# tohtsky/myFM

Hardware: AMD Instinct MI355X
Metric: Gibbs iterations/sec (rank=32) (higher is better)
Workload: dtype f64

## Files before the change

### include/myfm_hip.h

```cpp
#ifndef MYFM_HIP_H_
#define MYFM_HIP_H_

#include <stdint.h>

#ifdef __cplusplus
extern "C" {
#endif

#define MFM_OK 0
#define MFM_ERR_INVALID 1
#define MFM_ERR_RUNTIME 2
#define MFM_ERR_DEVICE 3

#define MFM_TASK_REGRESSION 0
#define MFM_TASK_CLASSIFICATION 1
#define MFM_TASK_ORDERED 2

typedef struct mfm_ctx mfm_ctx;
typedef struct mfm_design mfm_design;
typedef struct mfm_store mfm_store;

const char *mfm_version(void);
int mfm_device_count(void);
const char *mfm_global_error(void);

int mfm_create(int device, mfm_ctx **out);
void mfm_destroy(mfm_ctx *ctx);
const char *mfm_last_error(const mfm_ctx *ctx);
int mfm_get_device(const mfm_ctx *ctx);
int mfm_set_stream(mfm_ctx *ctx, void *hip_stream);
int mfm_synchronize(mfm_ctx *ctx);

int mfm_set_allreduce(mfm_ctx *ctx, int (*fn)(void *user, void *dev_buf, int64_t count), void *user);
int mfm_set_shard(mfm_ctx *ctx, int32_t rank, int32_t world);
int mfm_comm_unique_id(void *out128);
int mfm_comm_init(mfm_ctx *ctx, const void *id128, int32_t rank, int32_t world);
int mfm_comm_stats(const mfm_ctx *ctx, int64_t *calls, int64_t *doubles);
int mfm_comm_info(const mfm_ctx *ctx, int32_t *n_ranks, char *path, int64_t path_cap);
int mfm_peer_info(mfm_ctx *ctx, int32_t *pending, void **sum_buf, void **flag_buf, int64_t *sum_bytes, int64_t *flag_bytes);
int mfm_peer_set(mfm_ctx *ctx, int32_t world, int32_t rank, void *const *sum_bufs, void *const *flag_bufs);
int mfm_peer_model_info(mfm_ctx *ctx, void **w_buf, void **V_buf);
int mfm_peer_set_model(mfm_ctx *ctx, int32_t world, int32_t rank, void *const *w_bufs, void *const *V_bufs);
int mfm_peer_export(mfm_ctx *ctx, void *handles256);
int mfm_peer_import(mfm_ctx *ctx, int32_t world, int32_t rank, const void *all_handles);
int mfm_peer_drop(mfm_ctx *ctx);
int mfm_set_main_levels(mfm_ctx *ctx, const int32_t *level, int64_t D0);
int mfm_set_row_offset(mfm_ctx *ctx, int64_t first_global_row);

int mfm_set_main(mfm_ctx *ctx, int64_t N, int64_t D0, const int64_t *indptr, const int32_t *indices,
                 const double *data, const double *y);
int mfm_add_block(mfm_ctx *ctx, int64_t B, int64_t Db, const int64_t *indptr, const int32_t *indices,
                  const double *data, const int64_t *original_to_block);
int mfm_set_groups(mfm_ctx *ctx, const int32_t *group_index, int64_t D, int32_t G);
int mfm_set_residual_policy(mfm_ctx *ctx, int32_t recomputable);
int mfm_finalize(mfm_ctx *ctx, int32_t rank);

int64_t mfm_dim_all(const mfm_ctx *ctx);
int mfm_plan_info(const mfm_ctx *ctx, int64_t *n_levels_main, int64_t *n_launches_per_sweep);
int mfm_plan_flags(const mfm_ctx *ctx);
#define MFM_RES_INFO_FIELDS 13
int mfm_res_info(const mfm_ctx *ctx, int64_t *out, int n_out, char *why, int why_len);
#define MFM_CELL_INFO_FIELDS 74
int mfm_cell_info(const mfm_ctx *ctx, int64_t *out, int n_out, char *why, int why_len);

int mfm_set_state(mfm_ctx *ctx, double w0, const double *w, const double *V);
int mfm_get_state(mfm_ctx *ctx, double *w0, double *w, double *V);
int mfm_set_w0(mfm_ctx *ctx, double w0);
int mfm_zero_w(mfm_ctx *ctx);
int mfm_get_e(mfm_ctx *ctx, double *e);
int mfm_get_q(mfm_ctx *ctx, double *q);
int mfm_set_e(mfm_ctx *ctx, const double *e);

int mfm_reduce_e(mfm_ctx *ctx, double *sum_e, double *sum_e2);
int mfm_shift_e(mfm_ctx *ctx, double delta);
int mfm_group_stats_w(mfm_ctx *ctx, const double *mu_w, double *sum, double *ssd);
int mfm_group_stats_V(mfm_ctx *ctx, const double *mu_V, double *sum, double *ssd);
int mfm_hyper_stats(mfm_ctx *ctx, int32_t need_e, const double *mu_w, const double *mu_V, double *sum_e, double *sum_e2,
                    double *sum_w, double *ssd_w, double *sum_V, double *ssd_V);
int mfm_sweep_w(mfm_ctx *ctx, double alpha, const double *lambda_w, const double *mu_w, const double *z);
int mfm_sweep_V(mfm_ctx *ctx, int32_t f_begin, int32_t f_end, double alpha, const double *lambda_V,
                const double *mu_V, const double *z);
int mfm_sweep_wV(mfm_ctx *ctx, double alpha, double e_shift, const double *lambda_w, const double *mu_w, const double *zw,
                 int32_t f_begin, int32_t f_end, const double *lambda_V, const double *mu_V, const double *zv);

typedef struct mfm_hyper_prior {
  double alpha_0, beta_0, gamma_0, mu_0, reg_0, n_total;
  int32_t fit_w0, reserved;
} mfm_hyper_prior;
int mfm_regression_iteration_ready(mfm_ctx *ctx);
int mfm_regression_iteration(mfm_ctx *ctx, const mfm_hyper_prior *prior, const double *n_in_group, double *alpha, double *w0,
                             double *lambda_w, double *mu_w, double *lambda_V, double *mu_V);
int mfm_update_e_regression(mfm_ctx *ctx);
int mfm_update_e_classification(mfm_ctx *ctx, uint64_t seed, uint64_t draw_index);
int mfm_score_train(mfm_ctx *ctx);

int mfm_oprobit_add_group(mfm_ctx *ctx, int32_t n_class, const int64_t *rows, int64_t n_rows, int32_t *group);
int mfm_oprobit_eval(mfm_ctx *ctx, int32_t group, const double *gamma, double *ll, double *dgamma, double *H);
int mfm_oprobit_sample_z(mfm_ctx *ctx, int32_t group, const double *gamma, uint64_t seed, uint64_t draw_index);

#define MFM_RNG_NORMALS 0
#define MFM_RNG_GAMMA 1
#define MFM_RNG_LATENT 2
typedef struct mfm_rng_op {
  int32_t kind;
  int32_t dest;
  int64_t count;
  int64_t offset;
  double shape;
} mfm_rng_op;
int mfm_rng_prepare(int64_t n_features, int32_t rank, int32_t n_groups);
int mfm_rng_seed_mt19937(mfm_ctx *ctx, const uint32_t *state624, int32_t position);
int mfm_rng_set_program(mfm_ctx *ctx, const mfm_rng_op *ops, int32_t n_ops);
int mfm_rng_prefetch(mfm_ctx *ctx);
int mfm_rng_acquire(mfm_ctx *ctx, double *hyper_variates, int64_t n_hyper_variates);
int mfm_rng_get_z(mfm_ctx *ctx, double *zw, double *zv);

int mfm_update_e_classification_exact(mfm_ctx *ctx, int32_t *status);
int mfm_set_latent_order(mfm_ctx *ctx, const int64_t *rows, int64_t n);
int mfm_oprobit_sample_z_exact(mfm_ctx *ctx, int32_t group, const double *gamma, int32_t *status);
int mfm_latent_stats(mfm_ctx *ctx, int64_t *out8);
int mfm_rng_host_read(mfm_ctx *ctx, uint64_t offset, int64_t n, uint32_t *out);
int mfm_rng_host_advance(mfm_ctx *ctx, uint64_t words);

int mfm_timing_enable(mfm_ctx *ctx, int on);
int mfm_timing_select(mfm_ctx *ctx, int32_t kernel_class);
int mfm_timing_reset(mfm_ctx *ctx);
int mfm_timing_n_classes(void);
const char *mfm_timing_class_name(int cls);
int mfm_timing_get(mfm_ctx *ctx, int cls, double *ms_total, int64_t *launches, double *alg_bytes_total);

int mfm_design_create(int device, int64_t N, int64_t D0, const int64_t *indptr, const int32_t *indices,
                      const double *data, mfm_design **out);
int mfm_design_add_block(mfm_design *d, int64_t B, int64_t Db, const int64_t *indptr, const int32_t *indices,
                         const double *data, const int64_t *original_to_block);
void mfm_design_destroy(mfm_design *d);
const char *mfm_design_last_error(const mfm_design *d);
int64_t mfm_design_dim_all(const mfm_design *d);
int64_t mfm_design_n_rows(const mfm_design *d);
int mfm_design_predict(mfm_design *d, int32_t rank, int32_t n_samples, const double *w0s, const double *ws,
                       const double *Vs, int32_t mode, int32_t n_cut, const double *cutpoints, double *out);

int mfm_store_create(int device, int64_t D, int32_t rank, mfm_store **out);
void mfm_store_destroy(mfm_store *st);
const char *mfm_store_last_error(const mfm_store *st);
int32_t mfm_store_size(const mfm_store *st);
int mfm_store_reserve(mfm_store *st, int32_t n_samples);
int mfm_store_push_ctx(mfm_store *st, mfm_ctx *ctx);
int mfm_store_push_host(mfm_store *st, double w0, const double *w, const double *V);
int mfm_store_get(mfm_store *st, int32_t idx, double *w0, double *w, double *V);
int mfm_design_predict_store(mfm_design *d, mfm_store *st, int32_t first, int32_t count, int32_t mode, int32_t n_cut,
                             const double *cutpoints, double *out);

int mfm_design_summary_store(mfm_design *d, mfm_store *st, int32_t first, int32_t count, int32_t mode, int32_t n_q,
                             const double *probs, const double *precisions, const double *z, int64_t tile_rows,
                             int32_t chunk_samples, double *out_mean, double *out_std, double *out_q);
int mfm_design_summary(mfm_design *d, int32_t rank, int32_t n_samples, const double *w0s, const double *ws, const double *Vs,
                       int32_t mode, int32_t n_q, const double *probs, const double *precisions, const double *z,
                       int64_t tile_rows, int32_t chunk_samples, double *out_mean, double *out_std, double *out_q);

typedef struct mfm_pairs mfm_pairs;
int mfm_pairs_create(int device, int64_t D, int64_t U, const int64_t *q_indptr, const int32_t *q_indices, const double *q_data,
                     int64_t I, const int64_t *c_indptr, const int32_t *c_indices, const double *c_data, mfm_pairs **out);
void mfm_pairs_destroy(mfm_pairs *p);
const char *mfm_pairs_last_error(const mfm_pairs *p);
int mfm_pairs_set_exclude(mfm_pairs *p, const int64_t *indptr, const int32_t *indices);
int mfm_pairs_set_scratch_bound(mfm_pairs *p, int64_t bytes);
int mfm_pairs_add_block(mfm_pairs *p, int32_t side , int64_t col_offset, int64_t width, int64_t block_rows,
                        const int64_t *o2b , const int64_t *indptr, const int32_t *indices, const double *data);
int mfm_pairs_set_cutpoints(mfm_pairs *p, int32_t n_samples, int32_t n_cut, const double *cutpoints );
int mfm_pairs_scores_store(mfm_pairs *p, mfm_store *st, int32_t first, int32_t count, int32_t mode, double *out);
int mfm_pairs_topk_store(mfm_pairs *p, mfm_store *st, int32_t first, int32_t count, int32_t mode, int32_t k, int64_t *idx,
                         double *score);
int mfm_pairs_scores(mfm_pairs *p, int32_t rank, int32_t n_samples, const double *w0s, const double *ws, const double *Vs,
                     int32_t mode, double *out);
int mfm_pairs_topk(mfm_pairs *p, int32_t rank, int32_t n_samples, const double *w0s, const double *ws, const double *Vs,
                   int32_t mode, int32_t k, int64_t *idx, double *score);

int mfm_design_score_ctx(mfm_design *d, mfm_ctx *ctx, double *out);

int mfm_test_erfcx(int device, const double *x, int64_t n, double *out);
int mfm_test_truncated_normal(int device, int32_t kind, double lo, double hi, uint64_t seed, uint64_t draw_index,
                              int64_t n, double *out);

int mfm_host_column_levels(int64_t n_rows, int64_t n_cols, const int64_t *indptr, const int32_t *indices,
                           int32_t *level, int32_t *n_levels);
int mfm_cs_plan_selftest(int64_t n_rows, int32_t n_cols, const int64_t *colptr, const int32_t *rowidx, const double *val, int32_t cg,
                         int32_t lw, int32_t nb, int32_t rd, int32_t cap, double *max_rel_diff, int64_t *info);

typedef struct mfm_vb mfm_vb;
int mfm_vb_create(int device, int64_t N, int64_t D0, const int64_t *indptr, const int32_t *indices, const double *data,
                  const double *y, mfm_vb **out);
int mfm_vb_add_block(mfm_vb *v, int64_t B, int64_t Db, const int64_t *indptr, const int32_t *indices, const double *data,
                     const int64_t *original_to_block);
int mfm_vb_finalize(mfm_vb *v, const int32_t *group_index, int32_t G, int32_t rank);
int mfm_vb_set_stream(mfm_vb *v, void *hip_stream);
int mfm_vb_set_allreduce(mfm_vb *v, int (*fn)(void *user, void *dev_buf, int64_t count), void *user);
int mfm_vb_set_shard(mfm_vb *v, int32_t rank, int32_t world, int64_t n_total_rows, int64_t row_offset);
int mfm_vb_comm_init(mfm_vb *v, const void *id128, int32_t rank, int32_t world);
int mfm_vb_comm_stats(const mfm_vb *v, int64_t *calls, int64_t *doubles);
int mfm_vb_set_levels(mfm_vb *v, const int32_t *level, int64_t D);
int mfm_vb_design_levels(int64_t N, int64_t D0, const int64_t *indptr, const int32_t *indices, const double *data,
                         int32_t n_blocks, const int64_t *block_rows, const int64_t *block_cols,
                         const int64_t *const *block_indptr, const int32_t *const *block_indices,
                         const double *const *block_data, const int64_t *const *block_maps, int32_t *level_out,
                         int32_t *n_levels);
void mfm_vb_destroy(mfm_vb *v);
const char *mfm_vb_last_error(const mfm_vb *v);
int mfm_vb_plan_info(const mfm_vb *v, int64_t *n_levels, int64_t *n_launches_per_iteration);
int mfm_vb_set_state(mfm_vb *v, double w0, double w0_var, const double *w, const double *w_var, const double *V,
                     const double *V_var);
int mfm_vb_get_state(mfm_vb *v, double *w0, double *w0_var, double *w, double *w_var, double *V, double *V_var);
int mfm_vb_set_w0(mfm_vb *v, double w0, double w0_var);
int mfm_vb_update_e(mfm_vb *v, int32_t mode, double *out4);
int mfm_vb_shift_e(mfm_vb *v, double delta);
int mfm_vb_get_e(mfm_vb *v, double *e);
int mfm_vb_get_cache(mfm_vb *v, double *q, double *x2s, double *x3sv);
int mfm_vb_zero_w(mfm_vb *v);
int mfm_vb_sweep_w(mfm_vb *v, double alpha, const double *lambda_w, const double *mu_w);
int mfm_vb_sweep_V(mfm_vb *v, int32_t f_begin, int32_t f_end, double alpha, const double *lambda_V, const double *mu_V);
int mfm_vb_group_stats(mfm_vb *v, int32_t s_begin, int32_t s_end, const double *mu, const double *mu_var, double *out);
int mfm_vb_synchronize(mfm_vb *v);
int mfm_vb_truncated_normal(int32_t right, double mu, double *out3);

#ifdef __cplusplus
}
#endif
#endif
```

### myfm_amd/_capi.py

```python
import ctypes as C
import os

import numpy as np
import scipy.sparse as sps

_HERE = os.path.dirname(os.path.abspath(__file__))
LIB_PATH = os.path.join(_HERE, "libmyfm_hip.so")

MFM_OK, MFM_ERR_INVALID, MFM_ERR_RUNTIME, MFM_ERR_DEVICE = 0, 1, 2, 3
TASK_REGRESSION, TASK_CLASSIFICATION, TASK_ORDERED = 0, 1, 2

SYMBOLS = [
    "mfm_version", "mfm_device_count", "mfm_global_error", "mfm_create", "mfm_destroy", "mfm_last_error",
    "mfm_set_stream", "mfm_synchronize", "mfm_set_main", "mfm_add_block", "mfm_set_groups", "mfm_finalize",
    "mfm_peer_info", "mfm_peer_set", "mfm_peer_model_info", "mfm_peer_set_model", "mfm_peer_export", "mfm_peer_import", "mfm_peer_drop", "mfm_set_residual_policy", "mfm_dim_all", "mfm_plan_info", "mfm_plan_flags", "mfm_res_info", "mfm_cell_info", "mfm_set_state", "mfm_get_state", "mfm_set_w0", "mfm_zero_w", "mfm_get_e",
    "mfm_get_q", "mfm_set_e", "mfm_reduce_e", "mfm_shift_e", "mfm_group_stats_w", "mfm_group_stats_V",
    "mfm_sweep_w", "mfm_sweep_V", "mfm_sweep_wV", "mfm_update_e_regression", "mfm_update_e_classification", "mfm_score_train",
    "mfm_oprobit_add_group", "mfm_oprobit_eval", "mfm_oprobit_sample_z", "mfm_hyper_stats", "mfm_timing_enable", "mfm_timing_select", "mfm_timing_reset",
    "mfm_timing_n_classes", "mfm_timing_class_name", "mfm_timing_get", "mfm_design_create", "mfm_design_add_block",
    "mfm_design_destroy", "mfm_design_last_error", "mfm_design_dim_all", "mfm_design_predict",
    "mfm_host_column_levels", "mfm_rng_prepare", "mfm_rng_seed_mt19937", "mfm_rng_set_program", "mfm_rng_prefetch", "mfm_rng_acquire",
    "mfm_rng_get_z", "mfm_design_score_ctx", "mfm_design_n_rows", "mfm_set_allreduce", "mfm_set_row_offset", "mfm_set_main_levels",
    "mfm_test_erfcx", "mfm_test_truncated_normal", "mfm_get_device", "mfm_set_shard", "mfm_comm_unique_id", "mfm_comm_init",
    "mfm_comm_stats", "mfm_comm_info", "mfm_store_create", "mfm_store_destroy", "mfm_store_last_error", "mfm_store_size", "mfm_store_push_ctx",
# ... 113 lines not shown
    L.mfm_set_allreduce.argtypes = [vp, vp, vp]
    L.mfm_set_row_offset.argtypes = [vp, i64]
    L.mfm_set_main_levels.argtypes = [vp, P, i64]
    L.mfm_get_device.argtypes = [vp]
    L.mfm_set_shard.argtypes = [vp, i32, i32]
    L.mfm_comm_unique_id.argtypes = [P]
    L.mfm_comm_init.argtypes = [vp, P, i32, i32]
    L.mfm_comm_stats.argtypes = [vp, C.POINTER(i64), C.POINTER(i64)]
    L.mfm_comm_info.argtypes = [vp, C.POINTER(i32), C.c_char_p, i64]
    L.mfm_store_create.argtypes = [C.c_int, i64, i32, C.POINTER(vp)]
    L.mfm_store_destroy.argtypes = [vp]
    L.mfm_store_destroy.restype = None
    L.mfm_store_last_error.restype = C.c_char_p
    L.mfm_store_last_error.argtypes = [vp]
    L.mfm_store_size.argtypes = [vp]
    L.mfm_store_reserve.argtypes = [vp, i32]
    L.mfm_store_push_ctx.argtypes = [vp, vp]
    L.mfm_store_push_host.argtypes = [vp, dbl, P, P]
    L.mfm_store_get.argtypes = [vp, i32, C.POINTER(dbl), P, P]
    L.mfm_design_predict_store.argtypes = [vp, vp, i32, i32, i32, i32, P, P]
    L.mfm_design_summary_store.argtypes = [vp, vp, i32, i32, i32, i32, P, P, P, i64, i32, P, P, P]
    L.mfm_design_summary.argtypes = [vp, i32, i32, P, P, P, i32, i32, P, P, P, i64, i32, P, P, P]
    L.mfm_pairs_create.argtypes = [C.c_int, i64, i64, P, P, P, i64, P, P, P, C.POINTER(vp)]
    L.mfm_pairs_destroy.argtypes = [vp]
    L.mfm_pairs_destroy.restype = None
    L.mfm_pairs_last_error.restype = C.c_char_p
    L.mfm_pairs_last_error.argtypes = [vp]
    L.mfm_pairs_set_exclude.argtypes = [vp, P, P]
    L.mfm_pairs_set_scratch_bound.argtypes = [vp, i64]
    L.mfm_pairs_add_block.argtypes = [vp, i32, i64, i64, i64, P, P, P, P]
    L.mfm_pairs_set_cutpoints.argtypes = [vp, i32, i32, P]
    L.mfm_pairs_scores_store.argtypes = [vp, vp, i32, i32, i32, P]
    L.mfm_pairs_topk_store.argtypes = [vp, vp, i32, i32, i32, i32, P, P]
    L.mfm_pairs_scores.argtypes = [vp, i32, i32, P, P, P, i32, P]
    L.mfm_pairs_topk.argtypes = [vp, i32, i32, P, P, P, i32, i32, P, P]
    L.mfm_test_erfcx.argtypes = [C.c_int, P, i64, P]
    L.mfm_test_truncated_normal.argtypes = [C.c_int, i32, dbl, dbl, u64, u64, i64, P]
    _lib = L
    return L


def _p(a):
    return None if a is None else a.ctypes.data_as(C.c_void_p)


def _f64(a):
    return np.ascontiguousarray(a, dtype=np.float64)


def csr_parts(X):
    X = sps.csr_matrix(X, dtype=np.float64)
    return (
        X,
        np.ascontiguousarray(X.indptr, dtype=np.int64),
        np.ascontiguousarray(X.indices, dtype=np.int32),
        np.ascontiguousarray(X.data, dtype=np.float64),
    )


def _raise(code, msg):
    msg = msg.decode() if isinstance(msg, bytes) else msg
    if code == MFM_ERR_INVALID:
        raise ValueError(msg)
    raise RuntimeError(msg)


def column_levels(X):
    X, ip, ix, _ = csr_parts(X)
    level = np.zeros(X.shape[1], dtype=np.int32)
    n = C.c_int32()
    rc = lib().mfm_host_column_levels(X.shape[0], X.shape[1], _p(ip), _p(ix), _p(level), C.byref(n))
    if rc:
        _raise(rc, lib().mfm_global_error())
    return level, n.value


def device_erfcx(x, device=0):
    x = _f64(x)
    out = np.empty_like(x)
    rc = lib().mfm_test_erfcx(device, _p(x), x.size, _p(out))
    if rc:
        _raise(rc, lib().mfm_global_error())
    return out


def device_truncated_normal(kind, lo, hi, n, seed=1, draw_index=0, device=0):
    k = {"left": 0, "right": 1, "twoside": 2}[kind]
    out = np.empty(n)
    rc = lib().mfm_test_truncated_normal(device, k, float(lo), float(hi), seed, draw_index, n, _p(out))
    if rc:
        _raise(rc, lib().mfm_global_error())
    return out


class Context:

    def __init__(self, X, y, blocks=(), rank=4, group_index=None, device=0):
        L = lib()
        h = C.c_void_p()
        rc = L.mfm_create(device, C.byref(h))
        if rc:
            _raise(rc, L.mfm_global_error())
        self.h = h
        X, ip, ix, dv = csr_parts(X)
        y = _f64(y)
        self.N, self.D0 = X.shape
        self._ck(L.mfm_set_main(h, X.shape[0], X.shape[1], _p(ip), _p(ix), _p(dv), _p(y)))
        D = X.shape[1]
        for mp, B in blocks:
            B, bp, bx, bv = csr_parts(B)
            mp = np.ascontiguousarray(mp, dtype=np.int64)
            self._ck(L.mfm_add_block(h, B.shape[0], B.shape[1], _p(bp), _p(bx), _p(bv), _p(mp)))
            D += B.shape[1]
        if group_index is None:
            group_index = np.zeros(D, dtype=np.int32)
        group_index = np.ascontiguousarray(group_index, dtype=np.int32)
        self.G = int(group_index.max()) + 1 if D else 1
        self._ck(L.mfm_set_groups(h, _p(group_index), group_index.shape[0], self.G))
        self._ck(L.mfm_finalize(h, rank))
        self.D, self.K = D, rank

    def _ck(self, rc):
        if rc:
            _raise(rc, lib().mfm_last_error(self.h))

    def close(self):
        if getattr(self, "h", None):
            lib().mfm_destroy(self.h)
            self.h = None

    def __del__(self):
        try:
            self.close()
        except Exception:
            pass

    def set_state(self, w0, w, V):
        w = _f64(w)
        Vt = _f64(np.asarray(V, dtype=np.float64).T)
        self._ck(lib().mfm_set_state(self.h, float(w0), _p(w), _p(Vt)))

    def get_state(self):
        w0 = C.c_double()
        w = np.empty(self.D)
        V = np.empty((self.K, self.D))
        self._ck(lib().mfm_get_state(self.h, C.byref(w0), _p(w), _p(V)))
        return w0.value, w, np.ascontiguousarray(V.T)

    def set_w0(self, w0):
        self._ck(lib().mfm_set_w0(self.h, float(w0)))

    def zero_w(self):
        self._ck(lib().mfm_zero_w(self.h))

    def get_e(self):
        e = np.empty(self.N)
        self._ck(lib().mfm_get_e(self.h, _p(e)))
        return e

    def get_q(self):
        q = np.empty(self.N)
        self._ck(lib().mfm_get_q(self.h, _p(q)))
        return q

    def set_e(self, e):
        e = _f64(e)
        self._ck(lib().mfm_set_e(self.h, _p(e)))

    def reduce_e(self):
        a, b = C.c_double(), C.c_double()
        self._ck(lib().mfm_reduce_e(self.h, C.byref(a), C.byref(b)))
        return a.value, b.value

    def shift_e(self, delta):
        self._ck(lib().mfm_shift_e(self.h, float(delta)))

    def group_stats_w(self, mu_w):
        mu_w = _f64(mu_w)
        s, ss = np.empty(self.G), np.empty(self.G)
        self._ck(lib().mfm_group_stats_w(self.h, _p(mu_w), _p(s), _p(ss)))
        return s, ss

    def group_stats_V(self, mu_V):
        mu = _f64(np.asarray(mu_V).T)
        s, ss = np.empty((self.K, self.G)), np.empty((self.K, self.G))
        self._ck(lib().mfm_group_stats_V(self.h, _p(mu), _p(s), _p(ss)))
        return s.T.copy(), ss.T.copy()

    def sweep_w(self, alpha, lambda_w, mu_w, z):
        lambda_w, mu_w = _f64(lambda_w), _f64(mu_w)
        if z is not None:
            z = _f64(z)
            assert z.shape[0] == self.D
        self._ck(lib().mfm_sweep_w(self.h, float(alpha), _p(lambda_w), _p(mu_w), _p(z)))

    def sweep_V(self, f_begin, f_end, alpha, lambda_V, mu_V, z):
        lam, mu = _f64(np.asarray(lambda_V).T), _f64(np.asarray(mu_V).T)
        if z is not None:
            z = _f64(z)
            assert z.size == (f_end - f_begin) * self.D
        self._ck(lib().mfm_sweep_V(self.h, f_begin, f_end, float(alpha), _p(lam), _p(mu), _p(z)))

    def sweep_wV(self, alpha, e_shift, lambda_w, mu_w, zw, f_begin, f_end, lambda_V, mu_V, zv):
        lambda_w, mu_w = _f64(lambda_w), _f64(mu_w)
        lam, mu = _f64(np.asarray(lambda_V).T), _f64(np.asarray(mu_V).T)
        if zw is not None:
            zw, zv = _f64(zw), _f64(zv)
            assert zw.shape[0] == self.D and zv.size == (f_end - f_begin) * self.D
        self._ck(lib().mfm_sweep_wV(self.h, float(alpha), float(e_shift), _p(lambda_w), _p(mu_w), _p(zw), f_begin, f_end,
                                    _p(lam), _p(mu), _p(zv)))

    def update_e_regression(self):
        self._ck(lib().mfm_update_e_regression(self.h))

    def update_e_classification(self, seed, draw_index):
        self._ck(lib().mfm_update_e_classification(self.h, seed, draw_index))

    def score_train(self):
        self._ck(lib().mfm_score_train(self.h))

    def oprobit_add_group(self, n_class, rows=None):
        g = C.c_int32()
        if rows is None:
            self._ck(lib().mfm_oprobit_add_group(self.h, n_class, None, 0, C.byref(g)))
        else:
            rows = np.ascontiguousarray(rows, dtype=np.int64)
            self._ck(lib().mfm_oprobit_add_group(self.h, n_class, _p(rows), rows.shape[0], C.byref(g)))
        return g.value

    def oprobit_eval(self, group, gamma, want_h=True):
        gamma = _f64(gamma)
        m = gamma.shape[0]
        ll = C.c_double()
        dg = np.empty(m)
        H = np.empty((m, m)) if want_h else None
        self._ck(lib().mfm_oprobit_eval(self.h, group, _p(gamma), C.byref(ll), _p(dg), _p(H)))
        return ll.value, dg, H

    def oprobit_sample_z(self, group, gamma, seed, draw_index):
        gamma = _f64(gamma)
        self._ck(lib().mfm_oprobit_sample_z(self.h, group, _p(gamma), seed, draw_index))

    def synchronize(self):
        self._ck(lib().mfm_synchronize(self.h))

    RNG_OP = np.dtype([("kind", np.int32), ("dest", np.int32), ("count", np.int64), ("offset", np.int64), ("shape", np.float64)])

    def rng_seed_mt19937(self, state624, position):
        st = np.ascontiguousarray(state624, dtype=np.uint32)
        assert st.shape[0] == 624
        self._ck(lib().mfm_rng_seed_mt19937(self.h, _p(st), int(position)))

    def rng_set_program(self, ops):
        arr = np.array([tuple(o) for o in ops], dtype=self.RNG_OP)
        self._n_hv = int(sum(o[2] for o in ops if o[1] == 0))
        self._ck(lib().mfm_rng_set_program(self.h, _p(arr), len(ops)))

    def rng_prefetch(self):
        self._ck(lib().mfm_rng_prefetch(self.h))

    def rng_acquire(self):
        hv = np.empty(max(self._n_hv, 1))
        self._ck(lib().mfm_rng_acquire(self.h, _p(hv), self._n_hv))
        return hv[: self._n_hv]

    def rng_get_z(self):
        zw, zv = np.empty(self.D), np.empty((max(self.K, 1), self.D))
        self._ck(lib().mfm_rng_get_z(self.h, _p(zw), _p(zv)))
        return zw, zv[: self.K]

    def update_e_classification_exact(self):
        st = C.c_int32()
        self._ck(lib().mfm_update_e_classification_exact(self.h, C.byref(st)))
        return st.value

    def oprobit_sample_z_exact(self, group, gamma):
        gamma = _f64(gamma)
        st = C.c_int32()
        self._ck(lib().mfm_oprobit_sample_z_exact(self.h, group, _p(gamma), C.byref(st)))
        return st.value

    def latent_stats(self):
        out = np.zeros(8, dtype=np.int64)
        self._ck(lib().mfm_latent_stats(self.h, _p(out)))
        return dict(zip(("status", "chunks", "subs", "lq", "quads", "walkers", "attempts"), (int(v) for v in out)))

    def rng_host_read(self, offset, n):
        out = np.empty(max(int(n), 1), dtype=np.uint32)
        self._ck(lib().mfm_rng_host_read(self.h, int(offset), int(n), _p(out)))
        return out[: int(n)]

    def rng_host_advance(self, words):
        self._ck(lib().mfm_rng_host_advance(self.h, int(words)))

    def set_residual_policy(self, recomputable):
        self._ck(lib().mfm_set_residual_policy(self.h, 1 if recomputable else 0))

    def plan_flags(self):
        f = lib().mfm_plan_flags(self.h)
        return {"qfree": bool(f & 1), "unit": bool(f & 2), "ell": bool(f & 4), "sharded": bool(f & 8), "soa": bool(f & 16),
                "fused_next": bool(f & 32), "sharded_fused": bool(f & 64), "mf": bool(f & 128), "resident": bool(f & 256), "cell": bool(f & 512), "streamed_chain": bool(f & 1024), "resident_overflow": bool(f & 2048)}

    RES_INFO = ("ready", "G", "RV", "RL", "RX", "umax", "n_items", "item_bits", "n_runs", "max_wg_users", "max_slice_items",
                "e_where", "n_rows")
    E_WHERE = ("rows", "slots", "slots_with_sums", "cell", "dropped")

    def res_info(self):
        out = np.zeros(len(self.RES_INFO), dtype=np.int64)
        why = C.create_string_buffer(256)
        self._ck(lib().mfm_res_info(self.h, _p(out), out.shape[0], why, len(why)))
        d = dict(zip(self.RES_INFO, (int(v) for v in out)))
        d["ready"] = bool(d["ready"])
        d["e_where"] = self.E_WHERE[d["e_where"]]
        d["why"] = why.value.decode()
        return d

    CELL_INFO = ("ready", "G", "umax", "item32", "n_streams", "n_fields", "N", "Npad", "max_steps", "chunk_max", "chunk_min",
                 "chunks_empty", "split_mask", "score_fb")
    CELL_STREAM_TYPE = ("U", "I", "C")
    CELL_MAX_STREAMS, CELL_MAX_FIELDS = 4, 16
    CELL_INFO_FIELDS = len(CELL_INFO) + 3 * CELL_MAX_STREAMS + 3 * CELL_MAX_FIELDS

    def cell_info(self):
        out = np.zeros(self.CELL_INFO_FIELDS, dtype=np.int64)
        why = C.create_string_buffer(256)
        self._ck(lib().mfm_cell_info(self.h, _p(out), out.shape[0], why, len(why)))
        n = len(self.CELL_INFO)
        nf = n + 3 * self.CELL_MAX_STREAMS
        d = dict(zip(self.CELL_INFO, (int(v) for v in out[:n])))
        d["ready"], d["item32"] = bool(d["ready"]), bool(d["item32"])
        d["streams"] = [(self.CELL_STREAM_TYPE[int(out[n + 3 * s])], int(out[n + 3 * s + 1]), int(out[n + 3 * s + 2]))
                        for s in range(d["n_streams"])]
        d["fields"] = [tuple(int(x) for x in out[nf + 3 * k:nf + 3 * k + 3]) for k in range(d["n_fields"])]
        d["why"] = why.value.decode()
        return d

    def plan_info(self):
        a, b = C.c_int64(), C.c_int64()
        lib().mfm_plan_info(self.h, C.byref(a), C.byref(b))
        return a.value, b.value

    def timing_enable(self, on=True):
        self._ck(lib().mfm_timing_enable(self.h, int(on)))

    def timing_reset(self):
        self._ck(lib().mfm_timing_reset(self.h))

    def timing(self):
        L = lib()
        out = {}
        for c in range(L.mfm_timing_n_classes()):
            ms, n, by = C.c_double(), C.c_int64(), C.c_double()
            self._ck(L.mfm_timing_get(self.h, c, C.byref(ms), C.byref(n), C.byref(by)))
            if n.value:
                out[L.mfm_timing_class_name(c).decode()] = (ms.value, n.value, by.value)
        return out


class Design:

    def __init__(self, X, blocks=(), device=0):
        L = lib()
        h = C.c_void_p()
        X, ip, ix, dv = csr_parts(X)
        rc = L.mfm_design_create(device, X.shape[0], X.shape[1], _p(ip), _p(ix), _p(dv), C.byref(h))
        if rc:
            _raise(rc, L.mfm_global_error())
        self.h = h
        self.N = X.shape[0]
        for mp, B in blocks:
            B, bp, bx, bv = csr_parts(B)
            mp = np.ascontiguousarray(mp, dtype=np.int64)
            if mp.shape[0] != self.N:
                self.close()
                raise ValueError("Relation blocks have inconsistent mapper size with case_size")
            rc = L.mfm_design_add_block(h, B.shape[0], B.shape[1], _p(bp), _p(bx), _p(bv), _p(mp))
            if rc:
                msg = L.mfm_design_last_error(h)
                self.close()
                _raise(rc, msg)
        self.D = L.mfm_design_dim_all(h)

    def close(self):
        if getattr(self, "h", None):
            lib().mfm_design_destroy(self.h)
            self.h = None

    def __del__(self):
        try:
            self.close()
        except Exception:
            pass

    def score_ctx(self, ctx):
        out = np.empty(self.N)
        rc = lib().mfm_design_score_ctx(self.h, ctx.h, _p(out))
        if rc:
            _raise(rc, lib().mfm_design_last_error(self.h))
        return out

    def predict(self, samples, mode=0, cutpoints=None):
        K, S, w0s, ws, Vs = _pack_samples(samples)
        n_cut = 0
        cp = None
        if mode == 2:
            cp = _f64(np.stack([np.asarray(c, dtype=np.float64) for c in cutpoints]))
            n_cut = cp.shape[1]
        out = np.empty((self.N, n_cut + 1) if mode == 2 else self.N)
        rc = lib().mfm_design_predict(self.h, K, S, _p(w0s), _p(ws), _p(Vs), mode, n_cut, _p(cp), _p(out))
        if rc:
            _raise(rc, lib().mfm_design_last_error(self.h))
        return out

    def summary(self, samples, mode=0, quantiles=(), precisions=None, tile_rows=0, chunk_samples=0):
        K, S, w0s, ws, Vs = _pack_samples(samples)
        probs, prec, z, mean, std, q = _summary_args(self.N, quantiles, precisions)
        rc = lib().mfm_design_summary(self.h, K, S, _p(w0s), _p(ws), _p(Vs), mode, len(probs), _p(probs), _p(prec), _p(z),
                                      int(tile_rows), int(chunk_samples), _p(mean), _p(std), _p(q))
        if rc:
            _raise(rc, lib().mfm_design_last_error(self.h))
        return mean, std, q


def _summary_args(N, quantiles, precisions):
    from statistics import NormalDist

    probs = _f64(quantiles).reshape(-1)
    prec = None if precisions is None else _f64(precisions).reshape(-1)
    z = None
    if prec is not None:
        z = _f64([NormalDist().inv_cdf(float(p)) if 0.0 < p < 1.0 else np.nan for p in probs])
    return probs, prec, z, np.empty(N), np.empty(N), np.empty((len(probs), N))


class Store:

    def __init__(self, D, K, device=0):
        h = C.c_void_p()
        rc = lib().mfm_store_create(device, D, K, C.byref(h))
        if rc:
            _raise(rc, lib().mfm_global_error())
        self.h, self.D, self.K = h, D, K

    def close(self):
        if getattr(self, "h", None):
            lib().mfm_store_destroy(self.h)
            self.h = None

    def __del__(self):
        try:
            self.close()
        except Exception:
            pass

    def _ck(self, rc):
        if rc:
            _raise(rc, lib().mfm_store_last_error(self.h))

    def __len__(self):
        return lib().mfm_store_size(self.h)

    def push_ctx(self, ctx):
        self._ck(lib().mfm_store_push_ctx(self.h, ctx.h))

    def push(self, w0, w, V):
        w, Vt = _f64(w), _f64(np.asarray(V, dtype=np.float64).T)
        self._ck(lib().mfm_store_push_host(self.h, float(w0), _p(w), _p(Vt)))

    def get(self, idx):
        w0, w, V = C.c_double(), np.empty(self.D), np.empty((self.K, self.D))
        self._ck(lib().mfm_store_get(self.h, idx, C.byref(w0), _p(w), _p(V)))
        return w0.value, w, np.ascontiguousarray(V.T)

    def predict(self, design, mode=0, cutpoints=None, first=0, count=None):
        count = len(self) - first if count is None else count
        n_cut, cp = 0, None
        if mode == 2:
            cp = _f64(np.stack([np.asarray(c, dtype=np.float64) for c in cutpoints]))
            n_cut = cp.shape[1]
        out = np.empty((design.N, n_cut + 1) if mode == 2 else design.N)
        rc = lib().mfm_design_predict_store(design.h, self.h, first, count, mode, n_cut, _p(cp), _p(out))
        if rc:
            _raise(rc, lib().mfm_design_last_error(design.h))
        return out

    def summary(self, design, mode=0, quantiles=(), precisions=None, first=0, count=None, tile_rows=0, chunk_samples=0):
        count = len(self) - first if count is None else count
        probs, prec, z, mean, std, q = _summary_args(design.N, quantiles, precisions)
        rc = lib().mfm_design_summary_store(design.h, self.h, first, count, mode, len(probs), _p(probs), _p(prec), _p(z),
                                            int(tile_rows), int(chunk_samples), _p(mean), _p(std), _p(q))
        if rc:
            _raise(rc, lib().mfm_design_last_error(design.h))
        return mean, std, q


def _pack_samples(samples):
    S = len(samples)
    K = np.asarray(samples[0][2]).shape[1] if S else 0
    w0s = _f64([s[0] for s in samples])
    ws = _f64(np.stack([np.asarray(s[1], dtype=np.float64) for s in samples])) if S else np.empty(0)
    Vs = _f64(np.stack([np.asarray(s[2], dtype=np.float64).T for s in samples])) if S else np.empty(0)
    return K, S, w0s, ws, Vs


class Pairs:

    def __init__(self, X_query, X_cand, exclude=None, scratch_bound=None, device=0, rel_query=(), rel_cand=(), cutpoints=None):
        L = lib()
        h = C.c_void_p()
        Xq, qp, qx, qv = csr_parts(X_query)
        Xc, cp, cx, cv = csr_parts(X_cand)
        if Xq.shape[1] != Xc.shape[1]:
            raise ValueError("X_query and X_cand differ in width")
        rc = L.mfm_pairs_create(device, Xq.shape[1], Xq.shape[0], _p(qp), _p(qx), _p(qv), Xc.shape[0], _p(cp), _p(cx), _p(cv),
                                C.byref(h))
        if rc:
            _raise(rc, L.mfm_pairs_last_error(None))
        self.h, self.U, self.I, self.D = h, Xq.shape[0], Xc.shape[0], Xq.shape[1]
        if exclude is not None:
            E = sps.csr_matrix(exclude)
            if E.shape != (self.U, self.I):
                self.close()
                raise ValueError("exclude must have shape (n_queries, n_candidates)")
            ep = np.ascontiguousarray(E.indptr, dtype=np.int64)
            ex = np.ascontiguousarray(E.indices, dtype=np.int32)
            self._ck(L.mfm_pairs_set_exclude(h, _p(ep), _p(ex)))
        if scratch_bound is not None:
            self._ck(L.mfm_pairs_set_scratch_bound(h, int(scratch_bound)))
        try:
            for side, rels in ((0, rel_query), (1, rel_cand)):
                for off, o2b, B in rels:
                    B, bp, bx, bv = csr_parts(B)
                    o2b = np.ascontiguousarray(o2b, dtype=np.int64)
                    if o2b.shape != ((self.U, self.I)[side],):
                        raise ValueError("a block's o2b must have one entry per row of its side")
                    self._ck(L.mfm_pairs_add_block(h, side, int(off), B.shape[1], B.shape[0], _p(o2b), _p(bp), _p(bx), _p(bv)))
            if cutpoints is not None:
                cp = _f64(np.atleast_2d(np.asarray(cutpoints, dtype=np.float64)))
                self._ck(L.mfm_pairs_set_cutpoints(h, cp.shape[0], cp.shape[1], _p(cp)))
        except Exception:
            self.close()
            raise

    def _ck(self, rc):
        if rc:
            _raise(rc, lib().mfm_pairs_last_error(self.h))

    def close(self):
        if getattr(self, "h", None):
            lib().mfm_pairs_destroy(self.h)
            self.h = None

    def __del__(self):
        try:
            self.close()
        except Exception:
            pass

    def scores(self, samples, mode=0):
        K, S, w0s, ws, Vs = _pack_samples(samples)
        out = np.empty((self.U, self.I))
        self._ck(lib().mfm_pairs_scores(self.h, K, S, _p(w0s), _p(ws), _p(Vs), mode, _p(out)))
        return out

    def topk(self, samples, k, mode=0):
        K, S, w0s, ws, Vs = _pack_samples(samples)
        kk = max(int(k), 1)
        idx, val = np.empty((self.U, kk), dtype=np.int64), np.empty((self.U, kk))
        self._ck(lib().mfm_pairs_topk(self.h, K, S, _p(w0s), _p(ws), _p(Vs), mode, int(k), _p(idx), _p(val)))
        return idx, val

    def scores_store(self, store, mode=0, first=0, count=None):
        count = len(store) - first if count is None else count
        out = np.empty((self.U, self.I))
        self._ck(lib().mfm_pairs_scores_store(self.h, store.h, first, count, mode, _p(out)))
        return out

    def topk_store(self, store, k, mode=0, first=0, count=None):
        count = len(store) - first if count is None else count
        kk = max(int(k), 1)
        idx, val = np.empty((self.U, kk), dtype=np.int64), np.empty((self.U, kk))
        self._ck(lib().mfm_pairs_topk_store(self.h, store.h, first, count, mode, int(k), _p(idx), _p(val)))
        return idx, val
```

### myfm_amd/csrc/mfm_hip.hip

```cpp
#include <algorithm>
#include <cerrno>
#include <chrono>
#include <cmath>
#include <cstdio>
#include <cstring>
#include <map>
#include <memory>
#include <mutex>
#include <string>
#include <thread>
#include <type_traits>
#include <vector>

#include <fcntl.h>
#include <sys/file.h>
#include <sys/stat.h>
#include <unistd.h>

#include <hipcub/hipcub.hpp>

#include "mfm_common.hpp"
#include "mfm_kernels.hpp"
#include "mfm_plan.hpp"
#include "mfm_res_plan.hpp"
// ... 1273 lines not shown
    std::vector<int32_t> fs((size_t)c->D);
    std::vector<int64_t> cur(gptr.begin(), gptr.end() - 1);
    for (int64_t j = 0; j < c->D; j++) fs[cur[c->hgroup[j]]++] = (int32_t)j;
    c->group_ptr.upload(gptr);
    c->feat_sorted.upload(fs);
    int64_t big = 1;
    for (int g = 0; g < c->G; g++) big = std::max(big, gptr[g + 1] - gptr[g]);
    c->gs_chunks = (int)((big + GS_CHUNK - 1) / GS_CHUNK);
  }
  int64_t off = c->D0;
  int max_chunks = std::max(c->plan_V.max_hchunks, c->plan_W.max_hchunks);
  int max_long = std::max(c->plan_V.max_huge, c->plan_W.max_huge);
  {
    std::vector<std::unique_ptr<DevBlock>> built(c->hblocks.size());
    std::vector<std::exception_ptr> errs(c->hblocks.size());
    std::vector<int64_t> offs(c->hblocks.size());
    for (size_t b = 0; b < c->hblocks.size(); b++) {
      offs[b] = off;
      off += c->hblocks[b].X.cols;
    }
    auto build_one = [&](size_t b) {
      try {
        MFM_HIP_CHECK(hipSetDevice(c->device));
        built[b].reset(new DevBlock());
        built[b]->col_off = offs[b];
        built[b]->build(c->hblocks[b].X, c->hblocks[b].map.get(), c->N, c->KS, c->stream, c->cell_w,
                        b < c->pre_maps.size() ? &c->pre_maps[b] : nullptr);
      } catch (...) {
        errs[b] = std::current_exception();
      }
    };
    {
      (void)coop_capacity<PBlockV>();
      (void)coop_capacity<PBlockW>();
      std::vector<std::thread> pool;
      const bool par = c->hblocks.size() > 1;
      for (size_t b = 0; b < c->hblocks.size(); b++) {
        if (par && b + 1 < c->hblocks.size())
          pool.emplace_back(build_one, b);
        else
          build_one(b);
      }
      for (auto &t : pool) t.join();
    }
    for (size_t b = 0; b < built.size(); b++) {
      if (errs[b]) std::rethrow_exception(errs[b]);
      std::unique_ptr<DevBlock> &B = built[b];
      max_chunks = std::max({max_chunks, B->plan_V.max_hchunks, B->plan_W.max_hchunks});
      max_long = std::max({max_long, B->plan_V.max_huge, B->plan_W.max_huge});
      B->allreduce_fields(c->stream, c->comm, 6, 1);
      c->blocks.push_back(std::move(B));
    }
  }
  c->ls.reserve(std::max(max_chunks, 1), std::max(max_long, 1));
  c->w.alloc_zero((size_t)c->D, c->stream);
  c->V.alloc_zero((size_t)c->D * c->K, c->stream);
  c->Vt.alloc_zero((size_t)c->D * c->KS, c->stream);
  c->z.alloc((size_t)std::max<int64_t>(c->D, 1) * std::max(c->K, 1));
  c->lam.alloc((size_t)c->G * std::max(c->K, 1));
  c->mu.alloc((size_t)c->G * std::max(c->K, 1));
  c->red_partial.alloc(REDUCE_BLOCKS);
  c->red_out.alloc((size_t)1 + (size_t)c->G * std::max(c->K, 1));
  c->scratch_n.alloc((size_t)std::max<int64_t>(c->N, 1));
  if (c->v_path != VPath::Deferred) c->v_path = decide_main_paths(c);
  if (c->res.ready) {
    if (c->v_path != VPath::Deferred && env_flag("MFM_PLAN_CHECK")) {
      ResPlan chk;
      chk.build(Xt_keep, c->plan_V.h_level, &c->hgroup, c->res_plan_cus);
      const std::string diff = chk.ready ? res_plan_compare(c->res, chk, c->stream) : ("host builder: " + chk.why);
      if (!diff.empty()) throw Error(MFM_ERR_RUNTIME, "plan check: device and host resident layouts differ (" + diff + ")");
      lap("resident plan (host, check)");
    }
  } else if (!c->res_refused && c->v_path == VPath::TwoField && c->X.unit && c->N >= res_min_rows(c) && !env_flag("MFM_NO_RESIDENT")) {
    plan_resident(c, [&](ResPlan &rp, int n_cu) { rp.build(Xt_keep, c->plan_V.h_level, &c->hgroup, n_cu); }, tlog);
    lap("resident plan (host)");
  }
  if (c->v_path == VPath::ShardedTwoField && c->comm.shard_set && c->comm.world <= RES_MAX_PEERS && c->comm.world > 1 &&
      !env_flag("MFM_NO_RESIDENT") && !env_flag("MFM_NO_SHARDED_RESIDENT")) {
    const int64_t min_rows = res_min_rows(c);
    const bool want = c->X.unit && c->X.ell_width == 2 && c->N >= std::max<int64_t>(1, min_rows / c->comm.world) && c->K > 0;
    bool mine = false;
    if (want) {
      std::vector<char> draw_empty((size_t)c->D0, 0);
      for (int64_t j = 0; j < c->D0; j++) draw_empty[j] = (size_t)j < c->plan_V.special.size() && c->plan_V.special[j] == 2;
      plan_resident(c, [&](ResPlan &rp, int n_cu) {
        rp.allow_overflow = false;
        res_plan_build_device(rp, c->X, &c->hgroup, n_cu, c->stream, &c->hlevels, &draw_empty);
      }, tlog);
      if (c->res.ready && env_flag("MFM_PLAN_CHECK")) {
        ResPlan chk;
        chk.allow_overflow = false;
        chk.build(Xt_keep, c->hlevels, &c->hgroup, c->res_plan_cus, &draw_empty);
        const std::string diff = chk.ready ? res_plan_compare(c->res, chk, c->stream) : ("host builder: " + chk.why);
        if (!diff.empty()) throw Error(MFM_ERR_RUNTIME, "plan check: device and host resident layouts differ (sharded; " + diff + ")");
      }
      mine = c->res.ready;
      c->res.ready = false;
    }
    if (mine) {
      try {
        c->res.alloc_exchange(c->comm.world, c->comm.rank, c->stream);
      } catch (const Error &) {
        mine = false;
      }
    }
    double bad = mine ? 0.0 : 1.0;
    {
      DevBuf<double> d;
      d.upload(&bad, 1);
      c->comm.allreduce(d.p, 1);
      MFM_HIP_CHECK(hipStreamSynchronize(c->stream));
      MFM_HIP_CHECK(hipMemcpy(&bad, d.p, sizeof(double), hipMemcpyDeviceToHost));
    }
    if (bad == 0.0) {
      c->res_sharded_pending = true;
    } else {
      c->drop_resident();
    }
    lap("resident plan (row-sharded)");
  }
  Xt_keep = HostCsr();
  MFM_HIP_CHECK(hipStreamSynchronize(c->stream));
  lap("blocks, state, scratch");
  lap("(sync)");
  c->hX = HostCsr();
  c->hX_valid = false;
  c->hy = std::vector<double>();
  c->hblocks.clear();
  c->pre_maps.clear();
  lap("host copies released");
  c->finalized = true;
  MFM_CATCH(ctx)
}

int mfm_peer_info(mfm_ctx *ctx, int32_t *pending, void **sum_buf, void **flag_buf, int64_t *sum_bytes, int64_t *flag_bytes) {
  MFM_TRY(ctx)
  ctx->need_final();
  const bool p = ctx->res_sharded_pending;
  if (pending) *pending = p ? 1 : 0;
  if (sum_buf) *sum_buf = p ? (void *)ctx->res.xsum.p : nullptr;
  if (flag_buf) *flag_buf = p ? (void *)ctx->res.xflag.p : nullptr;
  if (sum_bytes) *sum_bytes = p ? (int64_t)(ctx->res.xsum.n * sizeof(double)) : 0;
  if (flag_bytes) *flag_bytes = p ? (int64_t)(ctx->res.xflag.n * sizeof(unsigned long long)) : 0;
  MFM_CATCH(ctx)
}

int mfm_peer_set(mfm_ctx *ctx, int32_t world, int32_t rank, void *const *sum_bufs, void *const *flag_bufs) {
  MFM_TRY(ctx)
  ctx->need_final();
  mfm_ctx *c = ctx;
  if (!c->res_sharded_pending) throw Error(MFM_ERR_RUNTIME, "mfm_peer_set: this context has no row-sharded persistent sweep waiting for its peers");
  if (world != c->res.xworld || rank != c->res.xrank) throw Error(MFM_ERR_INVALID, "mfm_peer_set: world / rank differ from the communicator's");
  for (int r = 0; r < world; r++) {
    if (!sum_bufs[r] || !flag_bufs[r]) throw Error(MFM_ERR_INVALID, "mfm_peer_set: null buffer");
    c->res.peer_sum[r] = (double *)sum_bufs[r];
    c->res.peer_flag[r] = (unsigned long long *)flag_bufs[r];
  }
  if (c->res.peer_sum[rank] != c->res.xsum.p || c->res.peer_flag[rank] != c->res.xflag.p)
    throw Error(MFM_ERR_INVALID, "mfm_peer_set: this rank's own entry must be the buffers of mfm_peer_info");
  MFM_HIP_CHECK(hipStreamSynchronize(c->stream));
  c->res.peers_set = true;
  c->res.ready = true;
  c->res_sharded_pending = false;
  MFM_CATCH(ctx)
}

int mfm_peer_set_model(mfm_ctx *ctx, int32_t world, int32_t rank, void *const *w_bufs, void *const *V_bufs) {
  MFM_TRY(ctx)
  ctx->need_final();
  mfm_ctx *c = ctx;
  if (!c->res.ready || !c->res.peers_set) throw Error(MFM_ERR_RUNTIME, "mfm_peer_set_model: mfm_peer_set comes first");
  if (world != c->res.xworld || rank != c->res.xrank) throw Error(MFM_ERR_INVALID, "mfm_peer_set_model: world / rank differ from the communicator's");
  for (int r = 0; r < world; r++) {
    if (!w_bufs[r] || (c->K > 0 && !V_bufs[r])) throw Error(MFM_ERR_INVALID, "mfm_peer_set_model: null buffer");
    c->res.peer_w[r] = (double *)w_bufs[r];
    c->res.peer_V[r] = (double *)V_bufs[r];
  }
  if (c->res.peer_w[rank] != c->w.p || c->res.peer_V[rank] != c->V.p)
    throw Error(MFM_ERR_INVALID, "mfm_peer_set_model: this rank's own entry must be its own w / V (mfm_peer_model_info)");
  MFM_HIP_CHECK(hipStreamSynchronize(c->stream));
  c->res.peers_model = true;
  MFM_CATCH(ctx)
}

int mfm_peer_model_info(mfm_ctx *ctx, void **w_buf, void **V_buf) {
  MFM_TRY(ctx)
  ctx->need_final();
  if (w_buf) *w_buf = ctx->w.p;
  if (V_buf) *V_buf = ctx->V.p;
  MFM_CATCH(ctx)
}

int mfm_peer_export(mfm_ctx *ctx, void *handles256) {
  MFM_TRY(ctx)
  ctx->need_final();
  if (!ctx->res_sharded_pending) throw Error(MFM_ERR_RUNTIME, "mfm_peer_export: no row-sharded persistent sweep waiting for its peers");
  static_assert(sizeof(hipIpcMemHandle_t) == 64, "IPC handle size");
  hipIpcMemHandle_t h[4];
  std::memset(h, 0, sizeof h);
  MFM_HIP_CHECK(hipIpcGetMemHandle(&h[0], ctx->res.xsum.p));
  MFM_HIP_CHECK(hipIpcGetMemHandle(&h[1], ctx->res.xflag.p));
  MFM_HIP_CHECK(hipIpcGetMemHandle(&h[2], ctx->w.p));
  if (ctx->K > 0) MFM_HIP_CHECK(hipIpcGetMemHandle(&h[3], ctx->V.p));
  std::memcpy(handles256, h, sizeof h);
  MFM_CATCH(ctx)
}

int mfm_peer_import(mfm_ctx *ctx, int32_t world, int32_t rank, const void *all_handles) {
  MFM_TRY(ctx)
  ctx->need_final();
  mfm_ctx *c = ctx;
  if (!c->res_sharded_pending) throw Error(MFM_ERR_RUNTIME, "mfm_peer_import: no row-sharded persistent sweep waiting for its peers");
  if (world != c->res.xworld || rank != c->res.xrank) throw Error(MFM_ERR_INVALID, "mfm_peer_import: world / rank differ from the communicator's");
  void *sums[RES_MAX_PEERS], *flags[RES_MAX_PEERS], *ws[RES_MAX_PEERS], *Vs[RES_MAX_PEERS];
  for (int r = 0; r < world; r++) {
    if (r == rank) {
      sums[r] = c->res.xsum.p;
      flags[r] = c->res.xflag.p;
      ws[r] = c->w.p;
      Vs[r] = c->V.p;
      continue;
    }
    hipIpcMemHandle_t h[4];
    std::memcpy(h, (const char *)all_handles + (size_t)r * 256, sizeof h);
    MFM_HIP_CHECK(hipIpcOpenMemHandle(&sums[r], h[0], hipIpcMemLazyEnablePeerAccess));
    c->res.peer_mapped.push_back(sums[r]);
    MFM_HIP_CHECK(hipIpcOpenMemHandle(&flags[r], h[1], hipIpcMemLazyEnablePeerAccess));
    c->res.peer_mapped.push_back(flags[r]);
    MFM_HIP_CHECK(hipIpcOpenMemHandle(&ws[r], h[2], hipIpcMemLazyEnablePeerAccess));
    c->res.peer_mapped.push_back(ws[r]);
    Vs[r] = nullptr;
    if (c->K > 0) {
      MFM_HIP_CHECK(hipIpcOpenMemHandle(&Vs[r], h[3], hipIpcMemLazyEnablePeerAccess));
      c->res.peer_mapped.push_back(Vs[r]);
    }
  }
  int rc = mfm_peer_set(ctx, world, rank, sums, flags);
  if (rc != MFM_OK) return rc;
  if (env_int("MYFM_PEER_MODEL", 0) != 0) {
    rc = mfm_peer_set_model(ctx, world, rank, ws, Vs);
    if (rc != MFM_OK) return rc;
  }
  MFM_CATCH(ctx)
}

int mfm_peer_drop(mfm_ctx *ctx) {
  MFM_TRY(ctx)
  ctx->need_final();
  MFM_HIP_CHECK(hipStreamSynchronize(ctx->stream));
  materialize_e(ctx);
  ctx->drop_resident();
  MFM_CATCH(ctx)
}

int mfm_set_residual_policy(mfm_ctx *ctx, int32_t recomputable) {
  if (!ctx) return MFM_ERR_INVALID;
  ctx->e_recomputable = recomputable != 0;
  return MFM_OK;
}

int64_t mfm_dim_all(const mfm_ctx *ctx) { return ctx->D; }

int mfm_plan_info(const mfm_ctx *ctx, int64_t *n_levels_main, int64_t *n_launches_per_sweep) {
  if (ctx->v_path == VPath::Deferred) {
    if (n_levels_main) *n_levels_main = 2;
    if (n_launches_per_sweep) *n_launches_per_sweep = 1;
    return MFM_OK;
  }
  if (n_levels_main) *n_levels_main = (int64_t)ctx->plan_V.n_levels;
  if (n_launches_per_sweep) {
    int64_t n = ctx->plan_V.launches;
    for (auto &B : ctx->blocks) n += B->plan_V.launches + 3;
    *n_launches_per_sweep = n;
  }
  return MFM_OK;
}

int mfm_plan_flags(const mfm_ctx *ctx) {
  bool streamed = false;
  for (auto &B : ctx->blocks)
    for (const Step &st : B->plan_V.steps) streamed = streamed || (st.is_chain && st.chain.stream);
  int form = 0;
  switch (ctx->v_path) {
    case VPath::QFree: form = 1; break;
    case VPath::Split: form = 16; break;
    case VPath::SplitFused: form = 16 | 32; break;
    case VPath::TwoField: form = 16 | 32 | 128; break;
    case VPath::ShardedSplit: form = 64; break;
    case VPath::ShardedTwoField: form = 64 | 128; break;
    case VPath::Deferred:
    case VPath::Generic:
    case VPath::Cell:
      break;
  }
  return (streamed ? 1024 : 0) | (ctx->res.ready && ctx->res.RX > 0 ? 2048 : 0) | form | (ctx->X.unit ? 2 : 0) | (ctx->X.ell_width >= 0 ? 4 : 0) |
         (ctx->comm.active() ? 8 : 0) | (ctx->res.ready ? 256 : 0) | (ctx->cell.ready ? 512 : 0);
}

int mfm_res_info(const mfm_ctx *ctx, int64_t *out, int n_out, char *why, int why_len) {
  if (!ctx || n_out < 0 || (n_out > 0 && !out) || why_len < 0 || (why_len > 0 && !why)) return MFM_ERR_INVALID;
  const ResPlan &rp = ctx->res;
  const int64_t v[MFM_RES_INFO_FIELDS] = {rp.ready ? 1 : 0, rp.G,       rp.RV,     rp.RL,           rp.RX,
                                          rp.umax,          rp.n_items, rp.item_bits, rp.n_runs,    rp.max_wg_users,
                                          rp.max_slice_items, (int64_t)ctx->e_where, rp.n_rows};
  for (int i = 0; i < n_out; i++) out[i] = i < MFM_RES_INFO_FIELDS ? v[i] : 0;
  if (why_len > 0) {
    std::strncpy(why, rp.ready ? "" : rp.why.c_str(), (size_t)why_len - 1);
    why[why_len - 1] = 0;
  }
  return MFM_OK;
}

int mfm_cell_info(const mfm_ctx *ctx, int64_t *out, int n_out, char *why, int why_len) {
  if (!ctx || n_out < 0 || (n_out > 0 && !out) || why_len < 0 || (why_len > 0 && !why)) return MFM_ERR_INVALID;
  const CellPlan &cp = ctx->cell;
  int64_t v[MFM_CELL_INFO_FIELDS] = {0};
  const int m = (int)cp.fields.size(), ns = (int)cp.streams.size();
  int64_t split = 0;
  const bool typed = ns > 0 && cp.sU == 0;
  for (int k = 0; k < m && typed; k++)
    if (cp.split_pass(k == 0 ? m - 1 : k - 1, k, k == 0)) split |= (int64_t)1 << k;
  const int64_t head[14] = {cp.ready ? 1 : 0, cp.G,         cp.umax,      cp.item32 ? 1 : 0, ns,    m, cp.N, cp.Npad, cp.max_steps,
                            cp.chunk_max,     cp.chunk_min, cp.chunks_empty, split,          cp.ready ? cp.score_fb() : 0};
  for (int i = 0; i < 14; i++) v[i] = head[i];
  for (int i = 0; i < ns && i < CELL_MAX_STREAMS; i++) {
    v[14 + 3 * i] = cp.streams[i].type;
    v[15 + 3 * i] = cp.streams[i].slot;
    v[16 + 3 * i] = cp.streams[i].card;
  }
  for (int k = 0; k < m && k < CELL_MAX_FIELDS; k++) {
    v[14 + 3 * CELL_MAX_STREAMS + 3 * k] = cp.fields[k].stream;
    v[15 + 3 * CELL_MAX_STREAMS + 3 * k] = cp.fields[k].kind;
    v[16 + 3 * CELL_MAX_STREAMS + 3 * k] = cp.fields[k].n;
  }
  for (int i = 0; i < n_out; i++) out[i] = i < MFM_CELL_INFO_FIELDS ? v[i] : 0;
  if (why_len > 0) {
    std::strncpy(why, cp.ready ? "" : cp.why.c_str(), (size_t)why_len - 1);
    why[why_len - 1] = 0;
  }
  return MFM_OK;
}

int mfm_set_state(mfm_ctx *ctx, double w0, const double *w, const double *V) {
  MFM_TRY(ctx)
  ctx->need_final();
  ctx->w0 = w0;
  ctx->ring.upload(ctx->w.p, w, (size_t)ctx->D * sizeof(double), ctx->stream);
  if (ctx->K) ctx->ring.upload(ctx->V.p, V, (size_t)ctx->D * ctx->K * sizeof(double), ctx->stream);
  MFM_CATCH(ctx)
}

int mfm_get_state(mfm_ctx *ctx, double *w0, double *w, double *V) {
  MFM_TRY(ctx)
  ctx->need_final();
  *w0 = ctx->w0;
  if (ctx->D)
    MFM_HIP_CHECK(hipMemcpyAsync(w, ctx->w.p, (size_t)ctx->D * sizeof(double), hipMemcpyDeviceToHost, ctx->stream));
  if (ctx->K && ctx->D)
    MFM_HIP_CHECK(
        hipMemcpyAsync(V, ctx->V.p, (size_t)ctx->D * ctx->K * sizeof(double), hipMemcpyDeviceToHost, ctx->stream));
  ctx->sync_and_check();
  MFM_CATCH(ctx)
}

int mfm_set_w0(mfm_ctx *ctx, double w0) {
  MFM_TRY(ctx)
  if (w0 != ctx->w0) ensure_e(ctx);
  ctx->w0 = w0;
  MFM_CATCH(ctx)
}

int mfm_zero_w(mfm_ctx *ctx) {
  MFM_TRY(ctx)
  ctx->need_final();
  if (ctx->D) MFM_HIP_CHECK(hipMemsetAsync(ctx->w.p, 0, (size_t)ctx->D * sizeof(double), ctx->stream));
  MFM_CATCH(ctx)
}

static int get_eq(mfm_ctx *ctx, double *dst, int which) {
  MFM_TRY(ctx)
  ctx->need_final();
  materialize_e(ctx);
  if (ctx->N) {
    hipLaunchKernelGGL(k_get_eq, dim3(cdiv(ctx->N, WG)), dim3(WG), 0, ctx->stream, ctx->eq_rows(), ctx->scratch_n.p, ctx->N,
                       which);
    MFM_HIP_CHECK(
        hipMemcpyAsync(dst, ctx->scratch_n.p, (size_t)ctx->N * sizeof(double), hipMemcpyDeviceToHost, ctx->stream));
    MFM_HIP_CHECK(hipStreamSynchronize(ctx->stream));
  }
  MFM_CATCH(ctx)
}
int mfm_get_e(mfm_ctx *ctx, double *e) { return get_eq(ctx, e, 0); }
int mfm_get_q(mfm_ctx *ctx, double *q) {
  if (ctx->finalized && ctx->q_stale_factor >= 0) {
    try {
      ctx->use_device();
      for (auto &B : ctx->blocks)
        if (ctx->cell.ready) block_rowcache(ctx->stream, ctx->timing, *B, ctx->V.p + (size_t)ctx->q_stale_factor * ctx->D + B->col_off, true);
      launch_qbuild(ctx, ctx->V.p + (size_t)ctx->q_stale_factor * ctx->D);
      ctx->q_stale_factor = -1;
    } catch (const std::exception &ex) {
      ctx->err = ex.what();
      return MFM_ERR_RUNTIME;
    }
  }
  return get_eq(ctx, q, 1);
}
int mfm_set_e(mfm_ctx *ctx, const double *e) {
  MFM_TRY(ctx)
  ctx->need_final();
  if (ctx->e_where == EWhere::Dropped) ctx->e_where = EWhere::Rows;
  ctx->e_is_residual = false;
  materialize_e(ctx);
  if (ctx->N) {
    MFM_HIP_CHECK(hipStreamSynchronize(ctx->stream));
    MFM_HIP_CHECK(hipMemcpy(ctx->scratch_n.p, e, (size_t)ctx->N * sizeof(double), hipMemcpyHostToDevice));
    hipLaunchKernelGGL(k_set_eq, dim3(cdiv(ctx->N, WG)), dim3(WG), 0, ctx->stream, ctx->eq_rows(), ctx->scratch_n.p, ctx->N, 0);
    MFM_HIP_CHECK(hipStreamSynchronize(ctx->stream));
  }
  MFM_CATCH(ctx)
}

int mfm_reduce_e(mfm_ctx *ctx, double *sum_e, double *sum_e2) {
  MFM_TRY(ctx)
  ctx->need_final();
  materialize_e(ctx);
  hipStream_t s = ctx->stream;
  {
    TimedLaunch t(ctx->timing, s, KC_REDUCE_E, 8.0 * ctx->N);
    hipLaunchKernelGGL(k_reduce_e_partial, dim3(REDUCE_BLOCKS), dim3(WG), 0, s, ctx->eq_rows(), ctx->N, ctx->red_partial.p);
    hipLaunchKernelGGL(k_reduce_final, dim3(1), dim3(WG), 0, s, ctx->red_partial.p, REDUCE_BLOCKS, ctx->red_out.p);
  }
  ctx->comm.allreduce(ctx->red_out.p, 2);
  double2 *h = ctx->readback(2);
  MFM_HIP_CHECK(hipMemcpyAsync(h, ctx->red_out.p, sizeof(double2), hipMemcpyDeviceToHost, s));
  MFM_HIP_CHECK(hipMemcpyAsync(h + 1, ctx->ls.error.p, sizeof(int), hipMemcpyDeviceToHost, s));
  MFM_HIP_CHECK(hipStreamSynchronize(s));
  ctx->check_coresident(*(const int *)(h + 1));
  *sum_e = h[0].x;
  *sum_e2 = h[0].y;
  MFM_CATCH(ctx)
}

int mfm_shift_e(mfm_ctx *ctx, double delta) {
  MFM_TRY(ctx)
  ctx->need_final();
  materialize_e(ctx);
  ctx->e_is_residual = false;
  if (ctx->N) {
    TimedLaunch t(ctx->timing, ctx->stream, KC_SHIFT_E, 16.0 * ctx->N);
    hipLaunchKernelGGL(k_shift_e, dim3(cdiv(ctx->N, WG)), dim3(WG), 0, ctx->stream, ctx->eq_rows(), ctx->N, delta);
    MFM_HIP_CHECK(hipGetLastError());
  }
  MFM_CATCH(ctx)
}

static int group_stats(mfm_ctx *ctx, const double *theta, int nf, const double *mu_host, double *sum, double *ssd) {
  MFM_TRY(ctx)
  ctx->need_final();
  hipStream_t s = ctx->stream;
  const int G = ctx->G;
  if (nf > 0) {
    ctx->ring.upload(ctx->mu.p, mu_host, (size_t)G * nf * sizeof(double), s);
    {
      TimedLaunch t(ctx->timing, s, KC_GROUP_STATS, 12.0 * ctx->D * nf);
      const int n_ch = std::max(1, ctx->gs_chunks);
      if (ctx->gs_partial.n < (size_t)G * nf * n_ch) ctx->gs_partial.alloc((size_t)G * nf * n_ch);
      hipLaunchKernelGGL(k_group_stats, dim3(G, nf, n_ch), dim3(WG), 0, s, theta, ctx->D, ctx->feat_sorted.p,
                         ctx->group_ptr.p, ctx->mu.p, G, ctx->gs_partial.p);
      hipLaunchKernelGGL(k_group_stats_final, dim3(cdiv(G * nf, 64)), dim3(64), 0, s, ctx->gs_partial.p, G * nf, n_ch,
                         ctx->red_out.p + 1);
    }
    if (ctx->res.peers_model && ctx->comm.active()) ctx->comm.allreduce(ctx->red_out.p, 1);
    double2 *h = ctx->readback((size_t)G * nf + 1);
    MFM_HIP_CHECK(hipMemcpyAsync(h, ctx->red_out.p + 1, (size_t)G * nf * sizeof(double2), hipMemcpyDeviceToHost, s));
    MFM_HIP_CHECK(hipStreamSynchronize(s));
    for (int i = 0; i < G * nf; i++) {
      sum[i] = h[i].x;
      ssd[i] = h[i].y;
    }
  }
  MFM_CATCH(ctx)
}
int mfm_group_stats_w(mfm_ctx *ctx, const double *mu_w, double *sum, double *ssd) {
  return group_stats(ctx, ctx->w.p, 1, mu_w, sum, ssd);
}
int mfm_group_stats_V(mfm_ctx *ctx, const double *mu_V, double *sum, double *ssd) {
  return group_stats(ctx, ctx->V.p, ctx->K, mu_V, sum, ssd);
}

int mfm_hyper_stats(mfm_ctx *ctx, int32_t need_e, const double *mu_w, const double *mu_V, double *sum_e, double *sum_e2,
                    double *sum_w, double *ssd_w, double *sum_V, double *ssd_V) {
  MFM_TRY(ctx)
  ctx->need_final();
  mfm_ctx *c = ctx;
  const bool slot_sums = need_e && c->e_where == EWhere::SlotsWithSums;
  if (need_e && !slot_sums) materialize_e(ctx);
  hipStream_t s = c->stream;
  const int G = c->G, K = c->K, n_ch = std::max(1, c->gs_chunks);
  const size_t n_out = 1 + (size_t)G * (K + 1);
  if (c->hs_out.n < n_out) c->hs_out.alloc(n_out);
  if (c->hs_mu.n < (size_t)G * (K + 1)) c->hs_mu.alloc((size_t)G * (K + 1));
  if (c->gs_partial.n < (size_t)G * (K + 1) * n_ch) c->gs_partial.alloc((size_t)G * (K + 1) * n_ch);
  {
    c->hs_stage.resize((size_t)G * (K + 1));
    std::memcpy(c->hs_stage.data(), mu_w, (size_t)G * sizeof(double));
    if (K) std::memcpy(c->hs_stage.data() + G, mu_V, (size_t)G * K * sizeof(double));
    c->ring.upload(c->hs_mu.p, c->hs_stage.data(), c->hs_stage.size() * sizeof(double), s);
  }
  {
    TimedLaunch t(c->timing, s, KC_GROUP_STATS, 12.0 * c->D * (K + 1));
    hipLaunchKernelGGL(k_group_stats, dim3(G, 1, n_ch), dim3(WG), 0, s, c->w.p, c->D, c->feat_sorted.p, c->group_ptr.p,
                       c->hs_mu.p, G, c->gs_partial.p);
    if (K)
      hipLaunchKernelGGL(k_group_stats, dim3(G, K, n_ch), dim3(WG), 0, s, c->V.p, c->D, c->feat_sorted.p, c->group_ptr.p,
                         c->hs_mu.p + G, G, c->gs_partial.p + (size_t)G * n_ch);
    hipLaunchKernelGGL(k_group_stats_final, dim3(cdiv(G * (K + 1), 64)), dim3(64), 0, s, c->gs_partial.p, G * (K + 1), n_ch,
                       c->hs_out.p + 1);
  }
  if (slot_sums) {
    TimedLaunch t(c->timing, s, KC_REDUCE_E, 16.0 * c->res.G);
    hipLaunchKernelGGL(k_reduce_final, dim3(1), dim3(WG), 0, s, c->res.sums.p, c->res.G, c->hs_out.p);
    c->comm.allreduce(c->hs_out.p, 2);
  } else if (need_e) {
    TimedLaunch t(c->timing, s, KC_REDUCE_E, 8.0 * c->N);
    hipLaunchKernelGGL(k_reduce_e_partial, dim3(REDUCE_BLOCKS), dim3(WG), 0, s, c->eq_rows(), c->N, c->red_partial.p);
    hipLaunchKernelGGL(k_reduce_final, dim3(1), dim3(WG), 0, s, c->red_partial.p, REDUCE_BLOCKS, c->hs_out.p);
    c->comm.allreduce(c->hs_out.p, 2);
  }
  if (!need_e && c->res.peers_model && c->comm.active()) c->comm.allreduce(c->hs_out.p, 1);
  MFM_HIP_CHECK(hipGetLastError());
  double2 *h = c->readback(n_out + 1);
  MFM_HIP_CHECK(hipMemcpyAsync(h, c->hs_out.p, n_out * sizeof(double2), hipMemcpyDeviceToHost, s));
  MFM_HIP_CHECK(hipMemcpyAsync(h + n_out, c->ls.error.p, sizeof(int), hipMemcpyDeviceToHost, s));
  MFM_HIP_CHECK(hipStreamSynchronize(s));
  c->check_coresident(*(const int *)(h + n_out));
  if (need_e) {
    *sum_e = h[0].x;
    *sum_e2 = h[0].y;
  }
  for (int g = 0; g < G; g++) {
    sum_w[g] = h[1 + g].x;
    ssd_w[g] = h[1 + g].y;
  }
  for (int i = 0; i < G * K; i++) {
    sum_V[i] = h[1 + G + i].x;
    ssd_V[i] = h[1 + G + i].y;
  }
  MFM_CATCH(ctx)
}

static void sync_model_sharded(mfm_ctx *c, bool with_w, int f_begin, int f_end) {
  hipStream_t s = c->stream;
  if (with_w) {
    hipLaunchKernelGGL(k_mask_rows, dim3(cdiv(c->D, 256)), dim3(256), 0, s, c->w.p, c->sync_mask.p, c->D, c->D);
    c->comm.allreduce(c->w.p, c->D);
  }
  if (f_end > f_begin) {
    const int64_t n = (int64_t)(f_end - f_begin) * c->D;
    double *Vb = c->V.p + (size_t)f_begin * c->D;
    hipLaunchKernelGGL(k_mask_rows, dim3(cdiv(n, 256)), dim3(256), 0, s, Vb, c->sync_mask.p, c->D, n);
    c->comm.allreduce(Vb, n);
  }
}

struct ResidentLinear {
  double *w = nullptr;
  const double *zw = nullptr, *lam_w = nullptr, *mu_w = nullptr;
  double e_shift = 0.0;
};
static void launch_resident(mfm_ctx *c, int f_begin, int f_end, const double *zbase, const double *lam, const double *mu, double alpha,
                            const ResidentLinear &lin = ResidentLinear(), const double *hyp = nullptr) {
  ensure_e(c);
  const mfm_ctx::ResidentE e = c->e_for_resident(lin.w != nullptr, f_begin, f_end);
  run_sweep_resident(c->stream, c->timing, c->res, KC_SWEEP_V_RESIDENT, c->eq_raw(), c->V.p, c->D, f_begin, f_end, zbase, lam, mu,
                     c->group.p, c->G, alpha, c->ls.error.p, lin.w, lin.zw, lin.lam_w, lin.mu_w, lin.e_shift, e.load_slots, e.no_store,
                     hyp);
  c->e_left_by_resident(e);
  c->q_stale_factor = f_end - 1;
  if (c->comm.active() && !c->res.peers_model) sync_model_sharded(c, lin.w != nullptr, f_begin, f_end);
}

int mfm_sweep_w(mfm_ctx *ctx, double alpha, const double *lambda_w, const double *mu_w, const double *z) {
  MFM_TRY(ctx)
  ctx->need_final();
  if (!ctx->cell_w) materialize_e(ctx);
  mfm_ctx *c = ctx;
  hipStream_t s = c->stream;
  c->ring.upload(c->lam.p, lambda_w, (size_t)c->G * sizeof(double), s);
  c->ring.upload(c->mu.p, mu_w, (size_t)c->G * sizeof(double), s);
  const double *zdev = c->z.p;
  if (z) {
    c->ring.upload(c->z.p, z, (size_t)c->D * sizeof(double), s);
  } else {
    if (c->rng.current < 0 || c->rng.n_zw != c->D)
      throw Error(MFM_ERR_RUNTIME, "mfm_sweep_w(z = NULL) needs an acquired device random set with D z_w variates");
    zdev = c->rng.slot[c->rng.current].zw.p;
  }
  if (c->cell_w) {
    run_sweep_w_cell(c, zdev, alpha);
    return MFM_OK;
  }
  c->ensure_main_plans();
  SweepArgs a = main_args(c, c->w.p, zdev, c->lam.p, c->mu.p, alpha);
  const SweepClasses kcw{KC_SWEEP_W_LIGHT, KC_SWEEP_W_HEAVY, KC_SWEEP_W_COOP, KC_SWEEP_W_LSTATS, KC_SWEEP_W_LDRAW,
                         KC_SWEEP_W_LAPPLY, KC_SWEEP_W_CHAIN, KC_SWEEP_W_SCAT};
  if (c->comm.active())
// ... 627 lines not shown
```

### myfm_amd/csrc/mfm_res.hpp

```cpp
#pragma once
#include <algorithm>
#include <cstdlib>
#include <cstring>
#include <atomic>
#include <string>
#include <thread>
#include <vector>

#include "mfm_common.hpp"
#include "mfm_mf_kernels.hpp"

namespace mfm {

#ifndef MFM_RES_CH
#define MFM_RES_CH 4
#endif
constexpr int RES_MAX_PEERS = 8;

struct ResArgs {
  double2 *eq;
  const double *e_in;
  double *e_slots;
  const int32_t *perm;
  const uint32_t *uidw;
  const uint32_t *headw;
  const int32_t *run_item;
  const int32_t *first_run;
  const int32_t *wg_run_ptr;
  const int32_t *wg_nruns;
  const int32_t *wg_user_ptr;
  const int2 *user_desc;
  const int32_t *wg_item_ptr;
  const int32_t *ent_ptr;
  const int2 *entries;
  const int32_t *scols;
  const int2 *item_desc;
  double *partials;
  double *dv;
  double *V;
  int64_t D;
  int f_begin, f_end;
  int linear;
  int n_sw;
  double *w;
  const double *zw;
  const double *lam_w, *mu_w;
  double e_shift;
  const double *z;
  const double *lam, *mu;
  const int32_t *group;
  int n_groups;
  double alpha;
  const double *scal;
  int n_items, umax;
  unsigned long long *bar;
  int n_wg;
  int *error;
  unsigned long long *prof;
  int xworld, xrank;
  unsigned long long xepoch0;
  double *xsum[RES_MAX_PEERS];
  unsigned long long *xflag[RES_MAX_PEERS];
  unsigned long long *xarrive;
  int xmodel;
  double *xw[RES_MAX_PEERS], *xV[RES_MAX_PEERS];
  int ngx;
  int no_store;
  int xch_break;
};

__device__ __forceinline__ void res_store2(double *p, double a, double b) {
  __hip_atomic_store(p, a, __ATOMIC_RELAXED, __HIP_MEMORY_SCOPE_AGENT);
  __hip_atomic_store(p + 1, b, __ATOMIC_RELAXED, __HIP_MEMORY_SCOPE_AGENT);
}

enum { RES_BAR_START = 0, RES_BAR_TOP = 16, RES_BAR_XCNT = 32, RES_BAR_GEN = 160, RES_BAR_CENSUS = 288, RES_BAR_WORDS = 416 };
struct ResBar {
  int xcc;
  unsigned long long n_x, nx;
};

__device__ __forceinline__ bool res_spin(const ResArgs &a, const unsigned long long *w, unsigned long long target, bool &dead) {
  unsigned spins = 0;
  while (__hip_atomic_load(w, __ATOMIC_RELAXED, __HIP_MEMORY_SCOPE_AGENT) < target) {
#ifndef MFM_RES_NO_SLEEP
    __builtin_amdgcn_s_sleep(1);
#endif
    if ((++spins & 1023u) == 0u) {
      if (spins > (1u << 22) || __hip_atomic_load(a.error, __ATOMIC_RELAXED, __HIP_MEMORY_SCOPE_AGENT) != 0) {
        __hip_atomic_store(a.error, 1, __ATOMIC_RELAXED, __HIP_MEMORY_SCOPE_AGENT);
        dead = true;
        return false;
      }
    }
  }
  return true;
}

__device__ __forceinline__ bool res_spin_sys(const ResArgs &a, const unsigned long long *w, unsigned long long target, bool &dead) {
  unsigned spins = 0;
  while (__hip_atomic_load(w, __ATOMIC_RELAXED, __HIP_MEMORY_SCOPE_SYSTEM) < target) {
    __builtin_amdgcn_s_sleep(2);
    if ((++spins & 1023u) == 0u) {
      const int seen = __hip_atomic_load(a.error, __ATOMIC_RELAXED, __HIP_MEMORY_SCOPE_AGENT);
      if (spins > (1u << 23) || seen != 0) {
        if (seen == 0) __hip_atomic_store(a.error, 2, __ATOMIC_RELAXED, __HIP_MEMORY_SCOPE_AGENT);
        dead = true;
        return false;
      }
    }
  }
  return true;
}

__device__ __forceinline__ void res_bar_init(const ResArgs &a, ResBar &rb, bool &dead) {
  unsigned x;
  asm volatile("s_getreg_b32 %0, hwreg(HW_REG_XCC_ID, 0, 4)" : "=s"(x));
  rb.xcc = (int)(x & 7u);
  __hip_atomic_fetch_add(a.bar + RES_BAR_CENSUS + 16 * rb.xcc, 1ull, __ATOMIC_RELAXED, __HIP_MEMORY_SCOPE_AGENT);
  asm volatile("s_waitcnt vmcnt(0)" ::: "memory");
  __hip_atomic_fetch_add(a.bar + RES_BAR_START, 1ull, __ATOMIC_RELAXED, __HIP_MEMORY_SCOPE_AGENT);
  rb.n_x = 1;
  rb.nx = 1;
  if (!res_spin(a, a.bar + RES_BAR_START, (unsigned long long)a.n_wg, dead)) return;
  rb.nx = 0;
  for (int i = 0; i < 8; i++) {
    const unsigned long long c = __hip_atomic_load(a.bar + RES_BAR_CENSUS + 16 * i, __ATOMIC_RELAXED, __HIP_MEMORY_SCOPE_AGENT);
    rb.nx += c > 0 ? 1 : 0;
    if (i == rb.xcc) rb.n_x = c;
  }
}

__device__ __forceinline__ void res_grid_barrier(const ResArgs &a, const ResBar &rb, unsigned long long k, int tid, bool &dead) {
  asm volatile("s_waitcnt vmcnt(0)" ::: "memory");
  __syncthreads();
  if (tid == 0 && !dead) {
    const unsigned long long old =
        __hip_atomic_fetch_add(a.bar + RES_BAR_XCNT + 16 * rb.xcc, 1ull, __ATOMIC_RELAXED, __HIP_MEMORY_SCOPE_AGENT);
    if (old + 1 == k * rb.n_x) {
      __builtin_amdgcn_fence(__ATOMIC_RELEASE, "agent");
      asm volatile("s_waitcnt vmcnt(0)" ::: "memory");
      __hip_atomic_fetch_add(a.bar + RES_BAR_TOP, 1ull, __ATOMIC_RELAXED, __HIP_MEMORY_SCOPE_AGENT);
      if (res_spin(a, a.bar + RES_BAR_TOP, k * rb.nx, dead))
        __hip_atomic_store(a.bar + RES_BAR_GEN + 16 * rb.xcc, k, __ATOMIC_RELAXED, __HIP_MEMORY_SCOPE_AGENT);
    } else {
      res_spin(a, a.bar + RES_BAR_GEN + 16 * rb.xcc, k, dead);
    }
    __builtin_amdgcn_fence(__ATOMIC_ACQUIRE, "agent");
  }
  __syncthreads();
}

typedef double res_d16_t __attribute__((ext_vector_type(16)));
typedef unsigned res_u4_t __attribute__((ext_vector_type(4)));

template <int NT, int NGV, int NGL, bool XCH = false, bool OVF = false>
__global__ __launch_bounds__(NT) void k_mf_resident(ResArgs a) {
  extern __shared__ __attribute__((aligned(16))) char res_smem[];
  constexpr int NW = NT / WAVE, NG = NGV + NGL, R = 16 * NG, RL = 16 * NGL;
  constexpr int B = 4;
  const int g = (int)blockIdx.x, tid = threadIdx.x, lane = tid & 63;
  const int wv = __builtin_amdgcn_readfirstlane(tid >> 6);
  const int U = a.umax;
  const double alpha_k = a.scal ? a.scal[0] : a.alpha, e_shift_k = a.scal ? a.scal[2] : a.e_shift;
  const int ngx = OVF ? a.ngx : 0, NGt = NG + ngx, Rt = 16 * NGt;
  d2_t *utab = (d2_t *)res_smem;
  double *elds = (double *)(utab + U);
  double *acc1 = elds + (size_t)RL * NT;
  double *acc2 = acc1 + NW * U;
  d2_t *wcarry = (d2_t *)(acc2 + NW * U);
  int *wflag = (int *)(wcarry + NW);
  const int32_t *perm_g = a.perm + (int64_t)g * Rt * NT;
  const int u0 = a.wg_user_ptr[g], nu = a.wg_user_ptr[g + 1] - u0;
  const int rb0 = a.wg_run_ptr[g];
  const int pad_item = a.n_items;
  const unsigned rb0b = 4u * (unsigned)rb0, padb = 16u * (unsigned)pad_item;
  const char *run_item_b = (const char *)a.run_item, *dv_b = (const char *)a.dv;
  double *acc1w = acc1 + wv * U, *acc2w = acc2 + wv * U;
  bool dead = false;
  unsigned long long nbar = 0;
  ResBar rbar;
  rbar.xcc = 0;
  rbar.n_x = rbar.nx = 1;
#define RES_STAMP0(k) \
  if (a.prof && tid == 0) a.prof[(int64_t)g * a.n_sw * 64 + 56 + (k)] = __builtin_amdgcn_s_memrealtime()
  RES_STAMP0(0);
  if (tid == 0) res_bar_init(a, rbar, dead);
  RES_STAMP0(1);
  const int wv_hi = wv >> 2;
#define RES_PRIO(j)                  \
  if ((((j) & 1) ^ wv_hi) != 0)      \
    __builtin_amdgcn_s_setprio(1);   \
  else                               \
    __builtin_amdgcn_s_setprio(0)
  const int trash_run = a.wg_run_ptr[g] + a.wg_nruns[g];
#define RES_STAMP(k)                                                                                      \
  if (a.prof && tid == 0) a.prof[((int64_t)g * a.n_sw + (f - f_first)) * 64 + (k)] = __builtin_amdgcn_s_memrealtime()

  for (int i = tid; i < 2 * NW * U; i += NT) acc1[i] = 0.0;
  for (int i = tid; i < U; i += NT) utab[i] = d2_t{0.0, 0.0};

  res_u4_t uw[NG];
  unsigned ux[NG];
  unsigned hbv[NG], nbv[NG];
#pragma unroll
  for (int j = 0; j < NG; j++) {
#pragma unroll
    for (int w = 0; w < 4; w++) uw[j][w] = a.uidw[((int64_t)g * (5 * NGt) + 5 * j + w) * NT + tid];
    ux[j] = a.uidw[((int64_t)g * (5 * NGt) + 5 * j + 4) * NT + tid];
    hbv[j] = a.headw[((int64_t)g * NGt + j) * NT + tid];
    nbv[j] = hbv[j] | (j == 0 ? 1u : 0u);
  }
  const unsigned nbx0 = OVF && ngx > 0 ? a.headw[((int64_t)g * NGt + NG) * NT + tid] : 0u;
  double *eog = OVF ? a.e_slots + ((int64_t)g * Rt + 16 * NG) * NT + tid : nullptr;
  const uint32_t *uidw_x = a.uidw + ((int64_t)g * (5 * NGt) + 5 * NG) * NT + tid;
  const uint32_t *headw_x = a.headw + ((int64_t)g * NGt + NG) * NT + tid;
  const int run0 = a.first_run[g * NT + tid];
  const bool head0 = (hbv[0] & 1u) != 0u;
#define RES_NIB(j, q) ((((nbv[j]) | ((j) + 1 < NG ? nbv[(j) + 1 < NG ? (j) + 1 : (j)] << 16 : nbx0 << 16)) >> (4 * (q))) & 15u)
#define RES_UIDS(j, bb, uid)                                                     \
  {                                                                              \
    const unsigned lo_ = uw[j][bb];                                              \
    uid[0] = (int)(lo_ & 0x3ffu);                                                \
    uid[1] = (int)((lo_ >> 10) & 0x3ffu);                                        \
    uid[2] = (int)((lo_ >> 20) & 0x3ffu);                                        \
    uid[3] = (int)((lo_ >> 30) | (((ux[j] >> (8 * (bb))) & 0xffu) << 2));        \
  }

#define RES_UIDSX(bb, uid)                                                       \
  {                                                                              \
    const unsigned lo_ = uwx[bb];                                                \
    uid[0] = (int)(lo_ & 0x3ffu);                                                \
    uid[1] = (int)((lo_ >> 10) & 0x3ffu);                                        \
    uid[2] = (int)((lo_ >> 20) & 0x3ffu);                                        \
    uid[3] = (int)((lo_ >> 30) | (((uxx >> (8 * (bb))) & 0xffu) << 2));          \
  }

#define RES_OPAQUE()                                                                            \
  _Pragma("unroll") for (int j_ = 0; j_ < NG; j_++) {                                           \
    asm volatile("" : "+v"(uw[j_]), "+v"(ux[j_]), "+v"(hbv[j_]), "+v"(nbv[j_]));                \
  }
  res_d16_t ev[NGV > 0 ? NGV : 1];
#pragma unroll
  for (int j = 0; j < NG; j++) {
#pragma unroll 1
    for (int bb = 0; bb < 4; bb++) {
      int row[B];
#pragma unroll
      for (int k = 0; k < B; k++) row[k] = a.e_in ? 0 : perm_g[(16 * j + 4 * bb + k) * NT + tid];
#pragma unroll
      for (int k = 0; k < B; k++) {
        const double x = (a.e_in ? a.e_in[((int64_t)g * Rt + 16 * j + 4 * bb + k) * NT + tid] : a.eq[row[k] < 0 ? 0 : row[k]].x) + e_shift_k;
        if (j < NGV)
          ev[j < NGV ? j : 0][4 * bb + k] = x;
        else
          elds[(16 * (j - NGV) + 4 * bb + k) * NT + tid] = x;
      }
    }
  }
  if (OVF) {
    for (int jx = 0; jx < ngx; jx++) {
#pragma unroll 4
      for (int i = 0; i < 16; i++) {
        const int64_t sl = 16 * (NG + jx) + i;
        const int row = a.e_in ? 0 : perm_g[sl * NT + tid];
        const double x = (a.e_in ? a.e_in[((int64_t)g * Rt + sl) * NT + tid] : a.eq[row < 0 ? 0 : row].x) + e_shift_k;
        eog[(16 * jx + i) * NT] = x;
      }
    }
  }
  __syncthreads();

  RES_STAMP0(2);
  const int f_first = a.f_begin - a.linear;
  for (int f = f_first; f < a.f_end; f++) {
    const bool lin = f < a.f_begin;
    double *Vf = lin ? a.w : a.V + (int64_t)f * a.D;
    const double *zf = lin ? a.zw : a.z + (int64_t)(f - a.f_begin) * a.D;
    const double *lamf = lin ? a.lam_w : a.lam + (int64_t)f * a.n_groups;
    const double *muf = lin ? a.mu_w : a.mu + (int64_t)f * a.n_groups;
    int uj = 0;
    double uold = 0.0, uz = 0.0, ulam = 0.0, umu = 0.0;
    if (tid < nu) {
      const int2 d = a.user_desc[u0 + tid];
      uj = d.x;
      uold = Vf[uj];
      uz = zf[uj];
      ulam = lamf[d.y];
      umu = muf[d.y];
    }
    RES_STAMP(0);
    {
      RES_OPAQUE();
      asm volatile(";; res sweep A");
      unsigned rcb = 4u * (unsigned)(run0 - 1);
      int itA[B];
      d2_t ddA[B];
      {
        int it0[B];
        const unsigned n0 = RES_NIB(0, 0), n1 = RES_NIB(0, 1);
#pragma unroll
        for (int k = 0; k < B; k++) {
          rcb += ((n0 >> k) & 1u) << 2;
          it0[k] = *(const int *)(run_item_b + ((n0 >> k) & 1u ? rcb : rb0b));
        }
#pragma unroll
        for (int k = 0; k < B; k++) {
          rcb += ((n1 >> k) & 1u) << 2;
          itA[k] = *(const int *)(run_item_b + ((n1 >> k) & 1u ? rcb : rb0b));
        }
#pragma unroll
        for (int k = 0; k < B; k++) ddA[k] = *(const d2_t *)(dv_b + ((n0 >> k) & 1u ? (unsigned)it0[k] << 4 : padb));
      }
      d2_t ddc = d2_t{0.0, 0.0};
      int itB[B];
      d2_t ddB[B];
#define RES_STEP_A(j, bb, iti, ito, ddi, ddo)                                                                              \
  {                                                                                                                        \
    const unsigned n4 = RES_NIB(j, bb), n4a = RES_NIB(j, (bb) + 1), n4b = RES_NIB(j, (bb) + 2);                            \
    _Pragma("unroll") for (int k = 0; k < B; k++) {                                                                        \
      rcb += ((n4b >> k) & 1u) << 2;                                                                                       \
      ito[k] = *(const int *)(run_item_b + ((n4b >> k) & 1u ? rcb : rb0b));                                                \
    }                                                                                                                      \
    _Pragma("unroll") for (int k = 0; k < B; k++)                                                                          \
      ddo[k] = *(const d2_t *)(dv_b + ((n4a >> k) & 1u ? (unsigned)iti[k] << 4 : padb));                                   \
    int uid[B];                                                                                                            \
    RES_UIDS(j, bb, uid);                                                                                                  \
    double up[B], ex[B];                                                                                                   \
    _Pragma("unroll") for (int k = 0; k < B; k++) {                                                                        \
      up[k] = utab[uid[k]][0];                                                                                             \
      ex[k] = j < NGV ? ev[j < NGV ? j : 0][4 * (bb) + k] : elds[(16 * (j - NGV) + 4 * (bb) + k) * NT + tid];              \
    }                                                                                                                      \
    _Pragma("unroll") for (int k = 0; k < B; k++) {                                                                        \
      const bool need = ((n4 >> k) & 1u) != 0u;                                                                            \
      ddc[0] = need ? ddi[k][0] : ddc[0];                                                                                  \
      ddc[1] = need ? ddi[k][1] : ddc[1];                                                                                  \
      const double er = ex[k] + up[k] * ddc[0];                                                                            \
      if (j < NGV)                                                                                                         \
        ev[j < NGV ? j : 0][4 * (bb) + k] = er;                                                                            \
      else                                                                                                                 \
        elds[(16 * (j - NGV) + 4 * (bb) + k) * NT + tid] = er;                                                             \
      const double c = ddc[1];                                                                                             \
      __hip_atomic_fetch_add(&acc1w[uid[k]], (-er) * c, __ATOMIC_RELAXED, __HIP_MEMORY_SCOPE_WORKGROUP);                   \
      __hip_atomic_fetch_add(&acc2w[uid[k]], c * c, __ATOMIC_RELAXED, __HIP_MEMORY_SCOPE_WORKGROUP);                       \
    }                                                                                                                      \
  }
#define RES_STEP_AX(bb, iti, ito, ddi, ddo)                                                                                 \
  {                                                                                                                        \
    const unsigned n4 = ((nbw >> (4 * (bb))) & 15u), n4a = ((nbw >> (4 * ((bb) + 1))) & 15u), n4b = ((nbw >> (4 * ((bb) + 2))) & 15u);                            \
    _Pragma("unroll") for (int k = 0; k < B; k++) {                                                                        \
      rcb += ((n4b >> k) & 1u) << 2;                                                                                       \
      ito[k] = *(const int *)(run_item_b + ((n4b >> k) & 1u ? rcb : rb0b));                                                \
    }                                                                                                                      \
    _Pragma("unroll") for (int k = 0; k < B; k++)                                                                          \
      ddo[k] = *(const d2_t *)(dv_b + ((n4a >> k) & 1u ? (unsigned)iti[k] << 4 : padb));                                   \
    int uid[B];                                                                                                            \
    RES_UIDSX(bb, uid);                                                                                                      \
    double up[B], ex[B];                                                                                                   \
    _Pragma("unroll") for (int k = 0; k < B; k++) {                                                                        \
      up[k] = utab[uid[k]][0];                                                                                             \
      ex[k] = eo[4 * (bb) + k];              \
    }                                                                                                                      \
    _Pragma("unroll") for (int k = 0; k < B; k++) {                                                                        \
      const bool need = ((n4 >> k) & 1u) != 0u;                                                                            \
      ddc[0] = need ? ddi[k][0] : ddc[0];                                                                                  \
      ddc[1] = need ? ddi[k][1] : ddc[1];                                                                                  \
      const double er = ex[k] + up[k] * ddc[0];                                                                            \
      eo[4 * (bb) + k] = er;                                                             \
      const double c = ddc[1];                                                                                             \
      __hip_atomic_fetch_add(&acc1w[uid[k]], (-er) * c, __ATOMIC_RELAXED, __HIP_MEMORY_SCOPE_WORKGROUP);                   \
      __hip_atomic_fetch_add(&acc2w[uid[k]], c * c, __ATOMIC_RELAXED, __HIP_MEMORY_SCOPE_WORKGROUP);                       \
    }                                                                                                                      \
  }
#pragma unroll
      for (int j = 0; j < NG; j++) {
        RES_PRIO(j);
#pragma unroll
        for (int bp = 0; bp < 2; bp++) {
          RES_STEP_A(j, 2 * bp, itA, itB, ddA, ddB);
          RES_STEP_A(j, 2 * bp + 1, itB, itA, ddB, ddA);
        }
      }
      asm volatile(";; res sweep end");
      if (OVF) {
        unsigned hb_c = nbx0;
        for (int jx = 0; jx < ngx; jx++) {
          res_u4_t uwx;
#pragma unroll
          for (int w = 0; w < 4; w++) uwx[w] = uidw_x[(5 * jx + w) * NT];
          const unsigned uxx = uidw_x[(5 * jx + 4) * NT];
          const unsigned hb_n = jx + 1 < ngx ? headw_x[(jx + 1) * NT] : 0u;
          const unsigned nbw = hb_c | (hb_n << 16);
          res_d16_t eo;
#pragma unroll
          for (int i = 0; i < 16; i++) eo[i] = eog[(16 * jx + i) * NT];
#pragma unroll 1
          for (int bp = 0; bp < 2; bp++) {
            RES_STEP_AX(2 * bp, itA, itB, ddA, ddB);
            RES_STEP_AX(2 * bp + 1, itB, itA, ddB, ddA);
          }
#pragma unroll
          for (int i = 0; i < 16; i++) eog[(16 * jx + i) * NT] = eo[i];
          hb_c = hb_n;
        }
      }
#undef RES_STEP_A
#undef RES_STEP_AX
    }
    __syncthreads();
    RES_STAMP(1);
    if (tid < nu) {
      double S1 = 0.0, S2 = 0.0;
#pragma unroll
      for (int w = 0; w < NW; w++) {
        S1 += acc1[w * U + tid];
        S2 += acc2[w * U + tid];
        acc1[w * U + tid] = 0.0;
        acc2[w * U + tid] = 0.0;
      }
      const double fresh = PMainV::draw(S1, S2, uold, alpha_k, ulam, umu, uz);
      Vf[uj] = fresh;
      if (XCH && a.xmodel) {
        for (int r = 0; r < a.xworld; r++)
          if (r != a.xrank)
            __hip_atomic_store((lin ? a.xw[r] : a.xV[r] + (int64_t)f * a.D) + uj, fresh, __ATOMIC_RELAXED, __HIP_MEMORY_SCOPE_SYSTEM);
      }
      utab[tid] = d2_t{lin ? 1.0 : fresh, fresh - uold};
    }
    __syncthreads();
    RES_STAMP(2);
    {
      bool have_head = false;
      double f1 = 0.0, f2 = 0.0, s1 = 0.0, s2 = 0.0;
      d2_t *part2 = (d2_t *)a.partials;
      char *part_b = (char *)a.partials - 16;
      const unsigned trashb = 16u * (unsigned)(trash_run + 1);
      {
        RES_OPAQUE();
        asm volatile(";; res sweep B");
        unsigned rcb = 4u * (unsigned)(run0 - 1);
        unsigned rcCb = 16u * (unsigned)(run0 - 1);
        int itA[B];
        double ccA[B];
        {
          int it0[B];
          const unsigned n0 = RES_NIB(0, 0), n1 = RES_NIB(0, 1);
#pragma unroll
          for (int k = 0; k < B; k++) {
            rcb += ((n0 >> k) & 1u) << 2;
            it0[k] = *(const int *)(run_item_b + ((n0 >> k) & 1u ? rcb : rb0b));
          }
#pragma unroll
          for (int k = 0; k < B; k++) {
            rcb += ((n1 >> k) & 1u) << 2;
            itA[k] = *(const int *)(run_item_b + ((n1 >> k) & 1u ? rcb : rb0b));
          }
#pragma unroll
          for (int k = 0; k < B; k++) ccA[k] = *(const double *)(dv_b + 8 + ((n0 >> k) & 1u ? (unsigned)it0[k] << 4 : padb));
        }
        double ccc = 0.0;
        int itB[B];
        double ccB[B];
#define RES_PARTIAL_STORE() *(d2_t *)(part_b + (head && have_head ? rcCb : trashb)) = d2_t{s1, s2}
#define RES_STEP_B(j, bb, iti, ito, cci, cco)                                                                              \
  {                                                                                                                        \
    const unsigned n4 = RES_NIB(j, bb), n4a = RES_NIB(j, (bb) + 1), n4b = RES_NIB(j, (bb) + 2);                            \
    const unsigned h4 = (hbv[j] >> (4 * (bb))) & 15u;                                                                      \
    _Pragma("unroll") for (int k = 0; k < B; k++) {                                                                        \
      rcb += ((n4b >> k) & 1u) << 2;                                                                                       \
      ito[k] = *(const int *)(run_item_b + ((n4b >> k) & 1u ? rcb : rb0b));                                                \
    }                                                                                                                      \
    _Pragma("unroll") for (int k = 0; k < B; k++)                                                                          \
      cco[k] = *(const double *)(dv_b + 8 + ((n4a >> k) & 1u ? (unsigned)iti[k] << 4 : padb));                             \
    int uid[B];                                                                                                            \
    RES_UIDS(j, bb, uid);                                                                                                  \
    d2_t ut[B];                                                                                                            \
    double ex[B];                                                                                                          \
    _Pragma("unroll") for (int k = 0; k < B; k++) {                                                                        \
      ut[k] = utab[uid[k]];                                                                                                \
      ex[k] = j < NGV ? ev[j < NGV ? j : 0][4 * (bb) + k] : elds[(16 * (j - NGV) + 4 * (bb) + k) * NT + tid];              \
    }                                                                                                                      \
    _Pragma("unroll") for (int k = 0; k < B; k++) {                                                                        \
      const bool need = ((n4 >> k) & 1u) != 0u;                                                                            \
      const bool head = ((h4 >> k) & 1u) != 0u;                                                                            \
      ccc = need ? cci[k] : ccc;                                                                                           \
      rcCb += need ? 16u : 0u;                                                         \
                              \
      RES_PARTIAL_STORE();                                                                                                 \
      f1 = head && !have_head ? s1 : f1;                                                                                   \
      f2 = head && !have_head ? s2 : f2;                                                                                   \
      have_head = have_head || head;                                                                                       \
      const double er = ex[k] + ccc * ut[k][1];                                                                            \
      if (j < NGV)                                                                                                         \
        ev[j < NGV ? j : 0][4 * (bb) + k] = er;                                                                            \
      else                                                                                                                 \
        elds[(16 * (j - NGV) + 4 * (bb) + k) * NT + tid] = er;                                                             \
      s1 = (head ? 0.0 : s1) + (-er) * ut[k][0];                                                                           \
      s2 = (head ? 0.0 : s2) + ut[k][0] * ut[k][0];                                                                        \
    }                                                                                                                      \
  }
#define RES_STEP_BX(bb, iti, ito, cci, cco)                                                                                 \
  {                                                                                                                        \
    const unsigned n4 = ((nbw >> (4 * (bb))) & 15u), n4a = ((nbw >> (4 * ((bb) + 1))) & 15u), n4b = ((nbw >> (4 * ((bb) + 2))) & 15u);                            \
    const unsigned h4 = (hb_c >> (4 * (bb))) & 15u;                                                                       \
    _Pragma("unroll") for (int k = 0; k < B; k++) {                                                                        \
      rcb += ((n4b >> k) & 1u) << 2;                                                                                       \
      ito[k] = *(const int *)(run_item_b + ((n4b >> k) & 1u ? rcb : rb0b));                                                \
    }                                                                                                                      \
    _Pragma("unroll") for (int k = 0; k < B; k++)                                                                          \
      cco[k] = *(const double *)(dv_b + 8 + ((n4a >> k) & 1u ? (unsigned)iti[k] << 4 : padb));                             \
    int uid[B];                                                                                                            \
    RES_UIDSX(bb, uid);                                                                                                      \
    d2_t ut[B];                                                                                                            \
    double ex[B];                                                                                                          \
    _Pragma("unroll") for (int k = 0; k < B; k++) {                                                                        \
      ut[k] = utab[uid[k]];                                                                                                \
      ex[k] = eo[4 * (bb) + k];              \
    }                                                                                                                      \
    _Pragma("unroll") for (int k = 0; k < B; k++) {                                                                        \
      const bool need = ((n4 >> k) & 1u) != 0u;                                                                            \
      const bool head = ((h4 >> k) & 1u) != 0u;                                                                            \
      ccc = need ? cci[k] : ccc;                                                                                           \
      rcCb += need ? 16u : 0u;                                                         \
                              \
      RES_PARTIAL_STORE();                                                                                                 \
      f1 = head && !have_head ? s1 : f1;                                                                                   \
      f2 = head && !have_head ? s2 : f2;                                                                                   \
      have_head = have_head || head;                                                                                       \
      const double er = ex[k] + ccc * ut[k][1];                                                                            \
      eo[4 * (bb) + k] = er;                                                             \
      s1 = (head ? 0.0 : s1) + (-er) * ut[k][0];                                                                           \
      s2 = (head ? 0.0 : s2) + ut[k][0] * ut[k][0];                                                                        \
    }                                                                                                                      \
  }
#pragma unroll
        for (int j = 0; j < NG; j++) {
          RES_PRIO(j);
#pragma unroll 1
          for (int bp = 0; bp < 2; bp++) {
            RES_STEP_B(j, 2 * bp, itA, itB, ccA, ccB);
            RES_STEP_B(j, 2 * bp + 1, itB, itA, ccB, ccA);
          }
          if (a.prof && lane == 0 && (wv == 4 || wv == 7))
            a.prof[((int64_t)g * a.n_sw + (f - f_first)) * 64 + 16 + (wv == 4 ? 0 : 20) + j] = __builtin_amdgcn_s_memrealtime();
        }
        asm volatile(";; res sweep end");
        if (OVF) {
          unsigned hb_c = nbx0;
          for (int jx = 0; jx < ngx; jx++) {
            res_u4_t uwx;
#pragma unroll
            for (int w = 0; w < 4; w++) uwx[w] = uidw_x[(5 * jx + w) * NT];
            const unsigned uxx = uidw_x[(5 * jx + 4) * NT];
            const unsigned hb_n = jx + 1 < ngx ? headw_x[(jx + 1) * NT] : 0u;
            const unsigned nbw = hb_c | (hb_n << 16);
            res_d16_t eo;
#pragma unroll
            for (int i = 0; i < 16; i++) eo[i] = eog[(16 * jx + i) * NT];
#pragma unroll 1
            for (int bp = 0; bp < 2; bp++) {
              RES_STEP_BX(2 * bp, itA, itB, ccA, ccB);
              RES_STEP_BX(2 * bp + 1, itB, itA, ccB, ccA);
            }
#pragma unroll
            for (int i = 0; i < 16; i++) eog[(16 * jx + i) * NT] = eo[i];
            hb_c = hb_n;
          }
        }
#undef RES_STEP_B
#undef RES_STEP_BX
#undef RES_PARTIAL_STORE
      }
      if (a.prof && lane == 0)
        a.prof[((int64_t)g * a.n_sw + (f - f_first)) * 64 + 8 + wv] = __builtin_amdgcn_s_memrealtime();
      double v1 = s1, v2 = s2;
      int fl = have_head ? 1 : 0;
      wave_segscan2(v1, v2, fl);
      if (lane == 63) {
        wcarry[wv] = d2_t{v1, v2};
        wflag[wv] = fl;
      }
      double x1 = dpp_f64<0x138, 0xf>(v1), x2 = dpp_f64<0x138, 0xf>(v2);
      int xf = dpp_i32<0x138, 0xf>(fl, 0);
      if (lane == 0) {
        x1 = 0.0;
        x2 = 0.0;
        xf = 0;
      }
      lds_barrier();
      if (have_head && tid > 0) {
        if (!xf) {
          double c1 = 0.0, c2 = 0.0;
          for (int w = 0; w < wv; w++) {
            const d2_t cw = wcarry[w];
            const bool fw = wflag[w] != 0;
            c1 = (fw ? 0.0 : c1) + cw[0];
            c2 = (fw ? 0.0 : c2) + cw[1];
          }
          x1 = c1 + x1;
          x2 = c2 + x2;
        }
        const int closing = head0 ? run0 - 1 : run0;
        part2[closing] = d2_t{x1 + f1, x2 + f2};
      }
    }
    RES_STAMP(3);
    constexpr int CH = MFM_RES_CH;
    const int c0 = a.ent_ptr[g] >> 6, c1 = a.ent_ptr[g + 1] >> 6;
    const int per = (c1 - c0 + NW - 1) / NW;
    const int wb = c0 + wv * per, we = wb + per < c1 ? wb + per : c1;
    const int i0 = a.wg_item_ptr[g], ni = a.wg_item_ptr[g + 1] - i0;
    const bool more = f + 1 < a.f_end;
    int ij = 0;
    double iold = 0.0, iz = 0.0, ivn = 0.0, ilam = 0.0, imu = 0.0;
    if (tid < ni) {
      const int2 d = a.item_desc[i0 + tid];
      ij = d.x;
      iold = Vf[ij];
      iz = zf[ij];
      ivn = more ? a.V[(int64_t)(f + 1) * a.D + ij] : 0.0;
      ilam = lamf[d.y];
      imu = muf[d.y];
    }
    int2 en[CH];
#pragma unroll
    for (int k = 0; k < CH; k++) en[k] = make_int2(0, 0);
    if (wb < we) {
#pragma unroll
      for (int k = 0; k < CH; k++) en[k] = a.entries[(int64_t)(wb + k < we ? wb + k : wb) * WAVE + lane];
    }
    res_grid_barrier(a, rbar, ++nbar, tid, dead);
    RES_STAMP(4);
    {
      const d2_t *part2 = (const d2_t *)a.partials;
      for (int cb = wb; cb < we; cb += CH) {
        d2_t sv[CH];
#pragma unroll
        for (int k = 0; k < CH; k++) sv[k] = part2[en[k].x];
        int il[CH];
#pragma unroll
        for (int k = 0; k < CH; k++) il[k] = en[k].y;
        if (cb + CH < we) {
#pragma unroll
          for (int k = 0; k < CH; k++) en[k] = a.entries[(int64_t)(cb + CH + k < we ? cb + CH + k : cb + CH) * WAVE + lane];
        }
#pragma unroll
        for (int k = 0; k < CH; k++) {
          if (cb + k >= we) break;
          __hip_atomic_fetch_add(&acc1[wv * U + il[k]], sv[k][0], __ATOMIC_RELAXED, __HIP_MEMORY_SCOPE_WORKGROUP);
          __hip_atomic_fetch_add(&acc2[wv * U + il[k]], sv[k][1], __ATOMIC_RELAXED, __HIP_MEMORY_SCOPE_WORKGROUP);
        }
      }
      __syncthreads();
      double S1 = 0.0, S2 = 0.0;
      if (tid < ni) {
#pragma unroll
        for (int w = 0; w < NW; w++) {
          S1 += acc1[w * U + tid];
          S2 += acc2[w * U + tid];
          acc1[w * U + tid] = 0.0;
          acc2[w * U + tid] = 0.0;
        }
      }
      if (XCH) {
        const unsigned long long E = a.xepoch0 + (unsigned long long)(f - f_first) + 1ull;
        const int64_t stride = 2 * ((int64_t)a.n_items + 1), par = (int64_t)(E & 1ull);
        if (tid < ni) {
          const int64_t off = ((int64_t)a.xrank * 2 + par) * stride + 2 * (int64_t)(i0 + tid);
          for (int r = 0; r < a.xworld; r++) {
            __hip_atomic_store(a.xsum[r] + off, S1, __ATOMIC_RELAXED, __HIP_MEMORY_SCOPE_SYSTEM);
            __hip_atomic_store(a.xsum[r] + off + 1, S2, __ATOMIC_RELAXED, __HIP_MEMORY_SCOPE_SYSTEM);
          }
        }
        asm volatile("s_waitcnt vmcnt(0)" ::: "memory");
        __syncthreads();
        if (tid == 0 && !dead) {
          const unsigned long long old = __hip_atomic_fetch_add(a.xarrive, 1ull, __ATOMIC_RELAXED, __HIP_MEMORY_SCOPE_AGENT);
          if (old + 1 == (unsigned long long)a.n_wg * E) {
            for (int r = 0; r < a.xworld && !a.xch_break; r++)
              __hip_atomic_store(a.xflag[r] + 16 * a.xrank, E, __ATOMIC_RELEASE, __HIP_MEMORY_SCOPE_SYSTEM);
          }
          for (int r = 0; r < a.xworld && !dead; r++) res_spin_sys(a, a.xflag[a.xrank] + 16 * r, E, dead);
        }
        __syncthreads();
        if (tid < ni) {
          S1 = S2 = 0.0;
          for (int r = 0; r < a.xworld; r++) {
            const int64_t off = ((int64_t)r * 2 + par) * stride + 2 * (int64_t)(i0 + tid);
            S1 += __hip_atomic_load(a.xsum[a.xrank] + off, __ATOMIC_RELAXED, __HIP_MEMORY_SCOPE_SYSTEM);
            S2 += __hip_atomic_load(a.xsum[a.xrank] + off + 1, __ATOMIC_RELAXED, __HIP_MEMORY_SCOPE_SYSTEM);
          }
        }
      }
      if (tid < ni) {
        const double fresh = PMainV::draw(S1, S2, iold, alpha_k, ilam, imu, iz);
        Vf[ij] = fresh;
        res_store2(a.dv + 2 * (int64_t)(i0 + tid), fresh - iold, ivn);
      }
    }
    RES_STAMP(5);
    res_grid_barrier(a, rbar, ++nbar, tid, dead);
    RES_STAMP(6);
  }
#undef RES_STAMP
  RES_STAMP0(3);
  if (!a.no_store) {
    int run_last = run0;
#pragma unroll
    for (int j = 0; j < NG; j++) {
#pragma unroll 1
      for (int bb = 0; bb < 4; bb++) {
        const unsigned h4 = (hbv[j] >> (4 * bb)) & 15u;
        int row[B], it[B];
#pragma unroll
        for (int k = 0; k < B; k++) {
          if (16 * j + 4 * bb + k > 0) run_last += (int)((h4 >> k) & 1u);
          it[k] = a.run_item[run_last];
          row[k] = perm_g[(16 * j + 4 * bb + k) * NT + tid];
        }
        int uid[B];
        RES_UIDS(j, bb, uid);
#pragma unroll
        for (int k = 0; k < B; k++) {
          const double dl = a.dv[2 * (int64_t)it[k]];
          const double ex = j < NGV ? ev[j < NGV ? j : 0][4 * bb + k] : elds[(16 * (j - NGV) + 4 * bb + k) * NT + tid];
          const double ef = ex + utab[uid[k]][0] * dl;
          if (a.e_slots)
            a.e_slots[((int64_t)g * Rt + 16 * j + 4 * bb + k) * NT + tid] = ef;
          else if (row[k] >= 0)
            a.eq[row[k]].x = ef;
        }
      }
    }
    if (OVF) {
      for (int jx = 0; jx < ngx; jx++) {
        res_u4_t uwx;
#pragma unroll
        for (int w = 0; w < 4; w++) uwx[w] = uidw_x[(5 * jx + w) * NT];
        const unsigned uxx = uidw_x[(5 * jx + 4) * NT];
        const unsigned hbx = headw_x[jx * NT];
#pragma unroll 1
        for (int bb = 0; bb < 4; bb++) {
          const unsigned h4 = (hbx >> (4 * bb)) & 15u;
          int it[B], uid[B];
#pragma unroll
          for (int k = 0; k < B; k++) {
            run_last += (int)((h4 >> k) & 1u);
            it[k] = a.run_item[run_last];
          }
          RES_UIDSX(bb, uid);
#pragma unroll
          for (int k = 0; k < B; k++) {
            const double dl = a.dv[2 * (int64_t)it[k]];
            double *ep = eog + (16 * jx + 4 * bb + k) * NT;
            *ep = *ep + utab[uid[k]][0] * dl;
          }
        }
      }
    }
  }
#undef RES_PRIO
#undef RES_NIB
#undef RES_UIDS
#undef RES_UIDSX
#undef RES_OPAQUE
  asm volatile("s_waitcnt vmcnt(0)" ::: "memory");
  RES_STAMP0(4);
#undef RES_STAMP0
}

__global__ void k_res_init_dv(const double *__restrict__ theta, const int32_t *__restrict__ scols, int n_items,
                              double *__restrict__ dv, unsigned long long *__restrict__ bar) {
  const int i = blockIdx.x * blockDim.x + threadIdx.x;
  if (blockIdx.x == 0)
    for (int k = threadIdx.x; k < RES_BAR_WORDS; k += blockDim.x) bar[k] = 0ull;
  if (i < n_items) {
    dv[2 * i] = 0.0;
    dv[2 * i + 1] = theta ? theta[scols[i]] : 1.0;
  } else if (i == n_items) {
    dv[2 * i] = 0.0;
    dv[2 * i + 1] = 0.0;
  }
}

__global__ void k_res_unpermute(const double *__restrict__ e_slots, const int32_t *__restrict__ perm, int64_t n_slots,
                                double2 *__restrict__ eq) {
  const int64_t i = (int64_t)blockIdx.x * blockDim.x + threadIdx.x;
  if (i >= n_slots) return;
  const int32_t row = perm[i];
  if (row >= 0) eq[row].x = e_slots[i];
}

struct ResScoreArgs {
  const uint32_t *uidw, *headw;
  const int32_t *first_run, *run_feat, *wg_user_ptr, *wg_fill;
  const int2 *user_desc;
  int umax, KS;
  const double *Vt, *w;
  double w0;
  const double *w0p;
  const double *y_slots;
  double *e_slots;
  double2 *sums;
  unsigned long long *prof;
};

template <int NT, int NG, int KPT>
__global__ __launch_bounds__(NT) void k_res_score(ResScoreArgs a) {
  extern __shared__ __attribute__((aligned(16))) char res_smem[];
  constexpr int R = 16 * NG, NW = NT / WAVE;
  constexpr int US = 2 * KPT + 2;
  const int g = blockIdx.x, tid = threadIdx.x, lane = tid & 63, wv = tid >> 6;
  const int KP = a.KS >> 1;
  const double w0_k = a.w0p ? *a.w0p : a.w0;
  double *uV = (double *)res_smem;
  double *uW = uV + (size_t)a.umax * US;
  double2 *wsum = (double2 *)(uW + ((a.umax + 1) & ~1));
  if (a.prof && tid == 0) a.prof[4 * g] = __builtin_amdgcn_s_memrealtime();
  int *ucol = (int *)(wsum + NW);
  const int u0 = a.wg_user_ptr[g], nu = a.wg_user_ptr[g + 1] - u0;
  for (int ul = tid; ul < a.umax; ul += NT) {
    const int ju = ul < nu ? a.user_desc[u0 + ul].x : -1;
    ucol[ul] = ju;
    uW[ul] = ju >= 0 ? a.w[ju] : 0.0;
  }
  __syncthreads();
#pragma unroll 4
  for (int i = tid; i < a.umax * KPT; i += NT) {
    const int ul = i / KPT, pr = i - ul * KPT;
    const int ju = ucol[ul];
    double2 v = make_double2(0.0, 0.0);
    if (ju >= 0 && pr < KP) v = ((const double2 *)(a.Vt + (int64_t)ju * a.KS))[pr];
    ((double2 *)(uV + (size_t)ul * US))[pr] = v;
  }
  res_u4_t uw[NG];
  unsigned ux[NG], hbv[NG];
#pragma unroll
  for (int j = 0; j < NG; j++) {
#pragma unroll
    for (int w = 0; w < 4; w++) uw[j][w] = a.uidw[((int64_t)g * (5 * NG) + 5 * j + w) * NT + tid];
    ux[j] = a.uidw[((int64_t)g * (5 * NG) + 5 * j + 4) * NT + tid];
    hbv[j] = a.headw[((int64_t)g * NG + j) * NT + tid];
  }
  int run = a.first_run[g * NT + tid];
  const int64_t fill = a.wg_fill[g];
  __syncthreads();
  if (a.prof && tid == 0) a.prof[4 * g + 1] = __builtin_amdgcn_s_memrealtime();
  double2 vi[KPT];
  double wi = 0.0, s1 = 0.0, s2 = 0.0;
#pragma unroll
  for (int p = 0; p < KPT; p++) vi[p] = make_double2(0.0, 0.0);
  int jc[4], jn[4];
  double yn[4];
#pragma unroll
  for (int k = 0; k < 4; k++) yn[k] = a.y_slots[((int64_t)g * R + k) * NT + tid];
  {
    const unsigned h0 = hbv[0] & 15u;
    int r = run;
#pragma unroll
    for (int k = 0; k < 4; k++) {
      if (k > 0) r += (int)((h0 >> k) & 1u);
      jc[k] = a.run_feat[r];
    }
    run = r;
  }
#pragma unroll
  for (int j = 0; j < NG; j++) {
    const unsigned hb2 = hbv[j] | (j + 1 < NG ? hbv[j + 1 < NG ? j + 1 : j] << 16 : 0u);
#pragma unroll 1
    for (int bb = 0; bb < 4; bb++) {
      {
        const unsigned hn = (hb2 >> (4 * (bb + 1))) & 15u;
        int r = run;
#pragma unroll
        for (int k = 0; k < 4; k++) {
          r += (int)((hn >> k) & 1u);
          jn[k] = a.run_feat[r];
        }
        run = r;
      }
      const unsigned lo_ = uw[j][bb];
      int uid[4];
      uid[0] = (int)(lo_ & 0x3ffu);
      uid[1] = (int)((lo_ >> 10) & 0x3ffu);
      uid[2] = (int)((lo_ >> 20) & 0x3ffu);
      uid[3] = (int)((lo_ >> 30) | (((ux[j] >> (8 * bb)) & 0xffu) << 2));
      const unsigned h4 = (hbv[j] >> (4 * bb)) & 15u;
      double yv[4], eb[4];
#pragma unroll
      for (int k = 0; k < 4; k++) yv[k] = yn[k];
      {
        const int nb = 16 * j + 4 * bb + 4 < R ? 16 * j + 4 * bb + 4 : 0;
#pragma unroll
        for (int k = 0; k < 4; k++) yn[k] = a.y_slots[((int64_t)g * R + nb + k) * NT + tid];
      }
#pragma unroll
      for (int k = 0; k < 4; k++) {
        const int slot = 16 * j + 4 * bb + k;
        const bool head = slot == 0 || ((h4 >> k) & 1u);
        if (head) {
          const int ji = jc[k];
          wi = 0.0;
          if (ji >= 0) {
            const double2 *src = (const double2 *)(a.Vt + (int64_t)ji * a.KS);
#pragma unroll
            for (int p = 0; p < KPT; p++) vi[p] = p < KP ? src[p] : make_double2(0.0, 0.0);
            wi = a.w[ji];
          } else {
#pragma unroll
            for (int p = 0; p < KPT; p++) vi[p] = make_double2(0.0, 0.0);
          }
        }
        const double2 *vu = (const double2 *)(uV + (size_t)uid[k] * US);
        double d0 = 0.0, d1 = 0.0;
#pragma unroll
        for (int p = 0; p < KPT; p += 2) {
          const double2 x0 = vu[p], x1 = vu[p + 1];
          d0 += x0.x * vi[p].x + x0.y * vi[p].y;
          d1 += x1.x * vi[p + 1].x + x1.y * vi[p + 1].y;
        }
        const double pred = w0_k + (uW[uid[k]] + wi) + (d0 + d1);
        const bool real = (int64_t)tid * R + slot < fill;
        const double e = real ? pred - yv[k] : 0.0;
        eb[k] = e;
        s1 += e;
        s2 += e * e;
      }
#pragma unroll
      for (int k = 0; k < 4; k++) a.e_slots[((int64_t)g * R + 16 * j + 4 * bb + k) * NT + tid] = eb[k];
#pragma unroll
      for (int k = 0; k < 4; k++) jc[k] = jn[k];
    }
  }
  if (a.prof && lane == 0) a.prof[4 * g + 2] = __builtin_amdgcn_s_memrealtime();
  wave_allreduce_sum2(s1, s2);
  if (lane == 0) wsum[wv] = make_double2(s1, s2);
  __syncthreads();
  if (a.prof && tid == 0) a.prof[4 * g + 3] = __builtin_amdgcn_s_memrealtime();
  if (tid == 0) {
    double t1 = 0.0, t2 = 0.0;
    for (int w = 0; w < NW; w++) {
      t1 += wsum[w].x;
      t2 += wsum[w].y;
    }
    a.sums[g] = make_double2(t1, t2);
  }
}

__global__ void k_res_permute_y(const double *__restrict__ y, const int32_t *__restrict__ perm, int64_t n_slots,
                                double *__restrict__ y_slots) {
  const int64_t i = (int64_t)blockIdx.x * blockDim.x + threadIdx.x;
  if (i >= n_slots) return;
  const int32_t row = perm[i];
  y_slots[i] = row >= 0 ? y[row] : 0.0;
}

template <class F>
static inline void res_parallel_for(int n, F f) {
  const int hw = (int)std::thread::hardware_concurrency();
  const int T = std::max(1, std::min({n, 16, hw > 0 ? hw : 1}));
  if (T == 1) {
    for (int i = 0; i < n; i++) f(i);
    return;
  }
  std::atomic<int> next(0);
  auto work = [&]() {
    for (;;) {
      const int i = next.fetch_add(1);
      if (i >= n) return;
      f(i);
    }
  };
  std::vector<std::thread> pool;
  for (int t = 1; t < T; t++) pool.emplace_back(work);
  work();
  for (auto &t : pool) t.join();
}

struct ResPlan {
  bool ready = false;
  int G = 0, NT = 512, RV = 0, RL = 0, umax = 0, item_bits = 0, n_items = 0;
  int RX = 0;
  int R() const { return RV + RL + RX; }
  bool allow_overflow = true;
  int64_t n_rows = 0, n_runs = 0;
  size_t lds_bytes = 0;
  DevBuf<int32_t> perm, first_run, wg_run_ptr, wg_nruns, wg_user_ptr, wg_item_ptr, ent_ptr, scols;
  DevBuf<int2> entries;
  DevBuf<uint32_t> uidw, headw;
  DevBuf<int32_t> run_item;
  DevBuf<int2> user_desc, item_desc;
  DevBuf<double> partials, dv, e_slots;
  DevBuf<unsigned long long> bar;
  DevBuf<int32_t> run_feat, wg_fill;
  DevBuf<double> y_slots;
  DevBuf<double2> sums;
  int max_wg_users = 0, max_slice_items = 0;
  int xworld = 1, xrank = 0;
  bool peers_set = false;
  DevBuf<double> xsum;
  DevBuf<unsigned long long> xflag, xarrive;
  double *peer_sum[RES_MAX_PEERS] = {nullptr, nullptr, nullptr, nullptr, nullptr, nullptr, nullptr, nullptr};
  unsigned long long *peer_flag[RES_MAX_PEERS] = {nullptr, nullptr, nullptr, nullptr, nullptr, nullptr, nullptr, nullptr};
  unsigned long long xepoch = 0;
  bool peers_model = false;
  double *peer_w[RES_MAX_PEERS] = {nullptr, nullptr, nullptr, nullptr, nullptr, nullptr, nullptr, nullptr};
  double *peer_V[RES_MAX_PEERS] = {nullptr, nullptr, nullptr, nullptr, nullptr, nullptr, nullptr, nullptr};
  std::vector<void *> peer_mapped;
  size_t xsum_bytes(int world) const { return (size_t)world * 2 * 2 * ((size_t)n_items + 1) * sizeof(double); }
  void alloc_exchange(int world, int rank, hipStream_t s) {
    xworld = world;
    xrank = rank;
    peers_set = false;
    peers_model = false;
    xepoch = 0;
    auto alloc_shared = [&](auto &buf, size_t count) {
      buf.release();
      void *p = nullptr;
      const size_t bytes = count * sizeof(*buf.p);
      if (hipExtMallocWithFlags(&p, bytes, hipDeviceMallocUncached) != hipSuccess) {
        (void)hipGetLastError();
        throw Error(MFM_ERR_DEVICE, "no uncached device memory for the ranks' exchange buffers (hipExtMallocWithFlags(hipDeviceMallocUncached))");
      }
      buf.p = (decltype(buf.p))p;
      buf.n = count;
      buf.owned = true;
      MFM_HIP_CHECK(hipMemsetAsync(p, 0, bytes, s));
    };
    alloc_shared(xsum, xsum_bytes(world) / sizeof(double));
    alloc_shared(xflag, (size_t)16 * RES_MAX_PEERS);
    xarrive.alloc_zero(16, s);
  }
  std::string why;
  std::vector<int32_t> h_nruns;
  std::vector<std::string> h_diag;

  static int bits_for(int64_t n) {
    int b = 1;
    while (((int64_t)1 << b) < n) b++;
    return b;
  }
  struct Variant {
    int rv, rl;
  };
  static const Variant *variants(int &n) {
    static const Variant v[] = {{16, 0}, {32, 0}, {64, 16}};
    n = 3;
    return v;
  }

  bool choose_layout(int64_t N, const std::vector<int64_t> &ustart, int64_t max_user, int n_cu, std::vector<int64_t> &ucut) {
    const int64_t n_users = (int64_t)ustart.size() - 1;
    int nv = 0;
    const Variant *vs = variants(nv);
    bool found = false;
    for (int vi = 0; vi < nv && !found; vi++) {
      const int64_t cap = (int64_t)NT * (vs[vi].rv + vs[vi].rl) - 1;
      if (max_user > cap) continue;
      const int64_t slack = std::min<int64_t>(cap / 8, max_user);
      int64_t Gw = (N + (cap - slack) - 1) / (cap - slack);
      if (Gw > n_cu && N <= (int64_t)n_cu * cap) Gw = n_cu;
      if (Gw > n_cu) continue;
      if (env_flag("MFM_RES_WGS")) Gw = std::min<int64_t>(n_cu, std::max<int64_t>(Gw, env_i64("MFM_RES_WGS", 0)));
      Gw = std::min<int64_t>(Gw, n_users);
      ucut.assign(1, 0);
      bool ok = true;
      for (int64_t g = 1; g <= Gw && ok; g++) {
        const int64_t lo_u = ucut.back();
        int64_t hi_u;
        if (g == Gw) {
          hi_u = n_users;
        } else {
          const int64_t want = (N * g) / Gw;
          hi_u = std::upper_bound(ustart.begin(), ustart.end(), want) - ustart.begin() - 1;
          if (hi_u + 1 <= n_users && ustart[hi_u + 1] - want < want - ustart[hi_u]) hi_u++;
          hi_u = std::max(hi_u, lo_u + 1);
          hi_u = std::min<int64_t>(hi_u, n_users - (Gw - g));
          hi_u = std::max<int64_t>(hi_u, n_users - (Gw - g) * NT);
          while (hi_u > lo_u + 1 && ustart[hi_u] - ustart[lo_u] > cap) hi_u--;
        }
        if (hi_u <= lo_u || ustart[hi_u] - ustart[lo_u] > cap) ok = false;
        ucut.push_back(hi_u);
      }
      if (!ok) continue;
      G = (int)Gw;
      RV = vs[vi].rv;
      RL = vs[vi].rl;
      found = true;
    }
    RX = 0;
    if (!found && allow_overflow) {
      const Variant big = vs[nv - 1];
      for (int rx = 16; rx <= 80 && !found; rx += 16) {
        const int64_t cap = (int64_t)NT * (big.rv + big.rl + rx) - 1;
        if (max_user > cap || N > (int64_t)n_cu * cap) continue;
        int64_t Gw = std::min<int64_t>(n_cu, n_users);
        ucut.assign(1, 0);
        bool ok = true;
        for (int64_t g = 1; g <= Gw && ok; g++) {
          const int64_t lo_u = ucut.back();
          int64_t hi_u;
          if (g == Gw) {
            hi_u = n_users;
          } else {
            const int64_t want = (N * g) / Gw;
            hi_u = std::upper_bound(ustart.begin(), ustart.end(), want) - ustart.begin() - 1;
            if (hi_u + 1 <= n_users && ustart[hi_u + 1] - want < want - ustart[hi_u]) hi_u++;
            hi_u = std::max(hi_u, lo_u + 1);
            hi_u = std::min<int64_t>(hi_u, n_users - (Gw - g));
            hi_u = std::max<int64_t>(hi_u, n_users - (Gw - g) * NT);
            while (hi_u > lo_u + 1 && ustart[hi_u] - ustart[lo_u] > cap) hi_u--;
          }
          if (hi_u <= lo_u || ustart[hi_u] - ustart[lo_u] > cap) ok = false;
          ucut.push_back(hi_u);
        }
        if (!ok) continue;
        G = (int)Gw;
        RV = big.rv;
        RL = big.rl;
        RX = rx;
        found = true;
      }
    }
    if (!found) return fail("no variant fits (rows per CU, or a first-level column longer than a workgroup's capacity)");
    return true;
  }
  bool choose_item_slices(const std::vector<int32_t> &slot_ptr, int64_t counter, std::vector<int32_t> &iptr) {
    iptr.assign((size_t)G + 1, 0);
    bool ok = false;
    for (double scale = 1.0; scale < 3.0 && !ok; scale *= 1.1) {
      const double target = scale * ((double)counter + 16.0 * n_items) / G;
      double acc = 0.0;
      int gq = 0, cnt = 0;
      for (int c = 0; c < n_items; c++) {
        acc += (double)(slot_ptr[c + 1] - slot_ptr[c]) + 16.0;
        cnt++;
        if ((acc >= target || cnt == NT) && gq + 1 < G) {
          iptr[++gq] = c + 1;
          acc = 0.0;
          cnt = 0;
        }
      }
      ok = cnt <= NT;
      for (gq++; gq <= G; gq++) iptr[gq] = n_items;
    }
    if (!ok) return fail("more second-level columns than the workgroups can draw");
    return true;
  }
  static std::vector<int32_t> run_bases(const std::vector<int32_t> &nruns) {
    const int G = (int)nruns.size();
    std::vector<int32_t> run_base((size_t)G + 1, 0);
    for (int g = 0; g < G; g++) run_base[g + 1] = run_base[g] + nruns[g] + 1;
    return run_base;
  }

  bool build(const HostCsr &csc, const std::vector<int32_t> &level, const std::vector<int32_t> *group_of, int n_cu,
             const std::vector<char> *draw_empty = nullptr) {
    ready = false;
    const int64_t N = csc.cols, D0 = csc.rows;
    n_rows = N;
    if (N < 1 || n_cu < 1 || (int64_t)level.size() != D0) return fail("shape");
    std::vector<int32_t> users, items, empties;
    for (int64_t j = 0; j < D0; j++) {
      if (level[j] == 0) {
        if (csc.ptr[j + 1] > csc.ptr[j])
          users.push_back((int32_t)j);
        else if (!draw_empty || (*draw_empty)[(size_t)j])
          empties.push_back((int32_t)j);
      } else if (level[j] == 1) {
        items.push_back((int32_t)j);
      } else {
        return fail("more than two levels");
      }
    }
    n_items = (int)items.size();
    if (users.empty() || items.empty()) return fail("empty level");
    std::sort(users.begin(), users.end(), [&](int32_t x, int32_t y) { return csc.idx[csc.ptr[x]] < csc.idx[csc.ptr[y]]; });
    std::vector<int64_t> ustart(users.size() + 1);
    int64_t next_row = 0, max_user = 0;
    for (size_t u = 0; u < users.size(); u++) {
      const int32_t j = users[u];
      const int64_t b = csc.ptr[j], len = csc.ptr[j + 1] - b;
      if (csc.idx[b] != next_row || csc.idx[b + len - 1] != next_row + len - 1) return fail("first level not contiguous");
      ustart[u] = next_row;
      next_row += len;
      max_user = std::max(max_user, len);
    }
    ustart[users.size()] = next_row;
    if (next_row != N) return fail("first level does not cover the rows");
    std::vector<int32_t> item_of_row((size_t)N, -1);
    {
      int64_t cnt = 0;
      for (int c = 0; c < n_items; c++) cnt += csc.ptr[items[c] + 1] - csc.ptr[items[c]];
      if (cnt != N) return fail("second level does not cover the rows");
      const int chunks = std::max(1, std::min(n_items, 64));
      res_parallel_for(chunks, [&](int k) {
        for (int c = (int)((int64_t)n_items * k / chunks); c < (int)((int64_t)n_items * (k + 1) / chunks); c++)
          for (int64_t p = csc.ptr[items[c]]; p < csc.ptr[items[c] + 1]; p++) item_of_row[csc.idx[p]] = c;
      });
      std::atomic<bool> bad(false);
      res_parallel_for(chunks, [&](int k) {
        for (int64_t r = N * k / chunks; r < N * (k + 1) / chunks; r++)
          if (item_of_row[r] < 0) bad = true;
      });
      if (bad) return fail("second level touches a row twice");
    }
    std::vector<int64_t> ucut;
    if (!choose_layout(N, ustart, max_user, n_cu, ucut)) return false;
    const int R = RV + RL + RX;
    const int64_t cap_slots = (int64_t)NT * R;
    std::vector<std::vector<int32_t>> wg_users((size_t)G);
    for (int g = 0; g < G; g++)
      for (int64_t u = ucut[g]; u < ucut[g + 1]; u++) wg_users[g].push_back(users[u]);
    for (size_t k = 0; k < empties.size(); k++) wg_users[k % G].push_back(empties[k]);
    int maxu = 0;
    for (int g = 0; g < G; g++) maxu = std::max(maxu, (int)wg_users[g].size());
    max_wg_users = maxu;
    if (maxu > NT) return fail("more first-level columns in a workgroup than threads");
    item_bits = bits_for((int64_t)n_items + 1);
    const int UW = 5 * (R / 16), HW = R / 16;
    std::vector<uint16_t> h_uid((size_t)G * cap_slots, 0xffffu);
    std::vector<uint32_t> h_headw((size_t)G * HW * NT, 0);
    std::vector<int32_t> h_perm((size_t)G * cap_slots, -1), h_first((size_t)G * NT, 0);
    std::vector<std::vector<int32_t>> wg_run_item((size_t)G);
    std::vector<int64_t> fill((size_t)G, 0);
    std::vector<int32_t> nruns((size_t)G, 0);
    res_parallel_for(G, [&](int g) {
      const int64_t row0 = ustart[ucut[g]], row1 = ustart[ucut[g + 1]];
      const int64_t n = row1 - row0;
      std::vector<int32_t> cnt((size_t)n_items + 1, 0), uloc((size_t)n);
      for (int64_t u = ucut[g]; u < ucut[g + 1]; u++)
        for (int64_t r = ustart[u]; r < ustart[u + 1]; r++) uloc[(size_t)(r - row0)] = (int32_t)(u - ucut[g]);
      for (int64_t r = row0; r < row1; r++) cnt[(size_t)item_of_row[r] + 1]++;
      std::vector<int32_t> &runs = wg_run_item[g];
      for (int c = 0; c < n_items; c++) {
        if (cnt[c + 1]) {
          const int64_t sidx = cnt[c];
          const int th = (int)(sidx / R), rh = (int)(sidx % R);
          h_headw[((size_t)g * HW + rh / 16) * NT + th] |= 1u << (rh % 16);
          runs.push_back(c);
        }
        cnt[c + 1] += cnt[c];
      }
      {
        size_t ri = 0;
        std::vector<int32_t> run_start(runs.size());
        for (size_t k = 0; k < runs.size(); k++) run_start[k] = cnt[runs[k]];
        for (int t = 0; t < NT; t++) {
          const int64_t s0 = (int64_t)t * R;
          if (s0 >= n) break;
          while (ri + 1 < runs.size() && run_start[ri + 1] <= s0) ri++;
          h_first[(size_t)g * NT + t] = (int32_t)ri;
        }
      }
      for (int64_t r = row0; r < row1; r++) {
        const int64_t sidx = cnt[(size_t)item_of_row[r]]++;
        const int t = (int)(sidx / R), rr = (int)(sidx % R);
        h_perm[(size_t)g * cap_slots + (size_t)rr * NT + t] = (int32_t)r;
        h_uid[(size_t)g * cap_slots + (size_t)sidx] = (uint16_t)uloc[(size_t)(r - row0)];
      }
      fill[g] = n;
      nruns[g] = (int32_t)runs.size();
    });
    std::vector<int32_t> h_slot_ptr((size_t)n_items + 1, 0);
    int64_t counter = 0;
    for (int g = 0; g < G; g++) {
      counter += nruns[g];
      for (int32_t c : wg_run_item[g]) h_slot_ptr[(size_t)c + 1]++;
    }
    for (int c = 0; c < n_items; c++) h_slot_ptr[(size_t)c + 1] += h_slot_ptr[c];
    h_slot_ptr[n_items] = (int32_t)counter;
    n_runs = counter;
    if (counter >= ((int64_t)1 << 31) - 2) return fail("too many runs");
    std::vector<int32_t> run_base = run_bases(nruns);
    const int32_t zero_run = run_base[G];
    std::vector<int32_t> h_run_item((size_t)zero_run + 1, n_items);
    for (int g = 0; g < G; g++) {
      std::copy(wg_run_item[g].begin(), wg_run_item[g].end(), h_run_item.begin() + run_base[g]);
      if (fill[g] < cap_slots) {
        const int th = (int)(fill[g] / R), rh = (int)(fill[g] % R);
        h_headw[((size_t)g * HW + rh / 16) * NT + th] |= 1u << (rh % 16);
      }
      h_headw[((size_t)g * HW) * NT] |= 1u;
      for (int t = 0; t < NT; t++) {
        const int64_t s0 = (int64_t)t * R;
        int32_t &fr = h_first[(size_t)g * NT + t];
        fr = (s0 >= fill[g] ? nruns[g] : fr) + run_base[g];
      }
    }
    std::vector<int32_t> h_uptr((size_t)G + 1, 0);
    std::vector<int2> h_udesc;
    for (int g = 0; g < G; g++) {
      for (int32_t j : wg_users[g]) h_udesc.push_back(make_int2(j, group_of && (size_t)j < group_of->size() ? (*group_of)[j] : 0));
      h_uptr[g + 1] = (int32_t)h_udesc.size();
    }
    std::vector<int32_t> h_iptr;
    if (!choose_item_slices(h_slot_ptr, counter, h_iptr)) return false;
    int imax = 0;
    for (int g = 0; g < G; g++) imax = std::max(imax, h_iptr[g + 1] - h_iptr[g]);
    max_slice_items = imax;
    umax = std::max(maxu, imax) + 1;
    if (umax > 1024) return fail("internal: user field");
    std::vector<uint32_t> h_uidw((size_t)G * UW * NT, 0);
    res_parallel_for(G, [&](int g) {
      for (int64_t sl = 0; sl < cap_slots; sl++) {
        const uint16_t u16 = h_uid[(size_t)g * cap_slots + (size_t)sl];
        const uint32_t u = u16 == 0xffffu ? (uint32_t)(umax - 1) : u16;
        const int t = (int)(sl / R), r = (int)(sl % R);
        const int w0 = 5 * (r / 16), bb = (r % 16) / 4, k = r % 4;
        if (k < 3) {
          h_uidw[((size_t)g * UW + w0 + bb) * NT + t] |= u << (10 * k);
        } else {
          h_uidw[((size_t)g * UW + w0 + bb) * NT + t] |= (u & 3u) << 30;
          h_uidw[((size_t)g * UW + w0 + 4) * NT + t] |= (u >> 2) << (8 * bb);
        }
      }
    });
    h_uid = std::vector<uint16_t>();
    std::vector<int32_t> slice_of((size_t)n_items);
    for (int g = 0; g < G; g++)
      for (int c = h_iptr[g]; c < h_iptr[g + 1]; c++) slice_of[c] = g;
    std::vector<int32_t> h_eptr((size_t)G + 1, 0);
    {
      std::vector<int64_t> cnt((size_t)G, 0);
      for (int g = 0; g < G; g++)
        for (int32_t c : wg_run_item[g]) cnt[slice_of[c]]++;
      for (int g = 0; g < G; g++) {
        const int64_t e = h_eptr[g] + ((cnt[g] + WAVE - 1) / WAVE) * WAVE;
        if (e >= ((int64_t)1 << 31)) return fail("too many entries");
        h_eptr[g + 1] = (int32_t)e;
      }
    }
    std::vector<int2> h_entries((size_t)h_eptr[G], make_int2(zero_run, 0));
    {
      std::vector<int64_t> pos((size_t)G);
      for (int g = 0; g < G; g++) pos[g] = h_eptr[g];
      for (int g = 0; g < G; g++)
        for (size_t l = 0; l < wg_run_item[g].size(); l++) {
          const int32_t c = wg_run_item[g][l];
          const int sgl = slice_of[c];
          h_entries[(size_t)pos[sgl]++] = make_int2(run_base[g] + (int32_t)l, c - h_iptr[sgl]);
        }
    }
    if (h_entries.size() >= ((size_t)1 << 31)) return fail("too many entries");
    lds_bytes = (size_t)RL * NT * 8 + (size_t)2 * (NT / WAVE) * umax * 8 + (size_t)umax * 16 + (size_t)(NT / WAVE) * 16 + (NT / WAVE) * 4 + 64;
    if (lds_bytes > 160 * 1024 - 512) return fail("LDS");
    uidw.upload(h_uidw);
    headw.upload(h_headw);
    run_item.upload(h_run_item);
    perm.upload(h_perm);
    first_run.upload(h_first);
    wg_user_ptr.upload(h_uptr);
    user_desc.upload(h_udesc.data(), h_udesc.size());
    wg_item_ptr.upload(h_iptr);
    ent_ptr.upload(h_eptr);
    entries.upload(h_entries.data(), h_entries.size());
    wg_run_ptr.upload(run_base);
    wg_nruns.upload(nruns);
    e_slots.alloc((size_t)G * cap_slots);
    {
      std::vector<int32_t> h_run_feat(h_run_item.size() + 8, -1);
      for (size_t r = 0; r < h_run_item.size(); r++) h_run_feat[r] = h_run_item[r] < n_items ? items[(size_t)h_run_item[r]] : -1;
      run_feat.upload(h_run_feat);
      std::vector<int32_t> h_fill((size_t)G);
      for (int g = 0; g < G; g++) h_fill[g] = (int32_t)fill[g];
      wg_fill.upload(h_fill);
      sums.alloc((size_t)G);
      y_slots = DevBuf<double>();
    }
    h_nruns = nruns;
    if (env_flag("MFM_RES_PROF")) {
      h_diag.assign((size_t)G, "");
      for (int g = 0; g < G; g++) {
        int64_t maxlen = 0;
        for (int64_t u = ucut[g]; u < ucut[g + 1]; u++) maxlen = std::max(maxlen, ustart[u + 1] - ustart[u]);
        int64_t sinstr = 0, maxst = 0, nthr_head = 0;
        for (int w = 0; w < NT / WAVE; w++) {
          std::vector<char> hh(WAVE, 0);
          std::vector<int> st(WAVE, 0);
          for (int r = 0; r < R; r++) {
            bool any = false;
            for (int l = 0; l < WAVE; l++) {
              const int t = w * WAVE + l;
              const bool head = (h_headw[((size_t)g * HW + r / 16) * NT + t] >> (r % 16)) & 1u;
              if (head && hh[l]) {
                any = true;
                st[l]++;
              }
              hh[l] = hh[l] || head;
            }
            sinstr += any;
          }
          for (int l = 0; l < WAVE; l++) {
            maxst = std::max<int64_t>(maxst, st[l]);
            nthr_head += hh[l];
          }
        }
        char buf[160];
        std::snprintf(buf, sizeof buf, "users %d maxlen %lld rows %lld store-instr %lld max-stores/thread %lld threads-with-head %lld",
                      (int)(ucut[g + 1] - ucut[g]), (long long)maxlen, (long long)fill[g], (long long)sinstr, (long long)maxst,
                      (long long)nthr_head);
        h_diag[g] = buf;
      }
    }
    scols.upload(items);
    {
      std::vector<int2> h_idesc(items.size());
      for (size_t i = 0; i < items.size(); i++) {
        const int32_t j = items[i];
        h_idesc[i] = make_int2(j, group_of && (size_t)j < group_of->size() ? (*group_of)[j] : 0);
      }
      item_desc.upload(h_idesc.data(), h_idesc.size());
    }
    partials.alloc((size_t)2 * ((size_t)zero_run + 1));
    MFM_HIP_CHECK(hipMemset(partials.p, 0, (size_t)16 * ((size_t)zero_run + 1)));
    dv.alloc((size_t)2 * (n_items + 1));
    bar.alloc(RES_BAR_WORDS);
    ready = true;
    why.clear();
    return true;
  }
  bool fail(const char *w) {
    why = w;
    ready = false;
    return false;
  }
};

static inline hipError_t res_occupancy(const ResPlan &rp, int *per_cu) {
  *per_cu = 0;
  const void *fn = nullptr;
  if (rp.RV == 16 && rp.RL == 0)
    fn = (const void *)k_mf_resident<512, 1, 0>;
  else if (rp.RV == 32 && rp.RL == 0)
    fn = (const void *)k_mf_resident<512, 2, 0>;
  else if (rp.RV == 64 && rp.RL == 16)
    fn = rp.RX ? (const void *)k_mf_resident<512, 4, 1, false, true> : (const void *)k_mf_resident<512, 4, 1>;
  else
    return hipErrorInvalidValue;
  hipError_t e = hipFuncSetAttribute(fn, hipFuncAttributeMaxDynamicSharedMemorySize, 160 * 1024);
  if (e != hipSuccess) return e;
  return hipOccupancyMaxActiveBlocksPerMultiprocessor(per_cu, fn, 512, rp.lds_bytes);
}

static inline void run_sweep_resident(hipStream_t s, Timing &tm, ResPlan &rp, int kernel_class, double2 *eq, double *V, int64_t D,
                                      int f_begin, int f_end, const double *zbase, const double *lam, const double *mu,
                                      const int32_t *group, int n_groups, double alpha, int *error,
                                      double *w = nullptr, const double *zw = nullptr, const double *lam_w = nullptr,
                                      const double *mu_w = nullptr, double e_shift = 0.0, bool load_slots = false,
                                      bool no_store = false, const double *scal = nullptr) {
  ResArgs a;
  std::memset(&a, 0, sizeof(a));
  a.scal = scal;
  a.eq = eq;
  a.e_slots = rp.e_slots.p;
  a.ngx = rp.RX / 16;
  a.no_store = no_store ? 1 : 0;
  a.e_in = load_slots ? rp.e_slots.p : nullptr;
  a.linear = w ? 1 : 0;
  a.n_sw = f_end - f_begin + a.linear;
  a.w = w;
  a.zw = zw;
  a.lam_w = lam_w;
  a.mu_w = mu_w;
  a.e_shift = e_shift;
  a.perm = rp.perm.p;
  a.uidw = rp.uidw.p;
  a.headw = rp.headw.p;
  a.run_item = rp.run_item.p;
  a.first_run = rp.first_run.p;
  a.wg_user_ptr = rp.wg_user_ptr.p;
  a.user_desc = rp.user_desc.p;
  a.wg_item_ptr = rp.wg_item_ptr.p;
  a.ent_ptr = rp.ent_ptr.p;
  a.entries = rp.entries.p;
  a.wg_run_ptr = rp.wg_run_ptr.p;
  a.wg_nruns = rp.wg_nruns.p;
  a.scols = rp.scols.p;
  a.item_desc = rp.item_desc.p;
  a.partials = rp.partials.p;
  a.dv = rp.dv.p;
  a.V = V;
  a.D = D;
  a.f_begin = f_begin;
  a.f_end = f_end;
  a.z = zbase;
  a.lam = lam;
  a.mu = mu;
  a.group = group;
  a.n_groups = n_groups;
  a.alpha = alpha;
  a.n_items = rp.n_items;
  a.umax = rp.umax;
  a.bar = rp.bar.p;
  a.n_wg = rp.G;
  a.error = error;
  const bool xch = rp.xworld > 1;
  a.xch_break = xch && rp.xrank == 1 && env_flag("MFM_RES_XCH_BREAK");
  a.xworld = rp.xworld;
  a.xrank = rp.xrank;
  a.xepoch0 = rp.xepoch;
  a.xarrive = rp.xarrive.p;
  a.xmodel = xch && rp.peers_model ? 1 : 0;
  for (int r = 0; r < RES_MAX_PEERS; r++) {
    a.xsum[r] = rp.peer_sum[r];
    a.xflag[r] = rp.peer_flag[r];
    a.xw[r] = rp.peer_w[r];
    a.xV[r] = rp.peer_V[r];
  }
  if (xch && !rp.peers_set) throw Error(MFM_ERR_RUNTIME, "row-sharded persistent sweep: the peers' exchange buffers are not set (mfm_peer_set)");
  static int prof_launch = 0;
  const bool prof = env_flag("MFM_RES_PROF") && ++prof_launch == env_int("MFM_RES_PROF", 0);
  DevBuf<unsigned long long> prof_buf;
  if (prof) {
    prof_buf.alloc((size_t)rp.G * a.n_sw * 64);
    MFM_HIP_CHECK(hipMemsetAsync(prof_buf.p, 0, (size_t)rp.G * a.n_sw * 512, s));
    a.prof = prof_buf.p;
  }
  const int K = a.n_sw;
  double bytes = (8.0 + (load_slots ? 0.0 : 4.0) + 1.4 + (no_store ? 0.0 : 8.0)) * rp.n_rows + K * 48.0 * rp.n_runs;
  if (rp.RX) bytes += (double)K * (16.0 + 1.75) * (double)rp.G * rp.NT * rp.RX;
  hipLaunchKernelGGL(k_res_init_dv, dim3((rp.n_items + 256) / 256), dim3(256), 0, s,
                     w ? (const double *)nullptr : V + (int64_t)f_begin * D, rp.scols.p, rp.n_items,
                     rp.dv.p, rp.bar.p);
  TimedLaunch t(tm, s, kernel_class, bytes);
#define MFM_RES_LAUNCH(RV_, RL_)                                                                                              \
  do {                                                                                                                        \
    static DeviceOnce raised;                                                                                                 \
    if (raised.need()) {                                                                                                      \
      MFM_HIP_CHECK(hipFuncSetAttribute((const void *)k_mf_resident<512, RV_ / 16, RL_ / 16>,                                  \
                                        hipFuncAttributeMaxDynamicSharedMemorySize, 160 * 1024));                             \
      raised.mark();                                                                                                          \
    }                                                                                                                         \
    if (xch) {                                                                                                                \
      static DeviceOnce raised_x;                                                                                             \
      if (raised_x.need()) {                                                                                                  \
        MFM_HIP_CHECK(hipFuncSetAttribute((const void *)k_mf_resident<512, RV_ / 16, RL_ / 16, true>,                          \
                                          hipFuncAttributeMaxDynamicSharedMemorySize, 160 * 1024));                           \
        raised_x.mark();                                                                                                      \
      }                                                                                                                       \
      hipLaunchKernelGGL((k_mf_resident<512, RV_ / 16, RL_ / 16, true>), dim3(rp.G), dim3(512), rp.lds_bytes, s, a);            \
    } else {                                                                                                                  \
      hipLaunchKernelGGL((k_mf_resident<512, RV_ / 16, RL_ / 16>), dim3(rp.G), dim3(512), rp.lds_bytes, s, a);                  \
    }                                                                                                                         \
  } while (0)
  if (rp.RV == 16 && rp.RL == 0)
    MFM_RES_LAUNCH(16, 0);
  else if (rp.RV == 32 && rp.RL == 0)
    MFM_RES_LAUNCH(32, 0);
  else if (rp.RV == 64 && rp.RL == 16 && rp.RX > 0) {
    if (xch) throw Error(MFM_ERR_RUNTIME, "internal: no row-sharded resident kernel with overflow slots");
    static DeviceOnce raised_o;
    if (raised_o.need()) {
      MFM_HIP_CHECK(hipFuncSetAttribute((const void *)k_mf_resident<512, 4, 1, false, true>, hipFuncAttributeMaxDynamicSharedMemorySize, 160 * 1024));
      raised_o.mark();
    }
    hipLaunchKernelGGL((k_mf_resident<512, 4, 1, false, true>), dim3(rp.G), dim3(512), rp.lds_bytes, s, a);
  } else if (rp.RV == 64 && rp.RL == 16)
    MFM_RES_LAUNCH(64, 16);
  else
    throw Error(MFM_ERR_RUNTIME, "internal: no resident kernel variant for this plan");
#undef MFM_RES_LAUNCH
  MFM_HIP_CHECK(hipGetLastError());
  if (xch) rp.xepoch += (unsigned long long)a.n_sw;
  if (prof) {
    MFM_HIP_CHECK(hipStreamSynchronize(s));
    const int K2 = a.n_sw;
    std::vector<unsigned long long> h((size_t)rp.G * K2 * 64);
    MFM_HIP_CHECK(hipMemcpy(h.data(), prof_buf.p, h.size() * 8, hipMemcpyDeviceToHost));
    const char *names[6] = {"sweep A", "user draw", "sweep B", "barrier 1 (wait)", "item draw", "barrier 2 (wait)"};
    std::fprintf(stderr, "[resident profile] G=%d factors=%d; us per factor: mean | mean of max over workgroups | mean of min\n", rp.G, K2);
    for (int ph = 0; ph < 6; ph++) {
      double sm = 0, smax = 0, smin = 0;
      for (int f = 0; f < K2; f++) {
        double mx = 0, mn = 1e30;
        for (int g = 0; g < rp.G; g++) {
          const unsigned long long *t = &h[((size_t)g * K2 + f) * 64];
          const double d = (double)(t[ph + 1] - t[ph]) * 0.01;
          sm += d;
          mx = std::max(mx, d);
          mn = std::min(mn, d);
        }
        smax += mx;
        smin += mn;
      }
      std::fprintf(stderr, "  %-18s %8.2f | %8.2f | %8.2f\n", names[ph], sm / ((double)rp.G * K2), smax / K2, smin / K2);
    }
    {
      std::vector<std::pair<double, int>> tb;
      for (int g = 0; g < rp.G; g++) {
        double d = 0;
        for (int f = 0; f < K2; f++) d += (double)(h[((size_t)g * K2 + f) * 64 + 3] - h[((size_t)g * K2 + f) * 64 + 2]) * 0.01;
        tb.push_back({d / K2, g});
      }
      std::sort(tb.begin(), tb.end());
      std::fprintf(stderr, "  sweep B by workgroup: fastest");
      for (int k = 0; k < 4; k++) std::fprintf(stderr, " wg %d %.1f (%d runs)", tb[k].second, tb[k].first, rp.h_nruns[tb[k].second]);
      std::fprintf(stderr, "; median wg %d %.1f (%d runs); slowest", tb[rp.G / 2].second, tb[rp.G / 2].first, rp.h_nruns[tb[rp.G / 2].second]);
      for (int k = rp.G - 4; k < rp.G; k++) std::fprintf(stderr, " wg %d %.1f (%d runs)", tb[k].second, tb[k].first, rp.h_nruns[tb[k].second]);
      std::fprintf(stderr, "\n");
      if (!rp.h_diag.empty())
        for (int k : {0, 1, rp.G / 2, rp.G - 3, rp.G - 2, rp.G - 1})
        {
          const int g = tb[k].second;
          std::fprintf(stderr, "    wg %d %.1f us: %s; waves:", g, tb[k].first, rp.h_diag[g].c_str());
          for (int w = 0; w < 8; w++) {
            double d = 0;
            for (int f = 0; f < K2; f++) d += (double)(h[((size_t)g * K2 + f) * 64 + 8 + w] - h[((size_t)g * K2 + f) * 64 + 2]) * 0.01;
            std::fprintf(stderr, " %.1f", d / K2);
          }
          std::fprintf(stderr, "\n      groups of 16 slots of waves 4 and 7 (factor 3 alone):");
          for (int w : {0, 20}) {
            std::fprintf(stderr, " |");
            for (int b = 0; b < (rp.RV + rp.RL) / 16; b++)
              std::fprintf(stderr, " %.1f", (double)(h[((size_t)g * K2 + 3) * 64 + 16 + w + b] - h[((size_t)g * K2 + 3) * 64 + 2]) * 0.01);
          }
          std::fprintf(stderr, "\n");
        }
    }
    if (const char *dump = env_str("MFM_RES_PROF_DUMP")) {
      if (FILE *fp = std::fopen(dump, "w")) {
        for (int g = 0; g < rp.G; g++) {
          std::fprintf(fp, "%d", g);
          for (int ph = 0; ph < 6; ph++) {
            double d = 0;
            for (int f = 0; f < K2; f++) d += (double)(h[((size_t)g * K2 + f) * 64 + ph + 1] - h[((size_t)g * K2 + f) * 64 + ph]) * 0.01;
            std::fprintf(fp, " %.2f", d / K2);
          }
          std::fprintf(fp, " | %s\n", rp.h_diag.empty() ? "" : rp.h_diag[g].c_str());
        }
        std::fclose(fp);
      }
    }
    {
      const char *nm[4] = {"census barrier", "residual load", "factor loop", "residual store"};
      for (int ph = 0; ph < 4; ph++) {
        double sm = 0, mx = 0;
        for (int g = 0; g < rp.G; g++) {
          const double d = (double)(h[(size_t)g * K2 * 64 + 56 + ph + 1] - h[(size_t)g * K2 * 64 + 56 + ph]) * 0.01;
          sm += d;
          mx = std::max(mx, d);
        }
        std::fprintf(stderr, "  %-18s %8.2f mean | %8.2f max (us, whole launch)\n", nm[ph], sm / rp.G, mx);
      }
      unsigned long long t0 = ~0ull, t1 = 0;
      for (int g = 0; g < rp.G; g++) {
        t0 = std::min(t0, h[(size_t)g * K2 * 64 + 56]);
        t1 = std::max(t1, h[(size_t)g * K2 * 64 + 60]);
      }
      std::fprintf(stderr, "  first workgroup in to last workgroup out: %.1f us\n", (double)(t1 - t0) * 0.01);
    }
    double tot = 0;
    for (int g = 0; g < rp.G; g++) tot += (double)(h[((size_t)g * K2 + K2 - 1) * 64 + 6] - h[(size_t)g * K2 * 64]) * 0.01;
    std::fprintf(stderr, "  factors, start to end: %.1f us (%.2f per factor)\n", tot / rp.G, tot / rp.G / K2);
  }
}

static inline bool res_score_supported(const ResPlan &rp, int K) {
  const int KS = (K + 1) & ~1;
  if (!rp.ready || K < 1 || KS > 32) return false;
  const size_t lds = ((size_t)rp.umax * (2 * 16 + 2) + ((rp.umax + 1) & ~1)) * 8 + 8 * 16 + (size_t)rp.umax * 4 + 64;
  return lds <= 160 * 1024 - 512;
}

static inline void run_res_score(hipStream_t s, Timing &tm, ResPlan &rp, int kernel_class, const double *Vt, const double *w,
                                 double w0, int K, const double *y, int64_t nnz, const double *w0p = nullptr) {
  const int KS = (K + 1) & ~1;
  const int64_t n_slots = (int64_t)rp.G * rp.R() * 512;
  if (!rp.y_slots.p) {
    rp.y_slots.alloc((size_t)n_slots);
    hipLaunchKernelGGL(k_res_permute_y, dim3((unsigned)((n_slots + 255) / 256)), dim3(256), 0, s, y, rp.perm.p, n_slots,
                       rp.y_slots.p);
  }
  ResScoreArgs a;
  a.uidw = rp.uidw.p;
  a.headw = rp.headw.p;
  a.first_run = rp.first_run.p;
  a.run_feat = rp.run_feat.p;
  a.wg_user_ptr = rp.wg_user_ptr.p;
  a.wg_fill = rp.wg_fill.p;
  a.user_desc = rp.user_desc.p;
  a.umax = rp.umax;
  a.KS = KS;
  a.Vt = Vt;
  a.w = w;
  a.w0 = w0;
  a.w0p = w0p;
  a.y_slots = rp.y_slots.p;
  a.e_slots = rp.e_slots.p;
  a.sums = rp.sums.p;
  static int prof_calls = 0;
  const bool prof = env_flag("MFM_RES_SCORE_PROF") && ++prof_calls == env_int("MFM_RES_SCORE_PROF", 0);
  DevBuf<unsigned long long> prof_buf;
  a.prof = nullptr;
  if (prof) {
    prof_buf.alloc((size_t)rp.G * 4);
    a.prof = prof_buf.p;
  }
  const size_t lds = ((size_t)rp.umax * (2 * 16 + 2) + ((rp.umax + 1) & ~1)) * 8 + 8 * 16 + (size_t)rp.umax * 4 + 64;
  TimedLaunch t(tm, s, kernel_class, 17.4 * rp.n_rows + 8.0 * KS * (double)rp.n_runs);
  (void)nnz;
#define MFM_RES_SCORE(NG_)                                                                                              \
  do {                                                                                                                  \
    static DeviceOnce raised;                                                                                           \
    if (raised.need()) {                                                                                                \
      MFM_HIP_CHECK(hipFuncSetAttribute((const void *)k_res_score<512, NG_, 16>, hipFuncAttributeMaxDynamicSharedMemorySize, \
                                        160 * 1024));                                                                   \
      raised.mark();                                                                                                    \
    }                                                                                                                   \
    hipLaunchKernelGGL((k_res_score<512, NG_, 16>), dim3(rp.G), dim3(512), lds, s, a);                                   \
  } while (0)
  const int NG = rp.R() / 16;
  if (NG == 1)
    MFM_RES_SCORE(1);
  else if (NG == 2)
    MFM_RES_SCORE(2);
  else if (NG == 5)
    MFM_RES_SCORE(5);
  else if (NG == 6)
    MFM_RES_SCORE(6);
  else if (NG == 7)
    MFM_RES_SCORE(7);
  else if (NG == 8)
    MFM_RES_SCORE(8);
  else if (NG == 9)
    MFM_RES_SCORE(9);
  else if (NG == 10)
    MFM_RES_SCORE(10);
  else
    throw Error(MFM_ERR_RUNTIME, "internal: no slot-order scorer for this plan");
#undef MFM_RES_SCORE
  MFM_HIP_CHECK(hipGetLastError());
  if (prof) {
    MFM_HIP_CHECK(hipStreamSynchronize(s));
    std::vector<unsigned long long> h((size_t)rp.G * 4);
    MFM_HIP_CHECK(hipMemcpy(h.data(), prof_buf.p, h.size() * 8, hipMemcpyDeviceToHost));
    unsigned long long t0 = ~0ull, t1 = 0;
    double st = 0, lp = 0, en = 0;
    for (int g = 0; g < rp.G; g++) {
      t0 = std::min(t0, h[4 * g]);
      t1 = std::max(t1, h[4 * g + 3]);
      st += (double)(h[4 * g + 1] - h[4 * g]) * 0.01;
      lp += (double)(h[4 * g + 2] - h[4 * g + 1]) * 0.01;
      en += (double)(h[4 * g + 3] - h[4 * g + 2]) * 0.01;
    }
    std::fprintf(stderr, "[k_res_score] first start to last end %.1f us; per workgroup (mean): users staged %.1f, slots %.1f, reduction %.1f us\n",
                 (double)(t1 - t0) * 0.01, st / rp.G, lp / rp.G, en / rp.G);
  }
}

}
```

### myfm_amd/csrc/mfm_res_plan.hpp

```cpp
#pragma once
#include <chrono>

#include <hipcub/hipcub.hpp>

#include "mfm_res.hpp"

namespace mfm {

namespace rp {

constexpr int TB = 256;

__global__ void k_rows(const int32_t *__restrict__ colidx, int64_t N, int32_t *__restrict__ bflag, int32_t *__restrict__ ucnt,
                       int32_t *__restrict__ icnt, int32_t *__restrict__ red) {
  const int64_t r = (int64_t)blockIdx.x * blockDim.x + threadIdx.x;
  int32_t mu = -1, mi = 0x7fffffff;
  if (r < N) {
    const int2 c = ((const int2 *)colidx)[r];
    const bool b = r == 0 || c.x != colidx[2 * (r - 1)];
    bflag[r] = b ? 1 : 0;
    if (b) atomicAdd(&ucnt[c.x], 1);
    atomicAdd(&icnt[c.y], 1);
    mu = c.x;
    mi = c.y;
// ... 150 lines not shown
    const bool head = sidx < fill ? headf[rowcut[g] + sidx] != 0 : sidx == fill;
    if (head || sidx == 0) hw |= 1u << q;
  }
  for (int k = 0; k < 5; k++) uidw[((int64_t)g * UW + 5 * grp + k) * NT + t] = w[k];
  headw[((int64_t)g * HW + grp) * NT + t] = hw;
}

__global__ void k_user_desc(const int32_t *__restrict__ users, const int32_t *__restrict__ empties, const int32_t *__restrict__ ucut,
                            const int32_t *__restrict__ uptr, const int32_t *__restrict__ group, int G, int32_t n_users, int32_t n_emp,
                            int2 *__restrict__ desc) {
  __shared__ int32_t cut[1026];
  for (int i = threadIdx.x; i <= G; i += blockDim.x) cut[i] = ucut[i];
  __syncthreads();
  const int32_t i = blockIdx.x * blockDim.x + threadIdx.x;
  if (i < n_users) {
    const int g = upper_group(cut, G, i);
    const int32_t j = users[i];
    desc[uptr[g] + (i - cut[g])] = make_int2(j, group ? group[j] : 0);
  } else if (i < n_users + n_emp) {
    const int32_t k = i - n_users;
    const int g = k % G;
    const int32_t j = empties[k];
    desc[uptr[g] + (cut[g + 1] - cut[g]) + k / G] = make_int2(j, group ? group[j] : 0);
  }
}

__global__ void k_item_desc(const int32_t *__restrict__ scols, const int32_t *__restrict__ group, int32_t n_items, int2 *__restrict__ desc) {
  const int32_t i = blockIdx.x * blockDim.x + threadIdx.x;
  if (i < n_items) desc[i] = make_int2(scols[i], group ? group[scols[i]] : 0);
}

__global__ void k_run_feat(const int32_t *__restrict__ run_item, const int32_t *__restrict__ scols, int32_t n_items, int64_t n_run_item,
                           int64_t n, int32_t *__restrict__ run_feat) {
  const int64_t r = (int64_t)blockIdx.x * blockDim.x + threadIdx.x;
  if (r >= n) return;
  int32_t f = -1;
  if (r < n_run_item) {
    const int32_t c = run_item[r];
    if (c < n_items) f = scols[c];
  }
  run_feat[r] = f;
}

__global__ void k_slice_keys(const int32_t *__restrict__ run_item_c, const int32_t *__restrict__ iptr, int G, int64_t n, uint32_t *__restrict__ key,
                             int32_t *__restrict__ val) {
  __shared__ int32_t cut[1026];
  for (int i = threadIdx.x; i <= G; i += blockDim.x) cut[i] = iptr[i];
  __syncthreads();
  const int64_t k = (int64_t)blockIdx.x * blockDim.x + threadIdx.x;
  if (k >= n) return;
  key[k] = (uint32_t)upper_group(cut, G, run_item_c[k]);
  val[k] = (int32_t)k;
}

__global__ void k_entries(const uint32_t *__restrict__ key, const int32_t *__restrict__ val, const int32_t *__restrict__ run_item_c,
                          const int32_t *__restrict__ hrun0, const int32_t *__restrict__ run_base, const int32_t *__restrict__ iptr,
                          const int32_t *__restrict__ eptr, const int32_t *__restrict__ sstart, int G, int64_t n, int2 *__restrict__ entries) {
  __shared__ int32_t cut[1026];
  for (int i = threadIdx.x; i <= G; i += blockDim.x) cut[i] = hrun0[i];
  __syncthreads();
  const int64_t q = (int64_t)blockIdx.x * blockDim.x + threadIdx.x;
  if (q >= n) return;
  const int sl = (int)key[q];
  const int32_t kc = val[q];
  const int g = upper_group(cut, G, kc);
  entries[eptr[sl] + (q - sstart[sl])] = make_int2(run_base[g] + (kc - cut[g]), run_item_c[kc] - iptr[sl]);
}

template <class T>
static inline std::vector<T> download(const T *p, size_t n, hipStream_t s) {
  std::vector<T> h(n);
  if (n) MFM_HIP_CHECK(hipMemcpyAsync(h.data(), p, n * sizeof(T), hipMemcpyDeviceToHost, s));
  MFM_HIP_CHECK(hipStreamSynchronize(s));
  return h;
}

static inline void inclusive_sum(const int32_t *in, int32_t *out, int64_t n, DevBuf<char> &tmp, hipStream_t s) {
  size_t bytes = 0;
  MFM_HIP_CHECK(hipcub::DeviceScan::InclusiveSum(nullptr, bytes, in, out, (int)n, s));
  if (tmp.n < bytes) tmp.alloc(bytes);
  MFM_HIP_CHECK(hipcub::DeviceScan::InclusiveSum(tmp.p, bytes, in, out, (int)n, s));
}
static inline void exclusive_sum(const int32_t *in, int32_t *out, int64_t n, DevBuf<char> &tmp, hipStream_t s) {
  size_t bytes = 0;
  MFM_HIP_CHECK(hipcub::DeviceScan::ExclusiveSum(nullptr, bytes, in, out, (int)n, s));
  if (tmp.n < bytes) tmp.alloc(bytes);
  MFM_HIP_CHECK(hipcub::DeviceScan::ExclusiveSum(tmp.p, bytes, in, out, (int)n, s));
}
static inline void sort_pairs(DevBuf<uint32_t> &k_in, DevBuf<uint32_t> &k_out, DevBuf<int32_t> &v_in, DevBuf<int32_t> &v_out, int64_t n, int bits,
                              DevBuf<char> &tmp, hipStream_t s) {
  size_t bytes = 0;
  MFM_HIP_CHECK(hipcub::DeviceRadixSort::SortPairs(nullptr, bytes, k_in.p, k_out.p, v_in.p, v_out.p, (int)n, 0, bits, s));
  if (tmp.n < bytes) tmp.alloc(bytes);
  MFM_HIP_CHECK(hipcub::DeviceRadixSort::SortPairs(tmp.p, bytes, k_in.p, k_out.p, v_in.p, v_out.p, (int)n, 0, bits, s));
}

}

static inline bool res_plan_build_device(ResPlan &rpn, const DevSparse &X, const std::vector<int32_t> *group_of, int n_cu, hipStream_t s,
                                         const std::vector<int32_t> *glevel = nullptr, const std::vector<char> *draw_empty = nullptr) {
  using namespace rp;
  rpn.ready = false;
  const int64_t N = X.rows, D0 = X.cols;
  const int NT = rpn.NT;
  rpn.n_rows = N;
  if (N < 1 || n_cu < 1 || D0 < 2 || !X.unit || X.ell_width != 2) return rpn.fail("shape");
  if (N >= ((int64_t)1 << 31) - 1) return rpn.fail("too many rows");
  auto grid = [](int64_t n) { return dim3((unsigned)((n + TB - 1) / TB)); };
  const bool tlog = env_flag("MFM_SETUP_TIMING");
  double t_prev = std::chrono::duration<double>(std::chrono::steady_clock::now().time_since_epoch()).count();
  auto lap = [&](const char *what) {
    if (!tlog) return;
    MFM_HIP_CHECK(hipStreamSynchronize(s));
    const double t = std::chrono::duration<double>(std::chrono::steady_clock::now().time_since_epoch()).count();
    std::fprintf(stderr, "[res_plan_build_device] %-34s %7.2f ms\n", what, (t - t_prev) * 1e3);
    t_prev = t;
  };
  DevBuf<char> tmp;
  DevBuf<int32_t> bflag, ucnt, icnt, red, iflag, eflag, iord, eord, uord1;
  bflag.alloc((size_t)N);
  uord1.alloc((size_t)N);
  ucnt.alloc_zero((size_t)D0, s);
  icnt.alloc_zero((size_t)D0, s);
  iflag.alloc((size_t)D0 + 1);
  eflag.alloc((size_t)D0 + 1);
  iord.alloc((size_t)D0 + 1);
  eord.alloc((size_t)D0 + 1);
  {
    const int32_t r0[4] = {-1, 0x7fffffff, 0, 0};
    red.upload(r0, 4);
  }
  lap("allocations");
  if (tlog) {
    hipLaunchKernelGGL(k_fill32, dim3(1), dim3(TB), 0, s, red.p + 3, (int64_t)1, 0);
    lap("first kernel of the library (code object load)");
  }
  hipLaunchKernelGGL(k_rows, grid(N), dim3(TB), 0, s, X.colidx.p, N, bflag.p, ucnt.p, icnt.p, red.p);
  lap("k_rows");
  const bool given = glevel && draw_empty && (int64_t)glevel->size() == D0 && (int64_t)draw_empty->size() == D0;
  if ((glevel || draw_empty) && !given) return rpn.fail("shape");
  if (given) {
    DevBuf<int32_t> d_level, d_de;
    d_level.upload(*glevel);
    std::vector<int32_t> de32(draw_empty->begin(), draw_empty->end());
    d_de.upload(de32);
    hipLaunchKernelGGL(k_cols_given, grid(D0), dim3(TB), 0, s, ucnt.p, icnt.p, d_level.p, d_de.p, D0, iflag.p, eflag.p, red.p);
    MFM_HIP_CHECK(hipStreamSynchronize(s));
  } else {
    hipLaunchKernelGGL(k_cols, grid(D0), dim3(TB), 0, s, ucnt.p, icnt.p, D0, iflag.p, eflag.p, red.p);
  }
  MFM_HIP_CHECK(hipMemsetAsync(iflag.p + D0, 0, sizeof(int32_t), s));
  MFM_HIP_CHECK(hipMemsetAsync(eflag.p + D0, 0, sizeof(int32_t), s));
  exclusive_sum(iflag.p, iord.p, D0 + 1, tmp, s);
  exclusive_sum(eflag.p, eord.p, D0 + 1, tmp, s);
  inclusive_sum(bflag.p, uord1.p, N, tmp, s);
  lap("rows, columns, scans (enqueued + run)");
  int32_t h_red[4], n_items = 0, n_emp = 0, n_users = 0;
  MFM_HIP_CHECK(hipMemcpyAsync(h_red, red.p, sizeof h_red, hipMemcpyDeviceToHost, s));
  MFM_HIP_CHECK(hipMemcpyAsync(&n_items, iord.p + D0, sizeof(int32_t), hipMemcpyDeviceToHost, s));
  MFM_HIP_CHECK(hipMemcpyAsync(&n_emp, eord.p + D0, sizeof(int32_t), hipMemcpyDeviceToHost, s));
  MFM_HIP_CHECK(hipMemcpyAsync(&n_users, uord1.p + (N - 1), sizeof(int32_t), hipMemcpyDeviceToHost, s));
  MFM_HIP_CHECK(hipStreamSynchronize(s));
  if (!given && h_red[0] >= h_red[1]) return rpn.fail("the two fields' column ranges overlap");
  if (h_red[2] != 0) return rpn.fail("first level not contiguous");
  if (n_users < 1 || n_items < 1) return rpn.fail("empty level");
  rpn.n_items = n_items;
  DevBuf<int32_t> empties, d_ustart, d_users;
  rpn.scols.alloc((size_t)n_items);
  empties.alloc((size_t)std::max(n_emp, 1));
  d_ustart.alloc((size_t)n_users + 1);
  d_users.alloc((size_t)n_users);
  hipLaunchKernelGGL(k_col_lists, grid(D0), dim3(TB), 0, s, iflag.p, eflag.p, iord.p, eord.p, D0, rpn.scols.p, empties.p);
  hipLaunchKernelGGL(k_users, grid(N), dim3(TB), 0, s, X.colidx.p, bflag.p, uord1.p, N, d_ustart.p, d_users.p);
  std::vector<int64_t> ustart((size_t)n_users + 1), ucut;
  int64_t max_user = 0;
  {
    const std::vector<int32_t> u32 = download(d_ustart.p, (size_t)n_users + 1, s);
    for (size_t u = 0; u < u32.size(); u++) ustart[u] = u32[u];
    for (int32_t u = 0; u < n_users; u++) max_user = std::max(max_user, ustart[u + 1] - ustart[u]);
  }
  if (!rpn.choose_layout(N, ustart, max_user, n_cu, ucut)) return false;
  const int G = rpn.G, R = rpn.R();
  const int64_t cap_slots = (int64_t)NT * R;
  if (G > 1024) return rpn.fail("more than 1024 workgroups");
  std::vector<int32_t> h_rowcut((size_t)G + 1), h_ucut((size_t)G + 1), h_uptr((size_t)G + 1, 0);
  int maxu = 0;
  for (int g = 0; g <= G; g++) {
    h_rowcut[g] = (int32_t)ustart[ucut[g]];
    h_ucut[g] = (int32_t)ucut[g];
  }
  for (int g = 0; g < G; g++) {
    const int nu = (int)(ucut[g + 1] - ucut[g]) + n_emp / G + (g < n_emp % G ? 1 : 0);
    maxu = std::max(maxu, nu);
    h_uptr[g + 1] = h_uptr[g] + nu;
  }
  rpn.max_wg_users = maxu;
  if (maxu > NT) return rpn.fail("more first-level columns in a workgroup than threads");
  rpn.item_bits = ResPlan::bits_for((int64_t)n_items + 1);
  const int gbits = ResPlan::bits_for(G);
  if (rpn.item_bits + gbits > 32) return rpn.fail("sort key width");
  DevBuf<int32_t> rowcut, d_ucut, hrun0, hs, headf;
  rowcut.upload(h_rowcut);
  d_ucut.upload(h_ucut);
  rpn.wg_user_ptr.upload(h_uptr);
  DevBuf<uint32_t> key, key2;
  DevBuf<int32_t> val, val2;
  key.alloc((size_t)N);
  key2.alloc((size_t)N);
  val.alloc((size_t)N);
  val2.alloc((size_t)N);
  hipLaunchKernelGGL(k_keys, grid(N), dim3(TB), 0, s, X.colidx.p, iord.p, rowcut.p, G, rpn.item_bits, N, key.p, val.p);
  sort_pairs(key, key2, val, val2, N, rpn.item_bits + gbits, tmp, s);
  lap("users, cuts, keys, sort");
  DevBuf<uint16_t> uid;
  uid.alloc((size_t)G * cap_slots);
  MFM_HIP_CHECK(hipMemsetAsync(uid.p, 0xff, (size_t)G * cap_slots * sizeof(uint16_t), s));
  rpn.perm.alloc((size_t)G * cap_slots);
  MFM_HIP_CHECK(hipMemsetAsync(rpn.perm.p, 0xff, (size_t)G * cap_slots * sizeof(int32_t), s));
  headf.alloc((size_t)N);
  hs.alloc((size_t)N);
  hipLaunchKernelGGL(k_slots, grid(N), dim3(TB), 0, s, key2.p, val2.p, uord1.p, rowcut.p, d_ucut.p, rpn.item_bits, R, NT, N, rpn.perm.p, uid.p,
                     headf.p);
  inclusive_sum(headf.p, hs.p, N, tmp, s);
  hrun0.alloc((size_t)G + 1);
  hipLaunchKernelGGL(k_wg_runs, dim3((G + 1 + TB - 1) / TB), dim3(TB), 0, s, hs.p, rowcut.p, G, hrun0.p);
  const std::vector<int32_t> h_hrun0 = download(hrun0.p, (size_t)G + 1, s);
  std::vector<int32_t> nruns((size_t)G);
  for (int g = 0; g < G; g++) nruns[g] = h_hrun0[g + 1] - h_hrun0[g];
  const int64_t counter = h_hrun0[G];
  rpn.n_runs = counter;
  if (counter >= ((int64_t)1 << 31) - 2) return rpn.fail("too many runs");
  const std::vector<int32_t> run_base = ResPlan::run_bases(nruns);
  const int32_t zero_run = run_base[G];
  rpn.wg_run_ptr.upload(run_base);
  rpn.wg_nruns.upload(nruns);
  rpn.run_item.alloc((size_t)zero_run + 1);
  hipLaunchKernelGGL(k_fill32, grid(zero_run + 1), dim3(TB), 0, s, rpn.run_item.p, (int64_t)zero_run + 1, n_items);
  DevBuf<int32_t> run_item_c, runs_per_item;
  run_item_c.alloc((size_t)std::max<int64_t>(counter, 1));
  runs_per_item.alloc_zero((size_t)n_items, s);
  hipLaunchKernelGGL(k_runs, grid(N), dim3(TB), 0, s, key2.p, headf.p, hs.p, hrun0.p, rpn.wg_run_ptr.p, rpn.item_bits, N, run_item_c.p,
                     rpn.run_item.p, runs_per_item.p);
  rpn.first_run.alloc((size_t)G * NT);
  hipLaunchKernelGGL(k_first, grid((int64_t)G * NT), dim3(TB), 0, s, hs.p, rowcut.p, hrun0.p, rpn.wg_run_ptr.p, G, R, NT, rpn.first_run.p);
  lap("slots, heads, runs, first");
  std::vector<int32_t> h_slot_ptr((size_t)n_items + 1, 0), h_iptr;
  {
    const std::vector<int32_t> rpi = download(runs_per_item.p, (size_t)n_items, s);
    for (int c = 0; c < n_items; c++) h_slot_ptr[(size_t)c + 1] = h_slot_ptr[c] + rpi[c];
  }
  if (!rpn.choose_item_slices(h_slot_ptr, counter, h_iptr)) return false;
  int imax = 0;
  for (int g = 0; g < G; g++) imax = std::max(imax, h_iptr[g + 1] - h_iptr[g]);
  rpn.max_slice_items = imax;
  rpn.umax = std::max(maxu, imax) + 1;
  if (rpn.umax > 1024) return rpn.fail("internal: user field");
  const int UW = 5 * (R / 16), HW = R / 16;
  rpn.uidw.alloc((size_t)G * UW * NT);
  rpn.headw.alloc((size_t)G * HW * NT);
  hipLaunchKernelGGL(k_pack, grid((int64_t)G * HW * NT), dim3(TB), 0, s, uid.p, headf.p, rowcut.p, G, R, NT, rpn.umax, rpn.uidw.p, rpn.headw.p);
  std::vector<int32_t> h_eptr((size_t)G + 1, 0), h_sstart((size_t)G + 1, 0);
  for (int g = 0; g < G; g++) {
    const int64_t cnt = h_slot_ptr[h_iptr[g + 1]] - h_slot_ptr[h_iptr[g]];
    const int64_t e = h_eptr[g] + ((cnt + WAVE - 1) / WAVE) * WAVE;
    if (e >= ((int64_t)1 << 31)) return rpn.fail("too many entries");
    h_eptr[g + 1] = (int32_t)e;
    h_sstart[g + 1] = h_sstart[g] + (int32_t)cnt;
  }
  rpn.wg_item_ptr.upload(h_iptr);
  rpn.ent_ptr.upload(h_eptr);
  rpn.entries.alloc((size_t)h_eptr[G]);
  if (h_eptr[G]) hipLaunchKernelGGL(k_fill_int2, grid(h_eptr[G]), dim3(TB), 0, s, rpn.entries.p, (int64_t)h_eptr[G], make_int2(zero_run, 0));
  if (counter > 0) {
    DevBuf<int32_t> sstart;
    sstart.upload(h_sstart);
    DevBuf<uint32_t> sk, sk2;
    DevBuf<int32_t> sv, sv2;
    sk.alloc((size_t)counter);
    sk2.alloc((size_t)counter);
    sv.alloc((size_t)counter);
    sv2.alloc((size_t)counter);
    hipLaunchKernelGGL(k_slice_keys, grid(counter), dim3(TB), 0, s, run_item_c.p, rpn.wg_item_ptr.p, G, counter, sk.p, sv.p);
    sort_pairs(sk, sk2, sv, sv2, counter, gbits, tmp, s);
    hipLaunchKernelGGL(k_entries, grid(counter), dim3(TB), 0, s, sk2.p, sv2.p, run_item_c.p, hrun0.p, rpn.wg_run_ptr.p, rpn.wg_item_ptr.p,
                       rpn.ent_ptr.p, sstart.p, G, counter, rpn.entries.p);
    MFM_HIP_CHECK(hipStreamSynchronize(s));
  }
  lap("slices, pack, entries");
  DevBuf<int32_t> d_group;
  if (group_of && (int64_t)group_of->size() >= D0) d_group.upload(group_of->data(), (size_t)D0);
  rpn.user_desc.alloc((size_t)h_uptr[G]);
  hipLaunchKernelGGL(k_user_desc, grid((int64_t)n_users + n_emp), dim3(TB), 0, s, d_users.p, empties.p, d_ucut.p, rpn.wg_user_ptr.p, d_group.p, G,
                     n_users, n_emp, rpn.user_desc.p);
  rpn.item_desc.alloc((size_t)n_items);
  hipLaunchKernelGGL(k_item_desc, grid(n_items), dim3(TB), 0, s, rpn.scols.p, d_group.p, n_items, rpn.item_desc.p);
  rpn.run_feat.alloc((size_t)zero_run + 1 + 8);
  hipLaunchKernelGGL(k_run_feat, grid((int64_t)zero_run + 9), dim3(TB), 0, s, rpn.run_item.p, rpn.scols.p, n_items, (int64_t)zero_run + 1,
                     (int64_t)zero_run + 9, rpn.run_feat.p);
  {
    std::vector<int32_t> h_fill((size_t)G);
    for (int g = 0; g < G; g++) h_fill[g] = h_rowcut[g + 1] - h_rowcut[g];
    rpn.wg_fill.upload(h_fill);
  }
  rpn.lds_bytes = (size_t)rpn.RL * NT * 8 + (size_t)2 * (NT / WAVE) * rpn.umax * 8 + (size_t)rpn.umax * 16 + (size_t)(NT / WAVE) * 16 +
                  (NT / WAVE) * 4 + 64;
  if (rpn.lds_bytes > 160 * 1024 - 512) return rpn.fail("LDS");
  rpn.e_slots.alloc((size_t)G * cap_slots);
  rpn.sums.alloc((size_t)G);
  rpn.y_slots = DevBuf<double>();
  rpn.h_nruns = nruns;
  rpn.h_diag.clear();
  rpn.partials.alloc((size_t)2 * ((size_t)zero_run + 1));
  MFM_HIP_CHECK(hipMemsetAsync(rpn.partials.p, 0, (size_t)16 * ((size_t)zero_run + 1), s));
  rpn.dv.alloc((size_t)2 * (n_items + 1));
  rpn.bar.alloc(RES_BAR_WORDS);
  MFM_HIP_CHECK(hipStreamSynchronize(s));
  MFM_HIP_CHECK(hipGetLastError());
  lap("descriptors, buffers");
  rpn.ready = true;
  rpn.why.clear();
  return true;
}

static inline std::string res_plan_compare(const ResPlan &a, const ResPlan &b, hipStream_t s) {
  if (a.G != b.G || a.RV != b.RV || a.RL != b.RL || a.RX != b.RX || a.umax != b.umax || a.item_bits != b.item_bits || a.n_items != b.n_items ||
      a.n_rows != b.n_rows || a.n_runs != b.n_runs || a.lds_bytes != b.lds_bytes || a.max_wg_users != b.max_wg_users ||
      a.max_slice_items != b.max_slice_items)
    return "scalars";
  auto same = [&](const void *p, size_t np, const void *q, size_t nq, size_t elem) {
    if (np != nq) return false;
    std::vector<char> x(np * elem), y(nq * elem);
    if (np) {
      MFM_HIP_CHECK(hipMemcpyAsync(x.data(), p, np * elem, hipMemcpyDeviceToHost, s));
      MFM_HIP_CHECK(hipMemcpyAsync(y.data(), q, nq * elem, hipMemcpyDeviceToHost, s));
    }
    MFM_HIP_CHECK(hipStreamSynchronize(s));
    return x == y;
  };
#define MFM_RP_CMP(f) \
  if (!same(a.f.p, a.f.n, b.f.p, b.f.n, sizeof(*a.f.p))) return #f;
  MFM_RP_CMP(perm)
  MFM_RP_CMP(first_run)
  MFM_RP_CMP(wg_run_ptr)
  MFM_RP_CMP(wg_nruns)
  MFM_RP_CMP(wg_user_ptr)
  MFM_RP_CMP(wg_item_ptr)
  MFM_RP_CMP(ent_ptr)
  MFM_RP_CMP(scols)
  MFM_RP_CMP(entries)
  MFM_RP_CMP(uidw)
  MFM_RP_CMP(headw)
  MFM_RP_CMP(run_item)
  MFM_RP_CMP(user_desc)
  MFM_RP_CMP(item_desc)
  MFM_RP_CMP(run_feat)
  MFM_RP_CMP(wg_fill)
#undef MFM_RP_CMP
  return "";
}

}
```

Baseline: 344.0.

## Precompute next factor's squared-coefficient sums during current factor's sweep B phase

Adds an S2B variant of the resident MF kernel that widens the per-item dv record to four doubles, carrying the next factor's squared coefficient. The sum of c² per user is then accumulated into a third LDS accumulator during the previous factor's second pass, so the first pass of each factor drops one LDS atomic per nonzero. It spends extra LDS (one more per-wave user array) and twice the dv footprint, and adds a prologue pass to seed the first factor. It is enabled only for the RV=64/RL=16 plan when LDS allows.

```diff
diff --git a/include/myfm_hip.h b/include/myfm_hip.h
--- a/include/myfm_hip.h
+++ b/include/myfm_hip.h
@@ -58,7 +58,7 @@
 int64_t mfm_dim_all(const mfm_ctx *ctx);
 int mfm_plan_info(const mfm_ctx *ctx, int64_t *n_levels_main, int64_t *n_launches_per_sweep);
 int mfm_plan_flags(const mfm_ctx *ctx);
-#define MFM_RES_INFO_FIELDS 13
+#define MFM_RES_INFO_FIELDS 15
 int mfm_res_info(const mfm_ctx *ctx, int64_t *out, int n_out, char *why, int why_len);
 #define MFM_CELL_INFO_FIELDS 74
 int mfm_cell_info(const mfm_ctx *ctx, int64_t *out, int n_out, char *why, int why_len);
diff --git a/myfm_amd/_capi.py b/myfm_amd/_capi.py
--- a/myfm_amd/_capi.py
+++ b/myfm_amd/_capi.py
@@ -439,7 +439,7 @@
                 "fused_next": bool(f & 32), "sharded_fused": bool(f & 64), "mf": bool(f & 128), "resident": bool(f & 256), "cell": bool(f & 512), "streamed_chain": bool(f & 1024), "resident_overflow": bool(f & 2048)}
 
     RES_INFO = ("ready", "G", "RV", "RL", "RX", "umax", "n_items", "item_bits", "n_runs", "max_wg_users", "max_slice_items",
-                "e_where", "n_rows")
+                "e_where", "n_rows", "s2_in_sweep_b", "lds_bytes")
     E_WHERE = ("rows", "slots", "slots_with_sums", "cell", "dropped")
 
     def res_info(self):
diff --git a/myfm_amd/csrc/mfm_hip.hip b/myfm_amd/csrc/mfm_hip.hip
--- a/myfm_amd/csrc/mfm_hip.hip
+++ b/myfm_amd/csrc/mfm_hip.hip
@@ -1599,7 +1599,7 @@
   const ResPlan &rp = ctx->res;
   const int64_t v[MFM_RES_INFO_FIELDS] = {rp.ready ? 1 : 0, rp.G,       rp.RV,     rp.RL,           rp.RX,
                                           rp.umax,          rp.n_items, rp.item_bits, rp.n_runs,    rp.max_wg_users,
-                                          rp.max_slice_items, (int64_t)ctx->e_where, rp.n_rows};
+                                          rp.max_slice_items, (int64_t)ctx->e_where, rp.n_rows, rp.s2b, (int64_t)rp.lds_bytes};
   for (int i = 0; i < n_out; i++) out[i] = i < MFM_RES_INFO_FIELDS ? v[i] : 0;
   if (why_len > 0) {
     std::strncpy(why, rp.ready ? "" : rp.why.c_str(), (size_t)why_len - 1);
diff --git a/myfm_amd/csrc/mfm_res.hpp b/myfm_amd/csrc/mfm_res.hpp
--- a/myfm_amd/csrc/mfm_res.hpp
+++ b/myfm_amd/csrc/mfm_res.hpp
@@ -5,6 +5,7 @@
 #include <atomic>
 #include <string>
 #include <thread>
+#include <type_traits>
 #include <vector>
 
 #include "mfm_common.hpp"
@@ -153,8 +154,13 @@
 
 typedef double res_d16_t __attribute__((ext_vector_type(16)));
 typedef unsigned res_u4_t __attribute__((ext_vector_type(4)));
-
-template <int NT, int NGV, int NGL, bool XCH = false, bool OVF = false>
+typedef double res_d2u_t __attribute__((ext_vector_type(2), aligned(8)));
+__device__ __forceinline__ double res_cc0(double x) { return x; }
+__device__ __forceinline__ double res_cc1(double) { return 0.0; }
+__device__ __forceinline__ double res_cc0(res_d2u_t x) { return x[0]; }
+__device__ __forceinline__ double res_cc1(res_d2u_t x) { return x[1]; }
+
+template <int NT, int NGV, int NGL, bool XCH = false, bool OVF = false, bool S2B = false>
 __global__ __launch_bounds__(NT) void k_mf_resident(ResArgs a) {
   extern __shared__ __attribute__((aligned(16))) char res_smem[];
   constexpr int NW = NT / WAVE, NG = NGV + NGL, R = 16 * NG, RL = 16 * NGL;
@@ -168,15 +174,17 @@
   double *elds = (double *)(utab + U);
   double *acc1 = elds + (size_t)RL * NT;
   double *acc2 = acc1 + NW * U;
-  d2_t *wcarry = (d2_t *)(acc2 + NW * U);
+  double *acc3 = acc2 + NW * U;
+  d2_t *wcarry = (d2_t *)(acc2 + (S2B ? 2 : 1) * NW * U);
   int *wflag = (int *)(wcarry + NW);
   const int32_t *perm_g = a.perm + (int64_t)g * Rt * NT;
   const int u0 = a.wg_user_ptr[g], nu = a.wg_user_ptr[g + 1] - u0;
   const int rb0 = a.wg_run_ptr[g];
   const int pad_item = a.n_items;
-  const unsigned rb0b = 4u * (unsigned)rb0, padb = 16u * (unsigned)pad_item;
+  constexpr int DSH = S2B ? 5 : 4;
+  const unsigned rb0b = 4u * (unsigned)rb0, padb = (unsigned)pad_item << DSH;
   const char *run_item_b = (const char *)a.run_item, *dv_b = (const char *)a.dv;
-  double *acc1w = acc1 + wv * U, *acc2w = acc2 + wv * U;
+  double *acc1w = acc1 + wv * U, *acc2w = acc2 + wv * U, *acc3w = acc3 + wv * U;
   bool dead = false;
   unsigned long long nbar = 0;
   ResBar rbar;
@@ -197,7 +205,7 @@
 #define RES_STAMP(k)                                                                                      \
   if (a.prof && tid == 0) a.prof[((int64_t)g * a.n_sw + (f - f_first)) * 64 + (k)] = __builtin_amdgcn_s_memrealtime()
 
-  for (int i = tid; i < 2 * NW * U; i += NT) acc1[i] = 0.0;
+  for (int i = tid; i < (S2B ? 3 : 2) * NW * U; i += NT) acc1[i] = 0.0;
   for (int i = tid; i < U; i += NT) utab[i] = d2_t{0.0, 0.0};
 
   res_u4_t uw[NG];
@@ -270,6 +278,31 @@
     }
   }
   __syncthreads();
+  if (S2B) {
+    const uint32_t *uidw_p = a.uidw + (int64_t)g * (5 * NGt) * NT + tid;
+    const uint32_t *headw_p = a.headw + (int64_t)g * NGt * NT + tid;
+    int run = run0 - 1;
+    double c = 0.0;
+#pragma unroll 1
+    for (int jp = 0; jp < NGt; jp++) {
+      const unsigned nb = headw_p[jp * NT] | (jp == 0 ? 1u : 0u);
+      const unsigned uxp = uidw_p[(5 * jp + 4) * NT];
+#pragma unroll 1
+      for (int bb = 0; bb < 4; bb++) {
+        const unsigned lo_ = uidw_p[(5 * jp + bb) * NT];
+#pragma unroll 1
+        for (int k = 0; k < B; k++) {
+          if ((nb >> (4 * bb + k)) & 1u) {
+            run++;
+            c = a.dv[((int64_t)a.run_item[run] << (DSH - 3)) + 1];
+          }
+          const int uid = k < 3 ? (int)((lo_ >> (10 * k)) & 0x3ffu) : (int)((lo_ >> 30) | (((uxp >> (8 * bb)) & 0xffu) << 2));
+          __hip_atomic_fetch_add(&acc3w[uid], c * c, __ATOMIC_RELAXED, __HIP_MEMORY_SCOPE_WORKGROUP);
+        }
+      }
+    }
+    __syncthreads();
+  }
 
   RES_STAMP0(2);
   const int f_first = a.f_begin - a.linear;
@@ -310,7 +343,7 @@
           itA[k] = *(const int *)(run_item_b + ((n1 >> k) & 1u ? rcb : rb0b));
         }
 #pragma unroll
-        for (int k = 0; k < B; k++) ddA[k] = *(const d2_t *)(dv_b + ((n0 >> k) & 1u ? (unsigned)it0[k] << 4 : padb));
+        for (int k = 0; k < B; k++) ddA[k] = *(const d2_t *)(dv_b + ((n0 >> k) & 1u ? (unsigned)it0[k] << DSH : padb));
       }
       d2_t ddc = d2_t{0.0, 0.0};
       int itB[B];
@@ -323,7 +356,7 @@
       ito[k] = *(const int *)(run_item_b + ((n4b >> k) & 1u ? rcb : rb0b));                                                \
     }                                                                                                                      \
     _Pragma("unroll") for (int k = 0; k < B; k++)                                                                          \
-      ddo[k] = *(const d2_t *)(dv_b + ((n4a >> k) & 1u ? (unsigned)iti[k] << 4 : padb));                                   \
+      ddo[k] = *(const d2_t *)(dv_b + ((n4a >> k) & 1u ? (unsigned)iti[k] << DSH : padb));                                 \
     int uid[B];                                                                                                            \
     RES_UIDS(j, bb, uid);                                                                                                  \
     double up[B], ex[B];                                                                                                   \
@@ -342,7 +375,7 @@
         elds[(16 * (j - NGV) + 4 * (bb) + k) * NT + tid] = er;                                                             \
       const double c = ddc[1];                                                                                             \
       __hip_atomic_fetch_add(&acc1w[uid[k]], (-er) * c, __ATOMIC_RELAXED, __HIP_MEMORY_SCOPE_WORKGROUP);                   \
-      __hip_atomic_fetch_add(&acc2w[uid[k]], c * c, __ATOMIC_RELAXED, __HIP_MEMORY_SCOPE_WORKGROUP);                       \
+      if (!S2B) __hip_atomic_fetch_add(&acc2w[uid[k]], c * c, __ATOMIC_RELAXED, __HIP_MEMORY_SCOPE_WORKGROUP);             \
     }                                                                                                                      \
   }
 #define RES_STEP_AX(bb, iti, ito, ddi, ddo)                                                                                 \
@@ -353,7 +386,7 @@
       ito[k] = *(const int *)(run_item_b + ((n4b >> k) & 1u ? rcb : rb0b));                                                \
     }                                                                                                                      \
     _Pragma("unroll") for (int k = 0; k < B; k++)                                                                          \
-      ddo[k] = *(const d2_t *)(dv_b + ((n4a >> k) & 1u ? (unsigned)iti[k] << 4 : padb));                                   \
+      ddo[k] = *(const d2_t *)(dv_b + ((n4a >> k) & 1u ? (unsigned)iti[k] << DSH : padb));                                 \
     int uid[B];                                                                                                            \
     RES_UIDSX(bb, uid);                                                                                                      \
     double up[B], ex[B];                                                                                                   \
@@ -369,7 +402,7 @@
       eo[4 * (bb) + k] = er;                                                             \
       const double c = ddc[1];                                                                                             \
       __hip_atomic_fetch_add(&acc1w[uid[k]], (-er) * c, __ATOMIC_RELAXED, __HIP_MEMORY_SCOPE_WORKGROUP);                   \
-      __hip_atomic_fetch_add(&acc2w[uid[k]], c * c, __ATOMIC_RELAXED, __HIP_MEMORY_SCOPE_WORKGROUP);                       \
+      if (!S2B) __hip_atomic_fetch_add(&acc2w[uid[k]], c * c, __ATOMIC_RELAXED, __HIP_MEMORY_SCOPE_WORKGROUP);             \
     }                                                                                                                      \
   }
 #pragma unroll
@@ -413,10 +446,11 @@
       double S1 = 0.0, S2 = 0.0;
 #pragma unroll
       for (int w = 0; w < NW; w++) {
+        double *accS = S2B ? acc3 : acc2;
         S1 += acc1[w * U + tid];
-        S2 += acc2[w * U + tid];
+        S2 += accS[w * U + tid];
         acc1[w * U + tid] = 0.0;
-        acc2[w * U + tid] = 0.0;
+        accS[w * U + tid] = 0.0;
       }
       const double fresh = PMainV::draw(S1, S2, uold, alpha_k, ulam, umu, uz);
       Vf[uj] = fresh;
@@ -430,6 +464,9 @@
     __syncthreads();
     RES_STAMP(2);
     {
+      typedef typename std::conditional<S2B, res_d2u_t, double>::type cc_t;
+#define RES_CC0(x) res_cc0(x)
+#define RES_CC1(x) res_cc1(x)
       bool have_head = false;
       double f1 = 0.0, f2 = 0.0, s1 = 0.0, s2 = 0.0;
       d2_t *part2 = (d2_t *)a.partials;
@@ -441,7 +478,7 @@
         unsigned rcb = 4u * (unsigned)(run0 - 1);
         unsigned rcCb = 16u * (unsigned)(run0 - 1);
         int itA[B];
-        double ccA[B];
+        cc_t ccA[B];
         {
           int it0[B];
           const unsigned n0 = RES_NIB(0, 0), n1 = RES_NIB(0, 1);
@@ -456,11 +493,11 @@
             itA[k] = *(const int *)(run_item_b + ((n1 >> k) & 1u ? rcb : rb0b));
           }
 #pragma unroll
-          for (int k = 0; k < B; k++) ccA[k] = *(const double *)(dv_b + 8 + ((n0 >> k) & 1u ? (unsigned)it0[k] << 4 : padb));
-        }
-        double ccc = 0.0;
+          for (int k = 0; k < B; k++) ccA[k] = *(const cc_t *)(dv_b + 8 + ((n0 >> k) & 1u ? (unsigned)it0[k] << DSH : padb));
+        }
+        double ccc = 0.0, cqc = 0.0;
         int itB[B];
-        double ccB[B];
+        cc_t ccB[B];
 #define RES_PARTIAL_STORE() *(d2_t *)(part_b + (head && have_head ? rcCb : trashb)) = d2_t{s1, s2}
 #define RES_STEP_B(j, bb, iti, ito, cci, cco)                                                                              \
   {                                                                                                                        \
@@ -471,7 +508,7 @@
       ito[k] = *(const int *)(run_item_b + ((n4b >> k) & 1u ? rcb : rb0b));                                                \
     }                                                                                                                      \
     _Pragma("unroll") for (int k = 0; k < B; k++)                                                                          \
-      cco[k] = *(const double *)(dv_b + 8 + ((n4a >> k) & 1u ? (unsigned)iti[k] << 4 : padb));                             \
+      cco[k] = *(const cc_t *)(dv_b + 8 + ((n4a >> k) & 1u ? (unsigned)iti[k] << DSH : padb));                             \
     int uid[B];                                                                                                            \
     RES_UIDS(j, bb, uid);                                                                                                  \
     d2_t ut[B];                                                                                                            \
@@ -483,7 +520,11 @@
     _Pragma("unroll") for (int k = 0; k < B; k++) {                                                                        \
       const bool need = ((n4 >> k) & 1u) != 0u;                                                                            \
       const bool head = ((h4 >> k) & 1u) != 0u;                                                                            \
-      ccc = need ? cci[k] : ccc;                                                                                           \
+      ccc = need ? RES_CC0(cci[k]) : ccc;                                                                                  \
+      if (S2B) {                                                                                                           \
+        cqc = need ? RES_CC1(cci[k]) : cqc;                                                                                \
+        __hip_atomic_fetch_add(&acc3w[uid[k]], cqc, __ATOMIC_RELAXED, __HIP_MEMORY_SCOPE_WORKGROUP);                       \
+      }                                                                                                                    \
       rcCb += need ? 16u : 0u;                                                         \
                               \
       RES_PARTIAL_STORE();                                                                                                 \
@@ -508,7 +549,7 @@
       ito[k] = *(const int *)(run_item_b + ((n4b >> k) & 1u ? rcb : rb0b));                                                \
     }                                                                                                                      \
     _Pragma("unroll") for (int k = 0; k < B; k++)                                                                          \
-      cco[k] = *(const double *)(dv_b + 8 + ((n4a >> k) & 1u ? (unsigned)iti[k] << 4 : padb));                             \
+      cco[k] = *(const cc_t *)(dv_b + 8 + ((n4a >> k) & 1u ? (unsigned)iti[k] << DSH : padb));                             \
     int uid[B];                                                                                                            \
     RES_UIDSX(bb, uid);                                                                                                      \
     d2_t ut[B];                                                                                                            \
@@ -520,7 +561,11 @@
     _Pragma("unroll") for (int k = 0; k < B; k++) {                                                                        \
       const bool need = ((n4 >> k) & 1u) != 0u;                                                                            \
       const bool head = ((h4 >> k) & 1u) != 0u;                                                                            \
-      ccc = need ? cci[k] : ccc;                                                                                           \
+      ccc = need ? RES_CC0(cci[k]) : ccc;                                                                                  \
+      if (S2B) {                                                                                                           \
+        cqc = need ? RES_CC1(cci[k]) : cqc;                                                                                \
+        __hip_atomic_fetch_add(&acc3w[uid[k]], cqc, __ATOMIC_RELAXED, __HIP_MEMORY_SCOPE_WORKGROUP);                       \
+      }                                                                                                                    \
       rcCb += need ? 16u : 0u;                                                         \
                               \
       RES_PARTIAL_STORE();                                                                                                 \
@@ -569,6 +614,8 @@
         }
 #undef RES_STEP_B
 #undef RES_STEP_BX
+#undef RES_CC0
+#undef RES_CC1
 #undef RES_PARTIAL_STORE
       }
       if (a.prof && lane == 0)
@@ -612,13 +659,14 @@
     const int i0 = a.wg_item_ptr[g], ni = a.wg_item_ptr[g + 1] - i0;
     const bool more = f + 1 < a.f_end;
     int ij = 0;
-    double iold = 0.0, iz = 0.0, ivn = 0.0, ilam = 0.0, imu = 0.0;
+    double iold = 0.0, iz = 0.0, ivn = 0.0, ivq = 0.0, ilam = 0.0, imu = 0.0;
     if (tid < ni) {
       const int2 d = a.item_desc[i0 + tid];
       ij = d.x;
       iold = Vf[ij];
       iz = zf[ij];
       ivn = more ? a.V[(int64_t)(f + 1) * a.D + ij] : 0.0;
+      if (S2B) ivq = f + 2 < a.f_end ? a.V[(int64_t)(f + 2) * a.D + ij] : 0.0;
       ilam = lamf[d.y];
       imu = muf[d.y];
     }
@@ -695,7 +743,8 @@
       if (tid < ni) {
         const double fresh = PMainV::draw(S1, S2, iold, alpha_k, ilam, imu, iz);
         Vf[ij] = fresh;
-        res_store2(a.dv + 2 * (int64_t)(i0 + tid), fresh - iold, ivn);
+        res_store2(a.dv + ((int64_t)(i0 + tid) << (DSH - 3)), fresh - iold, ivn);
+        if (S2B) __hip_atomic_store(a.dv + 4 * (int64_t)(i0 + tid) + 2, ivq * ivq, __ATOMIC_RELAXED, __HIP_MEMORY_SCOPE_AGENT);
       }
     }
     RES_STAMP(5);
@@ -722,7 +771,7 @@
         RES_UIDS(j, bb, uid);
 #pragma unroll
         for (int k = 0; k < B; k++) {
-          const double dl = a.dv[2 * (int64_t)it[k]];
+          const double dl = a.dv[(int64_t)it[k] << (DSH - 3)];
           const double ex = j < NGV ? ev[j < NGV ? j : 0][4 * bb + k] : elds[(16 * (j - NGV) + 4 * bb + k) * NT + tid];
           const double ef = ex + utab[uid[k]][0] * dl;
           if (a.e_slots)
@@ -751,7 +800,7 @@
           RES_UIDSX(bb, uid);
 #pragma unroll
           for (int k = 0; k < B; k++) {
-            const double dl = a.dv[2 * (int64_t)it[k]];
+            const double dl = a.dv[(int64_t)it[k] << (DSH - 3)];
             double *ep = eog + (16 * jx + 4 * bb + k) * NT;
             *ep = *ep + utab[uid[k]][0] * dl;
           }
@@ -770,10 +819,23 @@
 }
 
 __global__ void k_res_init_dv(const double *__restrict__ theta, const int32_t *__restrict__ scols, int n_items,
-                              double *__restrict__ dv, unsigned long long *__restrict__ bar) {
+                              double *__restrict__ dv, unsigned long long *__restrict__ bar, int wide = 0,
+                              const double *__restrict__ theta2 = nullptr) {
   const int i = blockIdx.x * blockDim.x + threadIdx.x;
   if (blockIdx.x == 0)
     for (int k = threadIdx.x; k < RES_BAR_WORDS; k += blockDim.x) bar[k] = 0ull;
+  if (wide) {
+    if (i < n_items) {
+      const double c2 = theta2 ? theta2[scols[i]] : 0.0;
+      dv[4 * i] = 0.0;
+      dv[4 * i + 1] = theta ? theta[scols[i]] : 1.0;
+      dv[4 * i + 2] = c2 * c2;
+      dv[4 * i + 3] = 0.0;
+    } else if (i == n_items) {
+      for (int k = 0; k < 4; k++) dv[4 * i + k] = 0.0;
+    }
+    return;
+  }
   if (i < n_items) {
     dv[2 * i] = 0.0;
     dv[2 * i + 1] = theta ? theta[scols[i]] : 1.0;
@@ -985,6 +1047,15 @@
   bool allow_overflow = true;
   int64_t n_rows = 0, n_runs = 0;
   size_t lds_bytes = 0;
+  int s2b = 0;
+  bool plan_lds() {
+    const size_t nw = (size_t)(NT / WAVE), lim = 160 * 1024 - 512;
+    lds_bytes = (size_t)RL * NT * 8 + 2 * nw * umax * 8 + (size_t)umax * 16 + nw * 16 + nw * 4 + 64;
+    if (lds_bytes > lim) return false;
+    s2b = allow_overflow && RV == 64 && RL == 16 && lds_bytes + nw * umax * 8 <= lim ? 1 : 0;
+    if (s2b) lds_bytes += nw * umax * 8;
+    return true;
+  }
   DevBuf<int32_t> perm, first_run, wg_run_ptr, wg_nruns, wg_user_ptr, wg_item_ptr, ent_ptr, scols;
   DevBuf<int2> entries;
   DevBuf<uint32_t> uidw, headw;
@@ -1343,8 +1414,7 @@
         }
     }
     if (h_entries.size() >= ((size_t)1 << 31)) return fail("too many entries");
-    lds_bytes = (size_t)RL * NT * 8 + (size_t)2 * (NT / WAVE) * umax * 8 + (size_t)umax * 16 + (size_t)(NT / WAVE) * 16 + (NT / WAVE) * 4 + 64;
-    if (lds_bytes > 160 * 1024 - 512) return fail("LDS");
+    if (!plan_lds()) return fail("LDS");
     uidw.upload(h_uidw);
     headw.upload(h_headw);
     run_item.upload(h_run_item);
@@ -1414,7 +1484,7 @@
     }
     partials.alloc((size_t)2 * ((size_t)zero_run + 1));
     MFM_HIP_CHECK(hipMemset(partials.p, 0, (size_t)16 * ((size_t)zero_run + 1)));
-    dv.alloc((size_t)2 * (n_items + 1));
+    dv.alloc((size_t)(s2b ? 4 : 2) * (n_items + 1));
     bar.alloc(RES_BAR_WORDS);
     ready = true;
     why.clear();
@@ -1435,7 +1505,8 @@
   else if (rp.RV == 32 && rp.RL == 0)
     fn = (const void *)k_mf_resident<512, 2, 0>;
   else if (rp.RV == 64 && rp.RL == 16)
-    fn = rp.RX ? (const void *)k_mf_resident<512, 4, 1, false, true> : (const void *)k_mf_resident<512, 4, 1>;
+    fn = rp.s2b ? (rp.RX ? (const void *)k_mf_resident<512, 4, 1, false, true, true> : (const void *)k_mf_resident<512, 4, 1, false, false, true>)
+                : (rp.RX ? (const void *)k_mf_resident<512, 4, 1, false, true> : (const void *)k_mf_resident<512, 4, 1>);
   else
     return hipErrorInvalidValue;
   hipError_t e = hipFuncSetAttribute(fn, hipFuncAttributeMaxDynamicSharedMemorySize, 160 * 1024);
@@ -1520,9 +1591,12 @@
   const int K = a.n_sw;
   double bytes = (8.0 + (load_slots ? 0.0 : 4.0) + 1.4 + (no_store ? 0.0 : 8.0)) * rp.n_rows + K * 48.0 * rp.n_runs;
   if (rp.RX) bytes += (double)K * (16.0 + 1.75) * (double)rp.G * rp.NT * rp.RX;
-  hipLaunchKernelGGL(k_res_init_dv, dim3((rp.n_items + 256) / 256), dim3(256), 0, s,
-                     w ? (const double *)nullptr : V + (int64_t)f_begin * D, rp.scols.p, rp.n_items,
-                     rp.dv.p, rp.bar.p);
+  {
+    const int f_second = f_begin + (w ? 0 : 1);
+    hipLaunchKernelGGL(k_res_init_dv, dim3((rp.n_items + 256) / 256), dim3(256), 0, s,
+                       w ? (const double *)nullptr : V + (int64_t)f_begin * D, rp.scols.p, rp.n_items,
+                       rp.dv.p, rp.bar.p, rp.s2b, rp.s2b && f_second < f_end ? V + (int64_t)f_second * D : (const double *)nullptr);
+  }
   TimedLaunch t(tm, s, kernel_class, bytes);
 #define MFM_RES_LAUNCH(RV_, RL_)                                                                                              \
   do {                                                                                                                        \
@@ -1548,7 +1622,19 @@
     MFM_RES_LAUNCH(16, 0);
   else if (rp.RV == 32 && rp.RL == 0)
     MFM_RES_LAUNCH(32, 0);
-  else if (rp.RV == 64 && rp.RL == 16 && rp.RX > 0) {
+  else if (rp.RV == 64 && rp.RL == 16 && rp.s2b) {
+    if (xch) throw Error(MFM_ERR_RUNTIME, "internal: no row-sharded resident kernel of the S2B form");
+    static DeviceOnce raised_s;
+    if (raised_s.need()) {
+      MFM_HIP_CHECK(hipFuncSetAttribute((const void *)k_mf_resident<512, 4, 1, false, false, true>, hipFuncAttributeMaxDynamicSharedMemorySize, 160 * 1024));
+      MFM_HIP_CHECK(hipFuncSetAttribute((const void *)k_mf_resident<512, 4, 1, false, true, true>, hipFuncAttributeMaxDynamicSharedMemorySize, 160 * 1024));
+      raised_s.mark();
+    }
+    if (rp.RX > 0)
+      hipLaunchKernelGGL((k_mf_resident<512, 4, 1, false, true, true>), dim3(rp.G), dim3(512), rp.lds_bytes, s, a);
+    else
+      hipLaunchKernelGGL((k_mf_resident<512, 4, 1, false, false, true>), dim3(rp.G), dim3(512), rp.lds_bytes, s, a);
+  } else if (rp.RV == 64 && rp.RL == 16 && rp.RX > 0) {
     if (xch) throw Error(MFM_ERR_RUNTIME, "internal: no row-sharded resident kernel with overflow slots");
     static DeviceOnce raised_o;
     if (raised_o.need()) {
diff --git a/myfm_amd/csrc/mfm_res_plan.hpp b/myfm_amd/csrc/mfm_res_plan.hpp
--- a/myfm_amd/csrc/mfm_res_plan.hpp
+++ b/myfm_amd/csrc/mfm_res_plan.hpp
@@ -476,9 +476,7 @@
     for (int g = 0; g < G; g++) h_fill[g] = h_rowcut[g + 1] - h_rowcut[g];
     rpn.wg_fill.upload(h_fill);
   }
-  rpn.lds_bytes = (size_t)rpn.RL * NT * 8 + (size_t)2 * (NT / WAVE) * rpn.umax * 8 + (size_t)rpn.umax * 16 + (size_t)(NT / WAVE) * 16 +
-                  (NT / WAVE) * 4 + 64;
-  if (rpn.lds_bytes > 160 * 1024 - 512) return rpn.fail("LDS");
+  if (!rpn.plan_lds()) return rpn.fail("LDS");
   rpn.e_slots.alloc((size_t)G * cap_slots);
   rpn.sums.alloc((size_t)G);
   rpn.y_slots = DevBuf<double>();
@@ -486,7 +484,7 @@
   rpn.h_diag.clear();
   rpn.partials.alloc((size_t)2 * ((size_t)zero_run + 1));
   MFM_HIP_CHECK(hipMemsetAsync(rpn.partials.p, 0, (size_t)16 * ((size_t)zero_run + 1), s));
-  rpn.dv.alloc((size_t)2 * (n_items + 1));
+  rpn.dv.alloc((size_t)(rpn.s2b ? 4 : 2) * (n_items + 1));
   rpn.bar.alloc(RES_BAR_WORDS);
   MFM_HIP_CHECK(hipStreamSynchronize(s));
   MFM_HIP_CHECK(hipGetLastError());
@@ -498,7 +496,7 @@
 
 static inline std::string res_plan_compare(const ResPlan &a, const ResPlan &b, hipStream_t s) {
   if (a.G != b.G || a.RV != b.RV || a.RL != b.RL || a.RX != b.RX || a.umax != b.umax || a.item_bits != b.item_bits || a.n_items != b.n_items ||
-      a.n_rows != b.n_rows || a.n_runs != b.n_runs || a.lds_bytes != b.lds_bytes || a.max_wg_users != b.max_wg_users ||
+      a.n_rows != b.n_rows || a.n_runs != b.n_runs || a.lds_bytes != b.lds_bytes || a.s2b != b.s2b || a.max_wg_users != b.max_wg_users ||
       a.max_slice_items != b.max_slice_items)
     return "scalars";
   auto same = [&](const void *p, size_t np, const void *q, size_t nq, size_t elem) {
```

Result: faster. 376.8, median of 6 (+9.5%).
